# zhm1205/Multimodal_TTA

Hardware: AMD Instinct MI355X
Metric: adapted volumes/sec (higher is better)
Workload: dtype bf16

## Files before the change

include/mmtta.h:

```cpp
#ifndef MMTTA_H
#define MMTTA_H

#include <stdint.h>

#ifdef __cplusplus
extern "C" {
#endif

#define MMTTA_ABI_VERSION 2

typedef enum {
  MMTTA_OK = 0,
  MMTTA_ERR_INVALID = -1,
  MMTTA_ERR_UNSUPPORTED = -2,
  MMTTA_ERR_LAUNCH = -3,
  MMTTA_ERR_WORKSPACE = -4
} mmtta_status;

typedef enum { MMTTA_F32 = 0, MMTTA_BF16 = 1 } mmtta_dtype;

typedef struct {
  void* ptr;
  int32_t n, c, d, h, w;
  int64_t sn, sc, sd, sh, sw;
  int32_t dtype;
  int32_t flags;
} mmtta_tensor;

#define MMTTA_TENSOR_OWNS_PAD 1

#define MMTTA_ACT_NONE 0
#define MMTTA_ACT_RELU 1
#define MMTTA_ACT_LEAKY_RELU 2
typedef struct {
  const float* mean;
  const float* rstd;
  const float* gamma;
  const float* beta;
  int32_t relu;
  int32_t per_item;
  const float* scale;
  const float* shift;
  float negative_slope;
  int32_t _pad2;
} mmtta_norm_on_load;

const char* mmtta_last_error(void);
int mmtta_abi_version(void);

#define MMTTA_OPT_PROFILE_MAIN_KERNEL_ONLY 1
#define MMTTA_OPT_SPLITK_BELOW 2
#define MMTTA_OPT_SPLITK_TARGET 3
#define MMTTA_OPT_WGRAD_WORKGROUPS 4
#define MMTTA_OPT_WGRAD_THIN_SLABS 5
#define MMTTA_OPT_IGEMM_PIPELINE 6
#define MMTTA_OPT_EPILOGUE_VEC16 9
#define MMTTA_OPT_IGEMM_LEAN 10
#define MMTTA_OPT_WGRAD_VECTOR_STAGING 11
#define MMTTA_OPT_CLASS_FUSED_MIN_WORKGROUPS 12
#define MMTTA_OPT_THIN_MFMA 13
#define MMTTA_OPT_IGEMM_FRAGMENT_REUSE 14
int mmtta_set_option(int key, int value);

int mmtta_copy_strided(const mmtta_tensor* src, const mmtta_tensor* dst, void* stream);

typedef enum {
  MMTTA_CONV_FWD = 0,
  MMTTA_CONV_DGRAD = 1,
  MMTTA_CONVT_FWD = 2,
  MMTTA_CONVT_DGRAD = 3
} mmtta_conv_op;

typedef struct {
  int32_t op;
  int32_t ksize;
  int32_t stride;
  int32_t cin;
  int32_t cout;
  int32_t dtype;
} mmtta_conv_desc;

int64_t mmtta_conv_packed_bytes(const mmtta_conv_desc* desc);

int mmtta_conv_pack_weights(const mmtta_conv_desc* desc, const float* w_master, void* packed, void* stream);

typedef struct {
  mmtta_conv_desc desc;
  const float* w_master;
  void* packed;
} mmtta_pack_item;
int64_t mmtta_conv_pack_table_bytes(int count);
int mmtta_conv_pack_table_build(const mmtta_pack_item* items, int count, void* table_host, int64_t* total);
int mmtta_conv_pack_batched(const void* table_dev, int count, int64_t total, void* stream);

typedef struct {
  int32_t tiles;
  int32_t launches;
  int32_t ksplit;
  int32_t stats_rows;
  int32_t config;
  int32_t _pad;
  int64_t workspace_bytes;
} mmtta_conv_plan_t;

int mmtta_conv_plan(const mmtta_conv_desc* desc, const mmtta_tensor* x, const mmtta_tensor* y,
                    mmtta_conv_plan_t* plan);

typedef struct {
  const mmtta_tensor* add;
  mmtta_norm_on_load add_norm;
} mmtta_conv_epilogue;

int mmtta_conv_run(const mmtta_conv_desc* desc, const mmtta_tensor* x, const mmtta_norm_on_load* x_norm,
                   const void* packed, const float* bias, const mmtta_conv_epilogue* epi,
                   const mmtta_tensor* y, int accumulate, float* stats, void* workspace,
                   int64_t workspace_bytes, void* stream);

int mmtta_conv_route(const mmtta_conv_desc* desc, const mmtta_tensor* x, const mmtta_norm_on_load* x_norm,
                     const mmtta_conv_epilogue* epi, const mmtta_tensor* y, int accumulate, const float* stats);

typedef struct {
  int32_t items_per_set;
  int32_t inner;
  int64_t packed_outer, packed_inner;
  int64_t weight_outer, weight_inner;
  int64_t bias_outer, bias_inner;
} mmtta_param_sets;

int mmtta_conv_run_sets(const mmtta_conv_desc* desc, const mmtta_tensor* x, const mmtta_norm_on_load* x_norm,
                        const void* packed, const float* bias, const mmtta_conv_epilogue* epi,
                        const mmtta_tensor* y, int accumulate, float* stats, void* workspace,
                        int64_t workspace_bytes, const mmtta_param_sets* sets, void* stream);

int64_t mmtta_conv_wgrad_workspace_bytes(const mmtta_conv_desc* desc, const mmtta_tensor* x,
                                         const mmtta_tensor* dy);
int mmtta_conv_wgrad_kernel(const mmtta_conv_desc* desc, const mmtta_tensor* x, const mmtta_tensor* dy);
int mmtta_conv_wgrad(const mmtta_conv_desc* desc, const mmtta_tensor* x, const mmtta_norm_on_load* x_norm,
                     const mmtta_tensor* dy, float* dw, float* db, int accumulate, void* workspace,
                     int64_t workspace_bytes, void* stream);

int64_t mmtta_conv_wgrad_workspace_bytes_sets(const mmtta_conv_desc* desc, const mmtta_tensor* x, const mmtta_tensor* dy,
                                              const mmtta_param_sets* sets);
int mmtta_conv_wgrad_sets(const mmtta_conv_desc* desc, const mmtta_tensor* x, const mmtta_norm_on_load* x_norm,
                          const mmtta_tensor* dy, float* dw, float* db, int accumulate, void* workspace,
                          int64_t workspace_bytes, const mmtta_param_sets* sets, void* stream);
int mmtta_conv_wgrad_plan_sets(const mmtta_conv_desc* desc, const mmtta_tensor* x, const mmtta_tensor* dy,
                               const mmtta_param_sets* sets, int32_t plan[4]);

typedef struct {
  int32_t clip, zscore, masked, min_count;
  float lo, hi, mask_gt, eps;
  float mean, std;
  int32_t legacy, _pad;
} mmtta_intensity_rule;
int64_t mmtta_intensity_scratch_bytes(int channels);
int mmtta_intensity_normalize(const mmtta_tensor* x, const mmtta_intensity_rule* rules, const mmtta_tensor* y,
                              void* scratch, void* stream);

typedef enum {
  MMTTA_NORM_INSTANCE = 0,
  MMTTA_NORM_BATCH = 1,
  MMTTA_NORM_GROUP = 2
} mmtta_norm_kind;

int mmtta_norm_stats_finalize(int kind, int groups, const float* part, int rows_per_n, int n, int c,
                              int64_t count, float eps, int training, float* running_mean,
                              float* running_var, float momentum, float* mean, float* rstd,
                              const float* gamma, const float* beta, float* scale, float* shift,
                              double* scratch, void* stream);

typedef struct {
  int32_t items_per_set;
  int32_t _pad;
  int64_t affine_stride;
  int64_t stats_stride;
} mmtta_norm_sets;

int mmtta_norm_stats_finalize_sets(int kind, int groups, const float* part, int rows_per_n, int n, int c,
                                   int64_t count, float eps, int training, float* running_mean,
                                   float* running_var, float momentum, float* mean, float* rstd,
                                   const float* gamma, const float* beta, float* scale, float* shift,
                                   float* gamma_items, float* beta_items, double* scratch,
                                   const mmtta_norm_sets* sets, void* stream);

int mmtta_reduce_rows_per_n(const mmtta_tensor* t);

int mmtta_channel_stats(const mmtta_tensor* x, float* part, void* stream);

int mmtta_combine(const mmtta_tensor* a, const mmtta_norm_on_load* ta, const mmtta_tensor* b,
                  const mmtta_norm_on_load* tb, const mmtta_tensor* out, void* stream);

int mmtta_norm_bwd_reduce(const mmtta_tensor* dout, const mmtta_tensor* y, const mmtta_norm_on_load* t,
                          float* part, void* stream);

int mmtta_norm_bwd_finalize(int kind, int groups, const float* part, int rows_per_n, int n, int c, int64_t count,
                            const float* gamma, int training, float* m1, float* m2, float* dgamma,
                            float* dbeta, int accumulate, double* scratch , void* stream);

int mmtta_norm_bwd_finalize_sets(int kind, int groups, const float* part, int rows_per_n, int n, int c, int64_t count,
                                 const float* gamma, int training, float* m1, float* m2, float* dgamma,
                                 float* dbeta, int accumulate, double* scratch ,
                                 const mmtta_norm_sets* sets, void* stream);

int mmtta_norm_bwd_apply(const mmtta_tensor* dout, const mmtta_tensor* y, const mmtta_norm_on_load* t,
                         const float* m1, const float* m2, const mmtta_tensor* dy, void* stream);

int mmtta_norm_bwd_small_ok(const mmtta_tensor* dout, const mmtta_tensor* y, const mmtta_norm_on_load* t,
                            const mmtta_tensor* dy);
int mmtta_norm_bwd_small(const mmtta_tensor* dout, const mmtta_tensor* y, const mmtta_norm_on_load* t, int64_t count,
                         const mmtta_tensor* dy, void* stream);

int mmtta_upsample2x_fwd(const mmtta_tensor* x, const mmtta_tensor* y, void* stream);
int mmtta_upsample2x_bwd(const mmtta_tensor* dy, const mmtta_tensor* dx, int accumulate, void* stream);

int mmtta_lincomb(int count, const mmtta_tensor* const* in, const float* w, const mmtta_tensor* out,
                  int accumulate, void* stream);

#define MMTTA_PW_OP_CHANNEL_STATS 0
#define MMTTA_PW_OP_NORM_BWD_REDUCE 1
#define MMTTA_PW_OP_NORM_BWD_APPLY 2
#define MMTTA_PW_OP_NORM_BWD_SMALL 3
#define MMTTA_PW_OP_COMBINE 4
#define MMTTA_PW_OP_LINCOMB 5
#define MMTTA_PW_OP_UPSAMPLE_FWD 6
#define MMTTA_PW_OP_UPSAMPLE_BWD 7
#define MMTTA_PW_REDUCE 0
#define MMTTA_PW_REDUCE_STREAM 1
#define MMTTA_PW_ELEMENTWISE 2
#define MMTTA_PW_COMBINE8 3
#define MMTTA_PW_NORM_BWD_APPLY8 4
#define MMTTA_PW_NORM_BWD_SMALL 5
#define MMTTA_PW_LINCOMB 6
#define MMTTA_PW_UPSAMPLE_FWD 7
#define MMTTA_PW_UPSAMPLE_BWD 8
typedef struct {
  int64_t vox_per_row;
  int64_t work_items;
  int64_t grid_x;
  int32_t grid_y;
  int32_t family;
  int32_t mode;
  int32_t vec;
  int32_t it;
  int32_t count;
  int32_t bf16_a;
  int32_t bf16_b;
  int32_t bf16_o;
  int32_t has_b;
  int32_t rows_per_n;
  int32_t rows_per_block;
  int32_t cpl, nvl;
  int32_t trips;
  int32_t cb_passes;
  int32_t second_trip;
  int32_t leaky;
} mmtta_pointwise_route_t;
int mmtta_pointwise_route(int op, const mmtta_tensor* const* operands, int count, const mmtta_norm_on_load* t,
                          const mmtta_norm_on_load* t2, const float* m1, const float* m2, mmtta_pointwise_route_t* out);

int64_t mmtta_entropy_partials(const mmtta_tensor* logits);
int mmtta_entropy_loss(const mmtta_tensor* logits, int softmax, const mmtta_tensor* dlogits,
                       double* partial, float* loss, void* stream);

int64_t mmtta_entropy_partials_items(const mmtta_tensor* logits);
int mmtta_entropy_loss_items(const mmtta_tensor* logits, int softmax, const mmtta_tensor* dlogits,
                             double* partial, float* loss, void* stream);

int64_t mmtta_entropy_filtered_partials(const mmtta_tensor* logits);
int mmtta_entropy_filtered_items(const mmtta_tensor* logits, int softmax, float margin, const uint8_t* keep_in,
                                 uint8_t* keep_out, const mmtta_tensor* dlogits, double* partial, float* loss,
                                 int64_t* kept, void* stream);

int mmtta_mirror_views(const mmtta_tensor* x, const mmtta_tensor* y, int views, const int32_t* view_axes, void* stream);
int64_t mmtta_memo_partials(const mmtta_tensor* logits, int views);
int mmtta_memo_loss_items(const mmtta_tensor* logits, int softmax, int views, const int32_t* view_axes,
                          const mmtta_tensor* dlogits, double* partial, float* loss, void* stream);
int mmtta_memo_ensemble(const mmtta_tensor* logits, int softmax, int views, const int32_t* view_axes,
                        const mmtta_tensor* out, void* stream);

int64_t mmtta_consistency_partials(const mmtta_tensor* logits);
int mmtta_consistency_loss_items(const mmtta_tensor* logits, const mmtta_tensor* target, int softmax,
                                 const mmtta_tensor* dlogits, double* partial, float* loss, void* stream);
int64_t mmtta_cotta_update_partials(int64_t n, int sets);
int mmtta_cotta_update_sets(float* w, float* teacher, const float* source, int64_t n, int sets, int64_t w_stride,
                            int64_t teacher_stride, double alpha, float restore_p, uint64_t seed, const int32_t* step,
                            const int32_t* ordinals, int64_t* partial, int64_t* restored, void* stream);

int64_t mmtta_intensity_range_partials(const mmtta_tensor* x);
int mmtta_intensity_range(const mmtta_tensor* x, float* partial, float* range, void* stream);
int mmtta_augment_views(const mmtta_tensor* x, const mmtta_tensor* y, int views, const int32_t* view_axes,
                        const float* table_host, const float* table, const float* range, uint64_t seed,
                        const int32_t* ordinals, void* stream);

int64_t mmtta_entropy_weighted_partials(const mmtta_tensor* logits);
int mmtta_entropy_weighted_items(const mmtta_tensor* logits, int softmax, float margin, uint8_t* keep_out,
                                 const mmtta_tensor* dlogits, double* partial, float* loss, int64_t* kept, void* stream);
int64_t mmtta_pseudo_label_partials(const mmtta_tensor* logits);
int mmtta_pseudo_label_loss_items(const mmtta_tensor* logits, int softmax, const mmtta_tensor* dlogits, double* partial,
                                  float* loss, void* stream);
int mmtta_fisher_accumulate_sets(float* fisher, const float* grads, int64_t n, int sets, int64_t set_stride, void* stream);
int mmtta_fisher_scale(float* fisher, int64_t n, float count, void* stream);
int64_t mmtta_fisher_penalty_partials(int64_t n, int sets);
int mmtta_fisher_penalty_sets(const float* w, float* g, const float* fisher, const float* source, int64_t n, int sets,
                              int replicas, int64_t set_stride, float lambda, double* partial, float* penalty, void* stream);

int mmtta_adam_step(float* p, const float* g, float* m, float* v, int64_t n, int64_t n_decay, float lr,
                    float beta1, float beta2, float eps, float weight_decay, int32_t* step, void* stream);

enum { MMTTA_OPTIM_ADAM = 0, MMTTA_OPTIM_ADAMW = 1, MMTTA_OPTIM_SGD = 2 };
typedef struct mmtta_optim_desc {
  int32_t kind;
  float lr, beta1, beta2, eps, weight_decay;
  float momentum, dampening;
  int32_t nesterov;
} mmtta_optim_desc;
int mmtta_optim_step(const mmtta_optim_desc* desc, float* p, const float* g, float* m, float* v, int64_t n,
                     int64_t n_decay, int32_t* step, void* stream);

int mmtta_optim_step_sets(const mmtta_optim_desc* desc, float* p, const float* g, float* m, float* v, int64_t n,
                          int64_t n_decay, int sets, int64_t set_stride, int32_t* step, void* stream);

typedef struct mmtta_update_target {
  mmtta_optim_desc optim;
  float* w_p; float* w_m; float* w_v;
  float* b_p; float* b_m; float* b_v;
  float* b_grad;
  void* image[2];
  int64_t image_outer[2], image_inner[2];
  const int32_t* step;
  int32_t w_decay, b_decay;
} mmtta_update_target;
int mmtta_fused_update_enabled(void);
int mmtta_conv_wgrad_update_sets(const mmtta_conv_desc* desc, const mmtta_tensor* x, const mmtta_norm_on_load* x_norm,
                                 const mmtta_tensor* dy, const mmtta_update_target* target, void* workspace,
                                 int64_t workspace_bytes, const mmtta_param_sets* sets, void* stream);

int mmtta_optim_step_segments(const mmtta_optim_desc* desc, float* p, const float* g, float* m, float* v, const int64_t* segments,
                              int count, int64_t total, int sets, int64_t set_stride, int32_t* step, void* stream);

int64_t mmtta_sam_ascent_partials(int64_t n, int sets);
int mmtta_sam_ascent_sets(float* p, const float* g, float* saved, int64_t saved_stride, double* partial, int64_t n, int sets,
                          int replicas, int64_t set_stride, float rho, void* stream);

int mmtta_mask_dice_counts(const mmtta_tensor* logits, const mmtta_tensor* label, float threshold,
                           int64_t* counts, uint8_t* mask, void* stream);

int64_t mmtta_dice_ce_scratch_bytes(const mmtta_tensor* logits);
int mmtta_dice_ce_sums(const mmtta_tensor* logits, const mmtta_tensor* label, const float* weight,
                       int squared_pred, int softmax, double* out, void* scratch, void* stream);

int mmtta_dice_ce_grad(const mmtta_tensor* logits, const mmtta_tensor* label, const float* weight, int squared_pred,
                       int softmax, int jaccard, int include_background, float lambda_dice, float lambda_ce, float smooth_nr,
                       float smooth_dr, const double* sums, const mmtta_tensor* dlogits, void* stream);

int64_t mmtta_calibration_scratch_bytes(const mmtta_tensor* logits, int bins);
int mmtta_calibration_bins(const mmtta_tensor* logits, const mmtta_tensor* label, int softmax, int bins, int scope,
                           double* out, void* scratch, void* stream);

int64_t mmtta_components_scratch_bytes(int64_t n_masks, int64_t d, int64_t h, int64_t w);
int mmtta_components_filter(const uint8_t* mask_in, uint8_t* mask_out, const mmtta_tensor* label, int n, int r, int d, int h,
                            int w, int connectivity, const int64_t* min_voxels, const int32_t* keep_largest, int64_t* counts,
                            int64_t* stats, int32_t* labels, void* scratch, void* stream);

int64_t mmtta_lesionwise_scratch_bytes(int64_t n_masks, int64_t d, int64_t h, int64_t w);
int mmtta_lesionwise_scores(const uint8_t* mask, const mmtta_tensor* label, int n, int r, int d, int h, int w, int iterations,
                            int dilation_connectivity, const int64_t* min_lesion_voxels, int64_t* stats, int32_t* labels,
                            void* scratch, void* stream);

int64_t mmtta_mask_fill_nest_scratch_bytes(int64_t n_masks, int64_t d, int64_t h, int64_t w);
int mmtta_mask_fill_nest(uint8_t* mask, const mmtta_tensor* label, int n, int r, int d, int h, int w, int fill_connectivity,
                         const int32_t* fill_holes, const int64_t* max_hole_voxels, const int32_t* chain, int chain_len,
                         int nest_mode, int64_t* counts, int64_t* stats, void* scratch, void* stream);

int64_t mmtta_surface_scratch_bytes(int64_t n_masks, int64_t d, int64_t h, int64_t w);
int mmtta_surface_distances(const uint8_t* pred_mask, const mmtta_tensor* label, const double* spacing,
                            double percentile, int asd_symmetric, float* hd, float* asd, void* scratch, void* stream);

#ifdef __cplusplus
}
#endif
#endif
```

multimodal_tta_amd/_lib.py:

```python
from __future__ import annotations

import ctypes as C
import os
from typing import Optional, Sequence

import torch

_HERE = os.path.dirname(os.path.abspath(__file__))
LIB_PATH = os.path.join(_HERE, "csrc", "libmmtta.so")

F32, BF16 = 0, 1
CONV_FWD, CONV_DGRAD, CONVT_FWD, CONVT_DGRAD = 0, 1, 2, 3
NORM_INSTANCE, NORM_BATCH, NORM_GROUP = 0, 1, 2


class MmttaError(RuntimeError):
    pass


class Tensor(C.Structure):
    _fields_ = [
        ("ptr", C.c_void_p),
        ("n", C.c_int32), ("c", C.c_int32), ("d", C.c_int32), ("h", C.c_int32), ("w", C.c_int32),
        ("sn", C.c_int64), ("sc", C.c_int64), ("sd", C.c_int64), ("sh", C.c_int64), ("sw", C.c_int64),
        ("dtype", C.c_int32), ("flags", C.c_int32),
    ]


class NormOnLoad(C.Structure):
    _fields_ = [
        ("mean", C.c_void_p), ("rstd", C.c_void_p), ("gamma", C.c_void_p), ("beta", C.c_void_p),
        ("relu", C.c_int32), ("per_item", C.c_int32), ("scale", C.c_void_p), ("shift", C.c_void_p),
    ]


class NormOnLoadAct(NormOnLoad):
    _fields_ = [("negative_slope", C.c_float), ("_pad2", C.c_int32)]


class NormSets(C.Structure):
    _fields_ = [("items_per_set", C.c_int32), ("_pad", C.c_int32), ("affine_stride", C.c_int64), ("stats_stride", C.c_int64)]


class ConvDesc(C.Structure):
    _fields_ = [
        ("op", C.c_int32), ("ksize", C.c_int32), ("stride", C.c_int32), ("cin", C.c_int32), ("cout", C.c_int32),
        ("dtype", C.c_int32),
    ]


class PackItem(C.Structure):
    _fields_ = [("desc", ConvDesc), ("w_master", C.c_void_p), ("packed", C.c_void_p)]


class ParamSets(C.Structure):
    _fields_ = [("items_per_set", C.c_int32), ("inner", C.c_int32), ("packed_outer", C.c_int64), ("packed_inner", C.c_int64),
                ("weight_outer", C.c_int64), ("weight_inner", C.c_int64), ("bias_outer", C.c_int64), ("bias_inner", C.c_int64)]


class ConvPlan(C.Structure):
    _fields_ = [
        ("tiles", C.c_int32), ("launches", C.c_int32), ("ksplit", C.c_int32), ("stats_rows", C.c_int32),
        ("config", C.c_int32), ("_pad", C.c_int32), ("workspace_bytes", C.c_int64),
    ]


class PointwiseRoute(C.Structure):
    _fields_ = [("vox_per_row", C.c_int64), ("work_items", C.c_int64), ("grid_x", C.c_int64), ("grid_y", C.c_int32),
                ("family", C.c_int32), ("mode", C.c_int32), ("vec", C.c_int32), ("it", C.c_int32), ("count", C.c_int32),
                ("bf16_a", C.c_int32), ("bf16_b", C.c_int32), ("bf16_o", C.c_int32), ("has_b", C.c_int32),
                ("rows_per_n", C.c_int32), ("rows_per_block", C.c_int32), ("cpl", C.c_int32), ("nvl", C.c_int32),
                ("trips", C.c_int32), ("cb_passes", C.c_int32), ("second_trip", C.c_int32), ("leaky", C.c_int32)]


PW_OPS = ("channel_stats", "norm_bwd_reduce", "norm_bwd_apply", "norm_bwd_small", "combine", "lincomb", "upsample_fwd",
          "upsample_bwd")
PW_FAMILIES = ("reduce", "reduce_stream", "elementwise", "combine8", "norm_bwd_apply8", "norm_bwd_small", "lincomb",
               "upsample_fwd", "upsample_bwd")


class OptimDesc(C.Structure):
    _fields_ = [("kind", C.c_int32), ("lr", C.c_float), ("beta1", C.c_float), ("beta2", C.c_float), ("eps", C.c_float),
                ("weight_decay", C.c_float), ("momentum", C.c_float), ("dampening", C.c_float), ("nesterov", C.c_int32)]


class UpdateTarget(C.Structure):
    _fields_ = [("optim", OptimDesc), ("w_p", C.c_void_p), ("w_m", C.c_void_p), ("w_v", C.c_void_p), ("b_p", C.c_void_p),
                ("b_m", C.c_void_p), ("b_v", C.c_void_p), ("b_grad", C.c_void_p), ("image", C.c_void_p * 2),
                ("image_outer", C.c_int64 * 2), ("image_inner", C.c_int64 * 2), ("step", C.c_void_p),
                ("w_decay", C.c_int32), ("b_decay", C.c_int32)]


OPTIM_ADAM, OPTIM_ADAMW, OPTIM_SGD = 0, 1, 2


class ConvEpilogue(C.Structure):
    _fields_ = [("add", C.POINTER(Tensor)), ("add_norm", NormOnLoadAct)]


class IntensityRule(C.Structure):
    _fields_ = [("clip", C.c_int32), ("zscore", C.c_int32), ("masked", C.c_int32), ("min_count", C.c_int32),
                ("lo", C.c_float), ("hi", C.c_float), ("mask_gt", C.c_float), ("eps", C.c_float),
                ("mean", C.c_float), ("std", C.c_float), ("legacy", C.c_int32), ("_pad", C.c_int32)]


_P = C.POINTER
_SIGNATURES = {
    "mmtta_last_error": (C.c_char_p, []),
    "mmtta_abi_version": (C.c_int, []),
    "mmtta_set_option": (C.c_int, [C.c_int, C.c_int]),
    "mmtta_intensity_scratch_bytes": (C.c_int64, [C.c_int]),
    "mmtta_intensity_normalize": (C.c_int, [_P(Tensor), _P(IntensityRule), _P(Tensor), C.c_void_p, C.c_void_p]),
    "mmtta_copy_strided": (C.c_int, [_P(Tensor), _P(Tensor), C.c_void_p]),
    "mmtta_conv_packed_bytes": (C.c_int64, [_P(ConvDesc)]),
    "mmtta_conv_pack_weights": (C.c_int, [_P(ConvDesc), C.c_void_p, C.c_void_p, C.c_void_p]),
    "mmtta_conv_pack_table_bytes": (C.c_int64, [C.c_int]),
    "mmtta_conv_pack_table_build": (C.c_int, [_P(PackItem), C.c_int, C.c_void_p, _P(C.c_int64)]),
    "mmtta_conv_pack_batched": (C.c_int, [C.c_void_p, C.c_int, C.c_int64, C.c_void_p]),
    "mmtta_conv_plan": (C.c_int, [_P(ConvDesc), _P(Tensor), _P(Tensor), _P(ConvPlan)]),
    "mmtta_conv_run": (C.c_int, [_P(ConvDesc), _P(Tensor), _P(NormOnLoad), C.c_void_p, C.c_void_p, _P(ConvEpilogue),
                                 _P(Tensor), C.c_int, C.c_void_p, C.c_void_p, C.c_int64, C.c_void_p]),
    "mmtta_conv_run_sets": (C.c_int, [_P(ConvDesc), _P(Tensor), _P(NormOnLoad), C.c_void_p, C.c_void_p, _P(ConvEpilogue),
                                      _P(Tensor), C.c_int, C.c_void_p, C.c_void_p, C.c_int64, _P(ParamSets), C.c_void_p]),
    "mmtta_conv_route": (C.c_int, [_P(ConvDesc), _P(Tensor), _P(NormOnLoad), _P(ConvEpilogue), _P(Tensor), C.c_int, C.c_void_p]),
    "mmtta_conv_wgrad_workspace_bytes": (C.c_int64, [_P(ConvDesc), _P(Tensor), _P(Tensor)]),
    "mmtta_conv_wgrad_workspace_bytes_sets": (C.c_int64, [_P(ConvDesc), _P(Tensor), _P(Tensor), _P(ParamSets)]),
    "mmtta_conv_wgrad_plan_sets": (C.c_int, [_P(ConvDesc), _P(Tensor), _P(Tensor), _P(ParamSets), _P(C.c_int32)]),
    "mmtta_conv_wgrad_sets": (C.c_int, [_P(ConvDesc), _P(Tensor), _P(NormOnLoad), _P(Tensor), C.c_void_p, C.c_void_p,
                                        C.c_int, C.c_void_p, C.c_int64, _P(ParamSets), C.c_void_p]),
    "mmtta_conv_wgrad_kernel": (C.c_int, [_P(ConvDesc), _P(Tensor), _P(Tensor)]),
    "mmtta_conv_wgrad": (C.c_int, [_P(ConvDesc), _P(Tensor), _P(NormOnLoad), _P(Tensor), C.c_void_p, C.c_void_p,
                                   C.c_int, C.c_void_p, C.c_int64, C.c_void_p]),
    "mmtta_norm_stats_finalize": (C.c_int, [C.c_int, C.c_int, C.c_void_p, C.c_int, C.c_int, C.c_int, C.c_int64,
                                            C.c_float, C.c_int, C.c_void_p, C.c_void_p, C.c_float, C.c_void_p,
                                            C.c_void_p, C.c_void_p, C.c_void_p, C.c_void_p, C.c_void_p, C.c_void_p,
                                            C.c_void_p]),
    "mmtta_norm_stats_finalize_sets": (C.c_int, [C.c_int, C.c_int, C.c_void_p, C.c_int, C.c_int, C.c_int, C.c_int64,
                                                 C.c_float, C.c_int, C.c_void_p, C.c_void_p, C.c_float, C.c_void_p,
                                                 C.c_void_p, C.c_void_p, C.c_void_p, C.c_void_p, C.c_void_p, C.c_void_p,
                                                 C.c_void_p, C.c_void_p, _P(NormSets), C.c_void_p]),
    "mmtta_reduce_rows_per_n": (C.c_int, [_P(Tensor)]),
    "mmtta_channel_stats": (C.c_int, [_P(Tensor), C.c_void_p, C.c_void_p]),
    "mmtta_combine": (C.c_int, [_P(Tensor), _P(NormOnLoad), _P(Tensor), _P(NormOnLoad), _P(Tensor), C.c_void_p]),
    "mmtta_norm_bwd_reduce": (C.c_int, [_P(Tensor), _P(Tensor), _P(NormOnLoad), C.c_void_p, C.c_void_p]),
    "mmtta_norm_bwd_finalize": (C.c_int, [C.c_int, C.c_int, C.c_void_p, C.c_int, C.c_int, C.c_int, C.c_int64,
                                          C.c_void_p, C.c_int, C.c_void_p, C.c_void_p, C.c_void_p, C.c_void_p,
                                          C.c_int, C.c_void_p, C.c_void_p]),
    "mmtta_norm_bwd_finalize_sets": (C.c_int, [C.c_int, C.c_int, C.c_void_p, C.c_int, C.c_int, C.c_int, C.c_int64,
                                               C.c_void_p, C.c_int, C.c_void_p, C.c_void_p, C.c_void_p, C.c_void_p,
                                               C.c_int, C.c_void_p, _P(NormSets), C.c_void_p]),
    "mmtta_norm_bwd_apply": (C.c_int, [_P(Tensor), _P(Tensor), _P(NormOnLoad), C.c_void_p, C.c_void_p, _P(Tensor),
                                       C.c_void_p]),
    "mmtta_norm_bwd_small_ok": (C.c_int, [_P(Tensor), _P(Tensor), _P(NormOnLoad), _P(Tensor)]),
    "mmtta_norm_bwd_small": (C.c_int, [_P(Tensor), _P(Tensor), _P(NormOnLoad), C.c_int64, _P(Tensor), C.c_void_p]),
    "mmtta_upsample2x_fwd": (C.c_int, [_P(Tensor), _P(Tensor), C.c_void_p]),
    "mmtta_upsample2x_bwd": (C.c_int, [_P(Tensor), _P(Tensor), C.c_int, C.c_void_p]),
    "mmtta_lincomb": (C.c_int, [C.c_int, _P(_P(Tensor)), _P(C.c_float), _P(Tensor), C.c_int, C.c_void_p]),
    "mmtta_pointwise_route": (C.c_int, [C.c_int, _P(_P(Tensor)), C.c_int, _P(NormOnLoad), _P(NormOnLoad), C.c_void_p, C.c_void_p,
                                        _P(PointwiseRoute)]),
    "mmtta_entropy_partials": (C.c_int64, [_P(Tensor)]),
    "mmtta_entropy_loss": (C.c_int, [_P(Tensor), C.c_int, _P(Tensor), C.c_void_p, C.c_void_p, C.c_void_p]),
    "mmtta_entropy_partials_items": (C.c_int64, [_P(Tensor)]),
    "mmtta_entropy_loss_items": (C.c_int, [_P(Tensor), C.c_int, _P(Tensor), C.c_void_p, C.c_void_p, C.c_void_p]),
    "mmtta_entropy_filtered_partials": (C.c_int64, [_P(Tensor)]),
    "mmtta_entropy_filtered_items": (C.c_int, [_P(Tensor), C.c_int, C.c_float, C.c_void_p, C.c_void_p, _P(Tensor), C.c_void_p,
                                               C.c_void_p, C.c_void_p, C.c_void_p]),
    "mmtta_mirror_views": (C.c_int, [_P(Tensor), _P(Tensor), C.c_int, _P(C.c_int32), C.c_void_p]),
    "mmtta_memo_partials": (C.c_int64, [_P(Tensor), C.c_int]),
    "mmtta_memo_loss_items": (C.c_int, [_P(Tensor), C.c_int, C.c_int, _P(C.c_int32), _P(Tensor), C.c_void_p, C.c_void_p,
                                        C.c_void_p]),
    "mmtta_memo_ensemble": (C.c_int, [_P(Tensor), C.c_int, C.c_int, _P(C.c_int32), _P(Tensor), C.c_void_p]),
    "mmtta_consistency_partials": (C.c_int64, [_P(Tensor)]),
    "mmtta_consistency_loss_items": (C.c_int, [_P(Tensor), _P(Tensor), C.c_int, _P(Tensor), C.c_void_p, C.c_void_p, C.c_void_p]),
    "mmtta_cotta_update_partials": (C.c_int64, [C.c_int64, C.c_int]),
    "mmtta_cotta_update_sets": (C.c_int, [C.c_void_p, C.c_void_p, C.c_void_p, C.c_int64, C.c_int, C.c_int64, C.c_int64,
                                          C.c_double, C.c_float, C.c_uint64, C.c_void_p, C.c_void_p, C.c_void_p, C.c_void_p,
                                          C.c_void_p]),
    "mmtta_intensity_range_partials": (C.c_int64, [_P(Tensor)]),
    "mmtta_intensity_range": (C.c_int, [_P(Tensor), C.c_void_p, C.c_void_p, C.c_void_p]),
    "mmtta_augment_views": (C.c_int, [_P(Tensor), _P(Tensor), C.c_int, _P(C.c_int32), C.c_void_p, C.c_void_p, C.c_void_p,
                                      C.c_uint64, C.c_void_p, C.c_void_p]),
    "mmtta_entropy_weighted_partials": (C.c_int64, [_P(Tensor)]),
    "mmtta_entropy_weighted_items": (C.c_int, [_P(Tensor), C.c_int, C.c_float, C.c_void_p, _P(Tensor), C.c_void_p, C.c_void_p,
                                               C.c_void_p, C.c_void_p]),
    "mmtta_pseudo_label_partials": (C.c_int64, [_P(Tensor)]),
    "mmtta_pseudo_label_loss_items": (C.c_int, [_P(Tensor), C.c_int, _P(Tensor), C.c_void_p, C.c_void_p, C.c_void_p]),
    "mmtta_fisher_accumulate_sets": (C.c_int, [C.c_void_p, C.c_void_p, C.c_int64, C.c_int, C.c_int64, C.c_void_p]),
    "mmtta_fisher_scale": (C.c_int, [C.c_void_p, C.c_int64, C.c_float, C.c_void_p]),
    "mmtta_fisher_penalty_partials": (C.c_int64, [C.c_int64, C.c_int]),
    "mmtta_fisher_penalty_sets": (C.c_int, [C.c_void_p, C.c_void_p, C.c_void_p, C.c_void_p, C.c_int64, C.c_int, C.c_int,
                                            C.c_int64, C.c_float, C.c_void_p, C.c_void_p, C.c_void_p]),
    "mmtta_adam_step": (C.c_int, [C.c_void_p, C.c_void_p, C.c_void_p, C.c_void_p, C.c_int64, C.c_int64, C.c_float,
                                  C.c_float, C.c_float, C.c_float, C.c_float, C.c_void_p, C.c_void_p]),
    "mmtta_optim_step": (C.c_int, [_P(OptimDesc), C.c_void_p, C.c_void_p, C.c_void_p, C.c_void_p, C.c_int64, C.c_int64,
                                   C.c_void_p, C.c_void_p]),
    "mmtta_optim_step_sets": (C.c_int, [_P(OptimDesc), C.c_void_p, C.c_void_p, C.c_void_p, C.c_void_p, C.c_int64, C.c_int64,
                                        C.c_int, C.c_int64, C.c_void_p, C.c_void_p]),
    "mmtta_optim_step_segments": (C.c_int, [_P(OptimDesc), C.c_void_p, C.c_void_p, C.c_void_p, C.c_void_p, C.c_void_p, C.c_int,
                                            C.c_int64, C.c_int, C.c_int64, C.c_void_p, C.c_void_p]),
    "mmtta_fused_update_enabled": (C.c_int, []),
    "mmtta_conv_wgrad_update_sets": (C.c_int, [_P(ConvDesc), _P(Tensor), _P(NormOnLoad), _P(Tensor), _P(UpdateTarget),
                                               C.c_void_p, C.c_int64, _P(ParamSets), C.c_void_p]),
    "mmtta_sam_ascent_partials": (C.c_int64, [C.c_int64, C.c_int]),
    "mmtta_sam_ascent_sets": (C.c_int, [C.c_void_p, C.c_void_p, C.c_void_p, C.c_int64, C.c_void_p, C.c_int64, C.c_int, C.c_int,
                                        C.c_int64, C.c_float, C.c_void_p]),
    "mmtta_mask_dice_counts": (C.c_int, [_P(Tensor), _P(Tensor), C.c_float, C.c_void_p, C.c_void_p, C.c_void_p]),
    "mmtta_dice_ce_scratch_bytes": (C.c_int64, [_P(Tensor)]),
    "mmtta_dice_ce_sums": (C.c_int, [_P(Tensor), _P(Tensor), C.c_void_p, C.c_int, C.c_int, C.c_void_p, C.c_void_p, C.c_void_p]),
    "mmtta_dice_ce_grad": (C.c_int, [_P(Tensor), _P(Tensor), C.c_void_p, C.c_int, C.c_int, C.c_int, C.c_int, C.c_float, C.c_float,
                                     C.c_float, C.c_float, C.c_void_p, _P(Tensor), C.c_void_p]),
    "mmtta_calibration_scratch_bytes": (C.c_int64, [_P(Tensor), C.c_int]),
    "mmtta_calibration_bins": (C.c_int, [_P(Tensor), _P(Tensor), C.c_int, C.c_int, C.c_int, C.c_void_p, C.c_void_p, C.c_void_p]),
    "mmtta_components_scratch_bytes": (C.c_int64, [C.c_int64, C.c_int64, C.c_int64, C.c_int64]),
    "mmtta_components_filter": (C.c_int, [C.c_void_p, C.c_void_p, _P(Tensor), C.c_int, C.c_int, C.c_int, C.c_int, C.c_int, C.c_int,
                                          _P(C.c_int64), _P(C.c_int32), C.c_void_p, C.c_void_p, C.c_void_p, C.c_void_p, C.c_void_p]),
    "mmtta_lesionwise_scratch_bytes": (C.c_int64, [C.c_int64, C.c_int64, C.c_int64, C.c_int64]),
    "mmtta_lesionwise_scores": (C.c_int, [C.c_void_p, _P(Tensor), C.c_int, C.c_int, C.c_int, C.c_int, C.c_int, C.c_int, C.c_int,
                                          _P(C.c_int64), C.c_void_p, C.c_void_p, C.c_void_p, C.c_void_p]),
    "mmtta_mask_fill_nest_scratch_bytes": (C.c_int64, [C.c_int64, C.c_int64, C.c_int64, C.c_int64]),
    "mmtta_mask_fill_nest": (C.c_int, [C.c_void_p, _P(Tensor), C.c_int, C.c_int, C.c_int, C.c_int, C.c_int, C.c_int, _P(C.c_int32),
                                       _P(C.c_int64), _P(C.c_int32), C.c_int, C.c_int, C.c_void_p, C.c_void_p, C.c_void_p, C.c_void_p]),
    "mmtta_surface_scratch_bytes": (C.c_int64, [C.c_int64, C.c_int64, C.c_int64, C.c_int64]),
    "mmtta_surface_distances": (C.c_int, [C.c_void_p, _P(Tensor), _P(C.c_double), C.c_double, C.c_int, C.c_void_p,
                                          C.c_void_p, C.c_void_p, C.c_void_p]),
}

_lib = None


def load() -> C.CDLL:
    global _lib
    if _lib is not None:
        return _lib
    if not os.path.exists(LIB_PATH):
        raise MmttaError(
            f"{LIB_PATH} is missing: build it with `python -m multimodal_tta_amd.build` (hipcc, gfx950). "
            "There is no CPU or PyTorch fallback for the adaptation path."
        )
    lib = C.CDLL(LIB_PATH)
    for name, (res, args) in _SIGNATURES.items():
        fn = getattr(lib, name)
        fn.restype = res
        fn.argtypes = args
    if lib.mmtta_abi_version() != 2:
        raise MmttaError("libmmtta.so ABI version mismatch")
    if os.environ.get("MMTTA_NO_PIPE", "0") == "1":
        lib.mmtta_set_option(6, 0)
    if os.environ.get("MMTTA_NO_EPIVEC", "0") == "1":
        lib.mmtta_set_option(9, 0)
    if "MMTTA_WGVEC" in os.environ:
        lib.mmtta_set_option(11, int(os.environ["MMTTA_WGVEC"]))
    if "MMTTA_THINMFMA" in os.environ:
        lib.mmtta_set_option(13, int(os.environ["MMTTA_THINMFMA"]))
    if "MMTTA_CLSFUSE" in os.environ:
        lib.mmtta_set_option(12, int(os.environ["MMTTA_CLSFUSE"]))
    if "MMTTA_LEAN" in os.environ:
        lib.mmtta_set_option(10, int(os.environ["MMTTA_LEAN"]))
    _lib = lib
    return lib


def exported_names() -> Sequence[str]:
    return list(_SIGNATURES)


def check(status: int, what: str = "") -> None:
    if status != 0:
        msg = load().mmtta_last_error().decode("utf-8", "replace")
        raise MmttaError(f"{what or 'libmmtta'} failed with status {status}: {msg}")


def stream_ptr() -> int:
    return int(torch.cuda.current_stream().cuda_stream)


def ptr(t: Optional[torch.Tensor]) -> Optional[int]:
    return None if t is None else int(t.data_ptr())


TENSOR_OWNS_PAD = 1


def desc_cl(t: torch.Tensor) -> Tensor:
    if t.dim() != 5 or t.dtype not in (torch.float32, torch.bfloat16) or not t.is_cuda:
        raise MmttaError(f"expected a CUDA float32 / bfloat16 [N,D,H,W,C] view, got {tuple(t.shape)} {t.dtype} {t.device}")
    n, d, h, w, c = t.shape
    sn, sd, sh, sw, sc = t.stride()
    if sc != 1 and c != 1:
        raise MmttaError("activation views must have unit stride along C")
    flags = TENSOR_OWNS_PAD if getattr(t, "_mmtta_owns_pad", False) else 0
    return Tensor(t.data_ptr(), n, c, d, h, w, sn, 1, sd, sh, sw, BF16 if t.dtype == torch.bfloat16 else F32, flags)


def desc_ncdhw(t: torch.Tensor) -> Tensor:
    if t.dim() != 5 or t.dtype != torch.float32 or not t.is_cuda:
        raise MmttaError(f"expected a CUDA float32 [N,C,D,H,W] tensor, got {tuple(t.shape)} {t.dtype} {t.device}")
    n, c, d, h, w = t.shape
    sn, sc, sd, sh, sw = t.stride()
    return Tensor(t.data_ptr(), n, c, d, h, w, sn, sc, sd, sh, sw, F32, 0)


ACT_NONE, ACT_RELU, ACT_LEAKY_RELU = 0, 1, 2


def norm_on_load(mean=None, rstd=None, gamma=None, beta=None, relu=False, scale=None, shift=None,
                 per_item=False, act=None, negative_slope=0.0) -> NormOnLoadAct:
    code = (ACT_RELU if relu else ACT_NONE) if act is None else int(act)
    return NormOnLoadAct(ptr(mean), ptr(rstd), ptr(gamma), ptr(beta), code, 1 if per_item else 0, ptr(scale),
                      ptr(shift), float(negative_slope) if code == ACT_LEAKY_RELU else 0.0, 0)
```

multimodal_tta_amd/csrc/api.hip:

```cpp
#include "common.h"
#include <string.h>

namespace mmtta {
static thread_local char g_err[512] = "";
void set_error(const char* fmt, ...) {
  va_list ap;
  va_start(ap, fmt);
  vsnprintf(g_err, sizeof(g_err), fmt, ap);
  va_end(ap);
}
int g_profile_main_only = 0;
int g_igemm_pipeline = 1;
int g_epilogue_vec = 1;
int g_igemm_lean = 1;
int g_igemm_reuse = 1;
int g_cls_fused_min = 128;
int g_thin_mfma = 2;
int g_wgrad_vec = 1;
int g_tune[4] = {96, 128, 128, 256};
}

extern "C" int mmtta_set_option(int key, int value) {
  if (key == MMTTA_OPT_PROFILE_MAIN_KERNEL_ONLY) {
    const int prev = mmtta::g_profile_main_only;
    mmtta::g_profile_main_only = value;
    return prev;
  }
  if (key == MMTTA_OPT_WGRAD_VECTOR_STAGING) {
    const int prev = mmtta::g_wgrad_vec;
    mmtta::g_wgrad_vec = value ? 1 : 0;
    return prev;
  }
  if (key == MMTTA_OPT_THIN_MFMA) {
    const int prev = mmtta::g_thin_mfma;
    mmtta::g_thin_mfma = value < 0 ? 0 : (value > 3 ? 3 : value);
    return prev;
  }
  if (key == MMTTA_OPT_CLASS_FUSED_MIN_WORKGROUPS) {
    const int prev = mmtta::g_cls_fused_min;
    mmtta::g_cls_fused_min = value < 0 ? 0 : value;
    return prev;
  }
  if (key == MMTTA_OPT_IGEMM_LEAN) {
    const int prev = mmtta::g_igemm_lean;
    mmtta::g_igemm_lean = value ? 1 : 0;
    return prev;
  }
  if (key == MMTTA_OPT_IGEMM_FRAGMENT_REUSE) {
    const int prev = mmtta::g_igemm_reuse;
    mmtta::g_igemm_reuse = value ? 1 : 0;
    return prev;
  }
  if (key == MMTTA_OPT_EPILOGUE_VEC16) {
    const int prev = mmtta::g_epilogue_vec;
    mmtta::g_epilogue_vec = value ? 1 : 0;
    return prev;
  }
  if (key == MMTTA_OPT_IGEMM_PIPELINE) {
    const int prev = mmtta::g_igemm_pipeline;
    mmtta::g_igemm_pipeline = value ? 1 : 0;
    return prev;
  }
  if (key >= MMTTA_OPT_SPLITK_BELOW && key <= MMTTA_OPT_WGRAD_THIN_SLABS) {
    if (value < 1) return MMTTA_ERR_INVALID;
    const int prev = mmtta::g_tune[key - MMTTA_OPT_SPLITK_BELOW];
    mmtta::g_tune[key - MMTTA_OPT_SPLITK_BELOW] = value;
    return prev;
  }
  return MMTTA_ERR_INVALID;
}

extern "C" const char* mmtta_last_error(void) { return mmtta::g_err; }
extern "C" int mmtta_abi_version(void) { return MMTTA_ABI_VERSION; }
```

multimodal_tta_amd/csrc/common.h:

```cpp
#pragma once
#include <hip/hip_runtime.h>
#include <type_traits>
#include <stdint.h>
#include <stdio.h>
#include <stdarg.h>
#include "../../include/mmtta.h"

namespace mmtta {

constexpr int WAVE = 64;

void set_error(const char* fmt, ...);

#define MMTTA_CHECK(cond, code, ...)      \
  do {                                    \
    if (!(cond)) {                        \
      ::mmtta::set_error(__VA_ARGS__);    \
      return (code);                      \
    }                                     \
  } while (0)

inline int launch_status(const char* what) {
  hipError_t e = hipGetLastError();
  if (e != hipSuccess) {
    set_error("%s: %s", what, hipGetErrorString(e));
    return MMTTA_ERR_LAUNCH;
  }
  return MMTTA_OK;
}

extern int g_profile_main_only;
extern int g_igemm_pipeline;
extern int g_wgrad_vec;
extern int g_igemm_lean;
extern int g_igemm_reuse;
extern int g_cls_fused_min;
extern int g_thin_mfma;
extern int g_epilogue_vec;
extern int g_tune[4];

inline bool nl_leaky(const mmtta_norm_on_load* t) { return t != nullptr && t->relu == MMTTA_ACT_LEAKY_RELU; }
inline int nl_act_check(const mmtta_norm_on_load* t, const char* what) {
  MMTTA_CHECK(t == nullptr || (t->relu >= MMTTA_ACT_NONE && t->relu <= MMTTA_ACT_LEAKY_RELU), MMTTA_ERR_INVALID,
              "%s: activation code %d (MMTTA_ACT_NONE, _RELU or _LEAKY_RELU)", what, t ? t->relu : 0);
  MMTTA_CHECK(t == nullptr || t->relu != MMTTA_ACT_LEAKY_RELU || __builtin_isfinite(t->negative_slope), MMTTA_ERR_INVALID,
              "%s: LeakyReLU negative_slope must be finite", what);
  return MMTTA_OK;
}

struct PackImageGeo {
  int A, B, T, Kp, Np, kn_is_ba, plain_bf16;
};
int pack_image_geometry(const mmtta_conv_desc* d, PackImageGeo& g);

#define MMTTA_ACT_BODIES                                                                                                    \
  int conv_run_body(const mmtta_conv_desc* d, const mmtta_tensor* x, const mmtta_norm_on_load* x_norm, const void* packed,  \
                    const float* bias, const mmtta_conv_epilogue* epi, const mmtta_tensor* y, int accumulate, float* stats, \
                    void* workspace, int64_t workspace_bytes, const mmtta_param_sets* sets, void* stream);                \
  int conv_wgrad_body(const mmtta_conv_desc* d, const mmtta_tensor* x, const mmtta_norm_on_load* x_norm,                    \
                      const mmtta_tensor* dy, float* dw, float* db, int accumulate, void* workspace,                        \
                      int64_t workspace_bytes, const mmtta_param_sets* sets, void* stream,                                  \
                      const mmtta_update_target* upd);                                                                      \
  int combine_body(const mmtta_tensor* a, const mmtta_norm_on_load* ta, const mmtta_tensor* b,                              \
                   const mmtta_norm_on_load* tb, const mmtta_tensor* out, void* stream);                                    \
  int norm_bwd_reduce_body(const mmtta_tensor* dout, const mmtta_tensor* y, const mmtta_norm_on_load* t, float* part,      \
                           void* stream);                                                                                   \
  int norm_bwd_apply_body(const mmtta_tensor* dout, const mmtta_tensor* y, const mmtta_norm_on_load* t, const float* m1,   \
                          const float* m2, const mmtta_tensor* dy, void* stream);                                           \
  int norm_bwd_small_body(const mmtta_tensor* dout, const mmtta_tensor* y, const mmtta_norm_on_load* t, int64_t count,     \
                          const mmtta_tensor* dy, void* stream);
namespace leaky { MMTTA_ACT_BODIES }

#ifdef MMTTA_ACT_LEAKY_TU
#define MMTTA_ACT_NS_OPEN namespace leaky {
#define MMTTA_ACT_NS_CLOSE }
#else
#define MMTTA_ACT_NS_OPEN
#define MMTTA_ACT_NS_CLOSE
#endif

MMTTA_ACT_NS_OPEN
MMTTA_ACT_BODIES

inline bool is_cl(const mmtta_tensor* t) { return t->sc == 1 || t->c == 1; }

inline bool is_f32(const mmtta_tensor* t) { return t->dtype == MMTTA_F32; }
inline bool is_bf16(const mmtta_tensor* t) { return t->dtype == MMTTA_BF16; }

inline bool quad_aligned(const mmtta_tensor* t, int base_bytes, int elems = 4) {
  return ((uintptr_t)t->ptr) % base_bytes == 0 && t->sw % elems == 0 && t->sh % elems == 0 && t->sd % elems == 0 &&
         t->sn % elems == 0;
}
inline int quad_bytes(const mmtta_tensor* t) { return is_bf16(t) ? 8 : 16; }
inline bool item_fits_31(const mmtta_tensor* t, int64_t pad) {
  const int64_t last = (int64_t)(t->d - 1) * t->sd + (int64_t)(t->h - 1) * t->sh + (int64_t)(t->w - 1) * t->sw + pad;
  return last < ((int64_t)1 << 31);
}
inline bool strides_fit_24(const mmtta_tensor* t) { return t->sw < (1 << 24) && t->sh < (1 << 24) && t->sd < (1 << 24); }
inline bool voxel_dense(const mmtta_tensor* t) { return t->sc == 1 && t->sh == (int64_t)t->w * t->sw && t->sd == (int64_t)t->h * t->sh; }
inline bool dense_rows16(const mmtta_tensor* t) {
  const int q = is_bf16(t) ? 8 : 4;
  return voxel_dense(t) && ((uintptr_t)t->ptr) % 16 == 0 && t->sw % q == 0 && t->sn % q == 0 &&
         (int64_t)t->d * t->h * t->w * t->sw < ((int64_t)1 << 31);
}
inline bool same_shape(const mmtta_tensor* a, const mmtta_tensor* b) {
  return a->n == b->n && a->c == b->c && a->d == b->d && a->h == b->h && a->w == b->w;
}

__device__ __forceinline__ float bf16_bits_to_f32(unsigned int h) { return __uint_as_float(h << 16); }
__device__ __forceinline__ unsigned int f32x2_to_bf16x2(float lo, float hi) {
  typedef __bf16 bf2 __attribute__((ext_vector_type(2)));
  bf2 v;
  v[0] = (__bf16)lo;
  v[1] = (__bf16)hi;
  return __builtin_bit_cast(unsigned int, v);
}
__device__ __forceinline__ unsigned short f32_to_bf16_bits(float v) { return __builtin_bit_cast(unsigned short, (__bf16)v); }
__device__ __forceinline__ uint4 bf16x8_pack(const unsigned short* h) {
  uint4 q;
  q.x = h[0] | ((unsigned)h[1] << 16); q.y = h[2] | ((unsigned)h[3] << 16);
  q.z = h[4] | ((unsigned)h[5] << 16); q.w = h[6] | ((unsigned)h[7] << 16);
  return q;
}
__device__ __forceinline__ float4 ld4_any(const float* base, long long eoff, int bf) {
  if (bf) {
    const uint2 u = *reinterpret_cast<const uint2*>(reinterpret_cast<const unsigned short*>(base) + eoff);
    return make_float4(bf16_bits_to_f32(u.x & 0xffffu), bf16_bits_to_f32(u.x >> 16), bf16_bits_to_f32(u.y & 0xffffu),
                       bf16_bits_to_f32(u.y >> 16));
  }
  return *reinterpret_cast<const float4*>(base + eoff);
}
__device__ __forceinline__ void st4_any(float* base, long long eoff, float4 v, int bf) {
  if (bf) {
    uint2 u;
    u.x = f32x2_to_bf16x2(v.x, v.y);
    u.y = f32x2_to_bf16x2(v.z, v.w);
    *reinterpret_cast<uint2*>(reinterpret_cast<unsigned short*>(base) + eoff) = u;
  } else {
    *reinterpret_cast<float4*>(base + eoff) = v;
  }
}
__device__ __forceinline__ float ld1_any(const float* base, long long eoff, int bf) {
  if (bf) return bf16_bits_to_f32(reinterpret_cast<const unsigned short*>(base)[eoff]);
  return base[eoff];
}
__device__ __forceinline__ void st1_any(float* base, long long eoff, float v, int bf) {
  if (bf) reinterpret_cast<unsigned short*>(base)[eoff] = (unsigned short)(f32x2_to_bf16x2(v, 0.f) & 0xffffu);
  else base[eoff] = v;
}
__device__ __forceinline__ void ld8_any(const float* base, long long eoff, int bf, float4& lo, float4& hi) {
  if (bf) {
    const uint4 u = *reinterpret_cast<const uint4*>(reinterpret_cast<const unsigned short*>(base) + eoff);
    lo = make_float4(bf16_bits_to_f32(u.x & 0xffffu), bf16_bits_to_f32(u.x >> 16), bf16_bits_to_f32(u.y & 0xffffu),
                     bf16_bits_to_f32(u.y >> 16));
    hi = make_float4(bf16_bits_to_f32(u.z & 0xffffu), bf16_bits_to_f32(u.z >> 16), bf16_bits_to_f32(u.w & 0xffffu),
                     bf16_bits_to_f32(u.w >> 16));
  } else {
    lo = *reinterpret_cast<const float4*>(base + eoff);
    hi = *reinterpret_cast<const float4*>(base + eoff + 4);
  }
}

template <bool BF> struct Oct8 { float4 lo, hi; };
template <> struct Oct8<true> { uint4 q; };
template <bool BF>
__device__ __forceinline__ Oct8<BF> oct8_ld(const float* base, unsigned eoff_lo, unsigned eoff_hi) {
  Oct8<BF> o;
  if constexpr (BF) {
    o.q = *reinterpret_cast<const uint4*>(reinterpret_cast<const unsigned short*>(base) + eoff_lo);
  } else {
    o.lo = *reinterpret_cast<const float4*>(base + eoff_lo);
    o.hi = *reinterpret_cast<const float4*>(base + eoff_hi);
  }
  return o;
}
__device__ __forceinline__ void oct8_f8(const Oct8<false>& o, float (&v)[8]) {
  v[0] = o.lo.x; v[1] = o.lo.y; v[2] = o.lo.z; v[3] = o.lo.w; v[4] = o.hi.x; v[5] = o.hi.y; v[6] = o.hi.z; v[7] = o.hi.w;
}
__device__ __forceinline__ void oct8_f8(const Oct8<true>& o, float (&v)[8]) {
  v[0] = bf16_bits_to_f32(o.q.x & 0xffffu); v[1] = __uint_as_float(o.q.x & 0xffff0000u);
  v[2] = bf16_bits_to_f32(o.q.y & 0xffffu); v[3] = __uint_as_float(o.q.y & 0xffff0000u);
  v[4] = bf16_bits_to_f32(o.q.z & 0xffffu); v[5] = __uint_as_float(o.q.z & 0xffff0000u);
  v[6] = bf16_bits_to_f32(o.q.w & 0xffffu); v[7] = __uint_as_float(o.q.w & 0xffff0000u);
}


template <bool BF>
__device__ __forceinline__ void oct8_st(float* base, unsigned eoff, const float (&v)[8]) {
  if constexpr (BF) {
    uint4 q;
    q.x = f32x2_to_bf16x2(v[0], v[1]); q.y = f32x2_to_bf16x2(v[2], v[3]);
    q.z = f32x2_to_bf16x2(v[4], v[5]); q.w = f32x2_to_bf16x2(v[6], v[7]);
    *reinterpret_cast<uint4*>(reinterpret_cast<unsigned short*>(base) + eoff) = q;
  } else {
    *reinterpret_cast<float4*>(base + eoff) = make_float4(v[0], v[1], v[2], v[3]);
    *reinterpret_cast<float4*>(base + eoff + 4) = make_float4(v[4], v[5], v[6], v[7]);
  }
}
template <bool BF>
__device__ __forceinline__ const float* item_base(const float* p, long long n, long long sn) {
  return BF ? reinterpret_cast<const float*>(reinterpret_cast<const unsigned short*>(p) + n * sn) : p + n * sn;
}

template <int I, int N, class F>
__device__ __forceinline__ void static_for(F&& f) {
  if constexpr (I < N) {
    f(std::integral_constant<int, I>{});
    static_for<I + 1, N>(f);
  }
}

template <int I, int N, int STEP, class F>
__device__ __forceinline__ void static_for_step(F&& f) {
  if constexpr (I < N) {
    f(std::integral_constant<int, I>{});
    static_for_step<I + STEP, N, STEP>(f);
  }
}

template <bool BF> __device__ __forceinline__ float4 ld4_t(const float* base, long long eoff) { return ld4_any(base, eoff, BF ? 1 : 0); }
template <bool BF> __device__ __forceinline__ float ld1_t(const float* base, long long eoff) { return ld1_any(base, eoff, BF ? 1 : 0); }
template <bool BF> __device__ __forceinline__ void st4_t(float* base, long long eoff, float4 v) { st4_any(base, eoff, v, BF ? 1 : 0); }
template <bool BF> __device__ __forceinline__ void st1_t(float* base, long long eoff, float v) { st1_any(base, eoff, v, BF ? 1 : 0); }
template <bool BF> __device__ __forceinline__ void ld8_t(const float* base, long long eoff, float4& lo, float4& hi) {
  ld8_any(base, eoff, BF ? 1 : 0, lo, hi);
}
#define MMTTA_BF_DISPATCH(flag, NAME, ...) \
  do {                                      \
    if (flag) {                             \
      constexpr bool NAME = true;           \
      __VA_ARGS__                           \
    } else {                                \
      constexpr bool NAME = false;          \
      __VA_ARGS__                           \
    }                                       \
  } while (0)

struct TV {
  float* p;
  int n, c, d, h, w;
  long long sn, sc, sd, sh, sw;
  int flags;
  int bf;
};

inline TV tv(const mmtta_tensor* t) {
  TV v;
  v.p = (float*)t->ptr;
  v.flags = t->flags;
  v.bf = t->dtype == MMTTA_BF16 ? 1 : 0;
  v.n = t->n; v.c = t->c; v.d = t->d; v.h = t->h; v.w = t->w;
  v.sn = t->sn; v.sc = t->sc; v.sd = t->sd; v.sh = t->sh; v.sw = t->sw;
  return v;
}

__device__ __forceinline__ void vox_decompose(const TV& t, long long v, int& n, int& z, int& y, int& x) {
  x = (int)(v % t.w); v /= t.w;
  y = (int)(v % t.h); v /= t.h;
  z = (int)(v % t.d);
  n = (int)(v / t.d);
}
__device__ __forceinline__ long long vox_addr(const TV& t, int n, int z, int y, int x) {
  return (long long)n * t.sn + (long long)z * t.sd + (long long)y * t.sh + (long long)x * t.sw;
}

#ifdef MMTTA_ACT_LEAKY_TU
typedef float act_t;
#define MMTTA_ACT_ID 1.f
#else
typedef int act_t;
#define MMTTA_ACT_ID 0
#endif
inline act_t act_arg(const mmtta_norm_on_load* t) {
#ifdef MMTTA_ACT_LEAKY_TU
  if (t == nullptr) return 1.f;
  return t->relu == MMTTA_ACT_LEAKY_RELU ? t->negative_slope : (t->relu == MMTTA_ACT_RELU ? 0.f : 1.f);
#else
  return t == nullptr ? 0 : t->relu;
#endif
}

struct NL {
  const float* mean;
  const float* rstd;
  const float* gamma;
  const float* beta;
  act_t relu;
  const float* scale;
  const float* shift;
};

inline NL nl(const mmtta_norm_on_load* t) {
  NL r;
  if (t == nullptr) { r.mean = r.rstd = r.gamma = r.beta = r.scale = r.shift = nullptr; r.relu = MMTTA_ACT_ID; return r; }
  r.mean = t->mean; r.rstd = t->rstd; r.gamma = t->gamma; r.beta = t->beta; r.relu = act_arg(t);
  r.scale = t->scale; r.shift = t->scale ? t->shift : nullptr;
  return r;
}
template <class Args>
inline int epilogue_add(const mmtta_conv_epilogue* epi, const mmtta_tensor* y, Args& a) {
  a.add = nullptr; a.asn = a.asd = a.ash = a.asw = 0; a.tadd = nl(nullptr);
  if (!(epi && epi->add)) return MMTTA_OK;
  const mmtta_tensor* ad = epi->add;
  MMTTA_CHECK(ad->ptr && is_cl(ad) && same_shape(ad, y), MMTTA_ERR_INVALID,
              "conv: epilogue `add` must be channels-last with the shape of y");
  a.add = (const float*)ad->ptr; a.asn = ad->sn; a.asd = ad->sd; a.ash = ad->sh; a.asw = ad->sw;
  a.tadd = nl(&epi->add_norm);
  return MMTTA_OK;
}
inline int nl_per_item_check(const mmtta_norm_on_load* t, const char* what) {
  MMTTA_CHECK(t == nullptr || t->per_item == 0 || t->mean == nullptr || t->scale != nullptr, MMTTA_ERR_INVALID,
              "%s: a norm-on-load with per-item gamma / beta needs its precombined scale / shift", what);
  return MMTTA_OK;
}

struct PSets {
  int ips, inner;
  long long packed_outer, packed_inner;
  long long weight_outer, weight_inner;
  long long bias_outer, bias_inner;
};

inline PSets psets(const mmtta_param_sets* g) {
  PSets r;
  if (g == nullptr) { r.ips = 1; r.inner = 1; r.packed_outer = r.packed_inner = r.weight_outer = r.weight_inner = r.bias_outer = r.bias_inner = 0; return r; }
  r.ips = g->items_per_set; r.inner = g->inner;
  r.packed_outer = g->packed_outer; r.packed_inner = g->packed_inner;
  r.weight_outer = g->weight_outer; r.weight_inner = g->weight_inner;
  r.bias_outer = g->bias_outer; r.bias_inner = g->bias_inner;
  return r;
}
inline int psets_validate(const mmtta_param_sets* g, int n) {
  if (g == nullptr) return MMTTA_OK;
  MMTTA_CHECK(g->items_per_set >= 1 && g->inner >= 1, MMTTA_ERR_INVALID, "param sets: items_per_set %d, inner %d (both >= 1)",
              g->items_per_set, g->inner);
  MMTTA_CHECK(n % g->items_per_set == 0, MMTTA_ERR_INVALID, "param sets: batch %d is no multiple of items_per_set %d", n,
              g->items_per_set);
  MMTTA_CHECK(g->packed_outer % 16 == 0 && g->packed_inner % 16 == 0 && g->weight_outer % 4 == 0 && g->weight_inner % 4 == 0 &&
                  g->bias_outer % 4 == 0 && g->bias_inner % 4 == 0,
              MMTTA_ERR_INVALID, "param sets: strides must keep 16-byte alignment");
  return MMTTA_OK;
}
__host__ __device__ __forceinline__ bool psets_on(const PSets& g) {
  return (g.packed_outer | g.packed_inner | g.weight_outer | g.weight_inner | g.bias_outer | g.bias_inner) != 0;
}
__device__ __forceinline__ int pset_of(const PSets& g, int n) { return g.ips == 1 ? n : n / g.ips; }
__device__ __forceinline__ long long pset_packed_bytes(const PSets& g, int q) {
  return g.inner == 1 ? q * g.packed_outer : (q / g.inner) * g.packed_outer + (q % g.inner) * g.packed_inner;
}
__device__ __forceinline__ long long pset_weight_elems(const PSets& g, int q) {
  return g.inner == 1 ? q * g.weight_outer : (q / g.inner) * g.weight_outer + (q % g.inner) * g.weight_inner;
}
__device__ __forceinline__ long long pset_bias_elems(const PSets& g, int q) {
  return g.inner == 1 ? q * g.bias_outer : (q / g.inner) * g.bias_outer + (q % g.inner) * g.bias_inner;
}
template <class T>
__device__ __forceinline__ const T* pset_packed(const PSets& g, const T* base, int n) {
  return reinterpret_cast<const T*>(reinterpret_cast<const char*>(base) + pset_packed_bytes(g, pset_of(g, n)));
}
__device__ __forceinline__ const float* pset_bias(const PSets& g, const float* base, int n) {
  return base == nullptr ? nullptr : base + pset_bias_elems(g, pset_of(g, n));
}

__device__ __forceinline__ void nl_coeff(const NL& t, int n, int C, int c, float& sc, float& sh) {
  if (t.scale != nullptr) { sc = t.scale[n * C + c]; sh = t.shift[n * C + c]; return; }
  if (t.mean == nullptr) { sc = 1.f; sh = 0.f; return; }
  float mu = t.mean[n * C + c], rs = t.rstd[n * C + c];
  float g = t.gamma ? t.gamma[c] : 1.f;
  float b = t.beta ? t.beta[c] : 0.f;
  sc = rs * g;
  sh = b - mu * sc;
}

template <int J>
__device__ __forceinline__ void nl_coeff_vec(const NL& t, int n, int C, int c0, float* sc, float* sh) {
  if (t.scale != nullptr) {
#pragma unroll
    for (int j = 0; j < J; ++j) {
      const int i = n * C + min(c0 + j, C - 1);
      sc[j] = t.scale[i]; sh[j] = t.shift[i];
    }
  } else if (t.mean == nullptr) {
#pragma unroll
    for (int j = 0; j < J; ++j) { sc[j] = 1.f; sh[j] = 0.f; }
  } else {
    float mu[J], rs[J], g[J], b[J];
#pragma unroll
    for (int j = 0; j < J; ++j) {
      const int cc = min(c0 + j, C - 1);
      mu[j] = t.mean[n * C + cc]; rs[j] = t.rstd[n * C + cc];
      g[j] = 1.f; b[j] = 0.f;
    }
    if (t.gamma != nullptr) {
#pragma unroll
      for (int j = 0; j < J; ++j) g[j] = t.gamma[min(c0 + j, C - 1)];
    }
    if (t.beta != nullptr) {
#pragma unroll
      for (int j = 0; j < J; ++j) b[j] = t.beta[min(c0 + j, C - 1)];
    }
#pragma unroll
    for (int j = 0; j < J; ++j) { sc[j] = rs[j] * g[j]; sh[j] = b[j] - mu[j] * sc[j]; }
  }
#pragma unroll
  for (int j = 0; j < J; ++j)
    if (c0 + j >= C) { sc[j] = 0.f; sh[j] = 0.f; }
}

#ifdef MMTTA_ACT_LEAKY_TU
__device__ __forceinline__ float act_max(float v, float k) { return v > 0.f ? v : k * v; }
__device__ __forceinline__ float act_lo(float k) { return k; }
__device__ __forceinline__ float nl_apply(float x, float sc, float sh, float k) { return act_max(fmaf(x, sc, sh), k); }
#define MMTTA_ACT_BWD(dz, k, post) \
  do {                             \
    if (!((post) > 0.f)) (dz) *= (k); \
  } while (0)
#else
__device__ __forceinline__ float nl_apply(float x, float sc, float sh, int relu) {
  float v = fmaf(x, sc, sh);
  return relu ? fmaxf(v, 0.f) : v;
}
__device__ __forceinline__ float act_max(float v, float lo) { return fmaxf(v, lo); }
__device__ __forceinline__ float act_lo(int relu) { return relu ? 0.f : -__builtin_inff(); }
#define MMTTA_ACT_BWD(dz, relu, post) \
  do {                                \
    if ((relu) && !((post) > 0.f)) (dz) = 0.f; \
  } while (0)
#endif

__device__ __forceinline__ unsigned xcd_contiguous_id(unsigned b, unsigned nwg) {
  const unsigned x = b & 7u, i = b >> 3, q = nwg >> 3, r = nwg & 7u;
  return (x < r ? x * (q + 1) : r * (q + 1) + (x - r) * q) + i;
}

__device__ __forceinline__ void unit_range(long long units, unsigned lb, unsigned nwg, long long& first, long long& last) {
  const long long per = (units + nwg - 1) / nwg;
  first = per * lb;
  last = first + per < units ? first + per : units;
}

__device__ __forceinline__ float wave_sum(float v) {
  auto step = [](float x, auto ctrl, auto rmask) {
    const int moved = __builtin_amdgcn_update_dpp(0, __builtin_bit_cast(int, x), decltype(ctrl)::value, decltype(rmask)::value, 0xf, true);
    return x + __builtin_bit_cast(float, moved);
  };
  v = step(v, std::integral_constant<int, 0x111>{}, std::integral_constant<int, 0xf>{});
  v = step(v, std::integral_constant<int, 0x112>{}, std::integral_constant<int, 0xf>{});
  v = step(v, std::integral_constant<int, 0x114>{}, std::integral_constant<int, 0xf>{});
  v = step(v, std::integral_constant<int, 0x118>{}, std::integral_constant<int, 0xf>{});
  v = step(v, std::integral_constant<int, 0x142>{}, std::integral_constant<int, 0xa>{});
  v = step(v, std::integral_constant<int, 0x143>{}, std::integral_constant<int, 0xc>{});
  return __builtin_bit_cast(float, __builtin_amdgcn_readlane(__builtin_bit_cast(int, v), 63));
}
__device__ __forceinline__ double wave_sum_d(double v) {
#pragma unroll
  for (int o = 32; o > 0; o >>= 1) v += __shfl_xor(v, o, 64);
  return v;
}

__device__ __forceinline__ double block_sum_d(double v, double* sh) {
  v = wave_sum_d(v);
  const int lane = threadIdx.x & 63, wave = threadIdx.x >> 6;
  if (lane == 0) sh[wave] = v;
  __syncthreads();
  double t = 0.0;
  if (threadIdx.x == 0)
    for (int w = 0; w < (int)(blockDim.x >> 6); ++w) t += sh[w];
  return t;
}

__device__ __forceinline__ void bernoulli_entropy_terms(float t, float& h, float& g) {
  const float a = fabsf(t);
  const float e = __builtin_amdgcn_exp2f(-a * 1.4426950408889634f);
  const float r = __builtin_amdgcn_rcpf(1.f + e);
  const float sig = t >= 0.f ? r : e * r;
  const float series = e * fmaf(e, fmaf(e, fmaf(e, -0.25f, 0.33333334f), -0.5f), 1.f);
  const float lg = __builtin_amdgcn_logf(1.f + e) * 0.6931471805599453f;
  const float l1p = e < 0.015625f ? series : lg;
  h = fmaxf(t, 0.f) + l1p - t * sig;
  g = -t * (e * r * r);
}

__device__ __forceinline__ void fent_store_partials(double acc, int cnt, double* partial, double* sh) {
  const double s = block_sum_d(acc, sh);
  __syncthreads();
  const double c = block_sum_d((double)cnt, sh);
  if (threadIdx.x == 0) {
    double* p = partial + (long long)blockIdx.y * 2 * gridDim.x;
    p[blockIdx.x] = s;
    p[gridDim.x + blockIdx.x] = c;
  }
}

__device__ __forceinline__ float fent_scale(const long long* kept) {
  const long long k = kept[blockIdx.y];
  return k > 0 ? (float)(1.0 / (double)k) : 0.f;
}

struct OptimArgs {
  float lr, beta1, beta2, eps, wd, momentum, dampening;
  int nesterov;
};

template <int KIND>
__device__ __forceinline__ void optim_update(float& pi, float gi, float& mi, float& vi, bool decay, const OptimArgs& a,
                                             float step_size, float bc2_sqrt, bool first) {
#pragma clang fp contract(off)
  if (KIND == 0) {
    if (decay) gi = fmaf(a.wd, pi, gi);
    mi = fmaf(1.f - a.beta1, gi - mi, mi);
    vi = fmaf((1.f - a.beta2) * gi, gi, vi * a.beta2);
    const float denom = sqrtf(vi) / bc2_sqrt + a.eps;
    pi = fmaf(-step_size, mi / denom, pi);
  } else if (KIND == 1) {
    if (decay) pi = pi * (1.f - a.lr * a.wd);
    mi = fmaf(1.f - a.beta1, gi - mi, mi);
    vi = fmaf((1.f - a.beta2) * gi, gi, vi * a.beta2);
    const float denom = sqrtf(vi) / bc2_sqrt + a.eps;
    pi = fmaf(-step_size, mi / denom, pi);
  } else {
    if (decay) gi = fmaf(a.wd, pi, gi);
    if (a.momentum != 0.f) {
      mi = first ? gi : fmaf(a.momentum, mi, (1.f - a.dampening) * gi);
      gi = a.nesterov ? fmaf(a.momentum, mi, gi) : mi;
    }
    pi = fmaf(-a.lr, gi, pi);
  }
}

__device__ __forceinline__ void optim_scalars(int kind, const OptimArgs& a, int t0, float& step_size, float& bc2_sqrt) {
  const double t = (double)(t0 + 1);
  const double bc1 = 1.0 - pow((double)a.beta1, t);
  const double bc2 = 1.0 - pow((double)a.beta2, t);
  step_size = kind == 2 ? a.lr : (float)((double)a.lr / bc1);
  bc2_sqrt = kind == 2 ? 1.f : (float)sqrt(bc2);
}

int channel_partial_rows(const mmtta_tensor* t);
int launch_channel_sums(const mmtta_tensor* x, float* part, hipStream_t s);

bool direct_applicable(const mmtta_conv_desc* d);
long long upconv8_image_bytes(const mmtta_conv_desc* d);
long long chan_frag_bytes(const mmtta_conv_desc* d);
int direct_blocks_per_n(const mmtta_conv_desc* d, const mmtta_tensor* x, const mmtta_tensor* y);
bool pointwise_small_applicable(const mmtta_conv_desc* d, const mmtta_tensor* x, const mmtta_tensor* y, const float* stats,
                                const mmtta_tensor* add, const mmtta_norm_on_load* x_norm);
int pointwise_small_run(const mmtta_tensor* x, const void* packed, int Kp, int Np, const float* bias, const mmtta_tensor* y,
                        int accumulate, const PSets& sets, hipStream_t stream);
bool chan_applicable(const mmtta_conv_desc* d, const mmtta_tensor* x, const mmtta_tensor* y);
int chan_tiles_per_n(const mmtta_tensor* y);
int chan_conv_run(const mmtta_conv_desc* d, const mmtta_tensor* x, const mmtta_norm_on_load* x_norm, const void* packed, int Kp,
                  int Np, const float* bias, const mmtta_conv_epilogue* epi, const mmtta_tensor* y, int accumulate, float* stats,
                  const PSets& sets, hipStream_t stream);
int direct_conv_run(const mmtta_conv_desc* d, const mmtta_tensor* x, const mmtta_norm_on_load* x_norm, const void* packed,
                    const float* bias, const mmtta_conv_epilogue* epi, const mmtta_tensor* y, int accumulate, float* stats,
                    const PSets& sets, hipStream_t stream);

MMTTA_ACT_NS_CLOSE
}
```

multimodal_tta_amd/csrc/conv_igemm.hip:

```cpp
#include "common.h"

namespace mmtta {
MMTTA_ACT_NS_OPEN

typedef float f32x16 __attribute__((ext_vector_type(16)));
typedef __bf16 bf16x8 __attribute__((ext_vector_type(8)));
typedef __bf16 bf16x2 __attribute__((ext_vector_type(2)));

__device__ __forceinline__ unsigned int pack_bf16x2(float lo, float hi) {
  bf16x2 v;
  v[0] = (__bf16)lo;
  v[1] = (__bf16)hi;
  return __builtin_bit_cast(unsigned int, v);
}

struct Taps {
  int n;
  int slab[27];
  signed char dz[27], dy[27], dx[27];
  int zmin, ymin, xmin;
  int zext, yext, xext;
};

struct ClassInfo {
  int tap0, ntaps;
  int oz, oy, ox;
  int zmin, ymin, xmin;
  int zext, yext, xext;
  int Dg, Hg, Wg;
  int BX, BXY;
  unsigned mBX, mBXY;
};

struct GArgs {
  const float* in; long long isn, isd, ish, isw; int Ci, Di, Hi, Wi;
  NL tin;
  float* out; long long osn, osd, osh, osw; int Co, Do, Ho, Wo;
  int so;
  int si;
  const float* wp; int Kp, Np;
  const float* bias;
  PSets ps;
  const float* add; long long asn, asd, ash, asw; NL tadd;
  int accumulate;
  float* stats; int stats_rows_per_n;
  float* ws; int ksplit, stages_per_split, nstages;
  int tz, ty, tx;
  int in_bf, out_bf, add_bf;
  int vec4;
  int ovec;
  int coef_off;
  int rowload;
  int flip27;
  int ncls;
  ClassInfo cls[8];
  int toff[27];
  int slab[27];
};

__device__ __forceinline__ void class_of_tile(const GArgs& a, int tile, int& cidx, int& t) {
  if (a.ncls == 8) { cidx = 7 - (tile & 7); t = tile >> 3; }
  else { cidx = 0; t = tile; }
}

template <int TZ, int TY, int TX, bool PERM>
__device__ __forceinline__ void row_to_local(int v, int& zl, int& yl, int& xl) {
  if (PERM) {
    static_assert(TX == 8 && TY % 4 == 0, "the permutation assumes 4 x 8 row blocks");
    const int r = v & 31, q = r >> 2;
    const int y = (0xEB14 >> (2 * q)) & 3;
    const int xh = (q >> 1) & 1;
    v = (v & ~31) + y * 8 + xh * 4 + (r & 3);
  }
  xl = v % TX;
  yl = (v / TX) % TY;
  zl = v / (TX * TY);
}

constexpr int LDS_PITCH_BF16 = 12;

__host__ __device__ constexpr int tap27_off(int t, int rby) { return ((t / 9) * rby + (t / 3) % 3) * LDS_PITCH_BF16 + t % 3; }

__host__ __device__ constexpr int reuse_xslot(int bx) { return (bx & 1) * 5 + (bx >> 1); }
__host__ __device__ constexpr int reuse_row(int i, int b) {
  const int yl = i >> 2, x = 2 * (i & 3) + b, xh = x >> 2;
  int q = 0;
  for (int c = 0; c < 8; ++c)
    if (((0xEB14 >> (2 * c)) & 3) == yl && ((c >> 1) & 1) == xh) q = c;
  return q * 4 + (x & 3);
}

template <int TZ, int TY, int TX, int MB, bool PERM, bool ABF, bool XPAR = false>
__device__ __forceinline__ void epilogue_vec16(const GArgs& a, const float* biasp, const ClassInfo& ci, f32x16 (&acc)[MB], float* tr,
                                               int lane, int rowblock0, int colbase, bool colact, int n, int gz0, int gy0, int gx0,
                                               float (&ssum)[4], float (&ssq)[4]) {
  int osd = (int)a.osd, osh = (int)a.osh, osw = (int)a.osw, asd = (int)a.asd, ash_ = (int)a.ash, asw = (int)a.asw;
  int so = a.so, Do = a.Do, Ho = a.Ho, Wo = a.Wo, coz = ci.oz, coy = ci.oy, cox = ci.ox, cDg = ci.Dg, cHg = ci.Hg, cWg = ci.Wg;
  asm volatile("" : "+s"(osd), "+s"(osh), "+s"(osw), "+s"(asd), "+s"(ash_), "+s"(asw), "+s"(so), "+s"(Do), "+s"(Ho), "+s"(Wo));
  asm volatile("" : "+s"(coz), "+s"(coy), "+s"(cox), "+s"(cDg), "+s"(cHg), "+s"(cWg));
  const int h = lane >> 5, r = lane & 31;
  const int rsub = lane >> 3, c4 = (lane & 7) * 4;
  const int colv = colbase + c4;
  const bool cvok = colact && colv < a.Co;
  const int colc = min(colv, a.Co - 4);
  float4 bias4 = make_float4(0.f, 0.f, 0.f, 0.f);
  float asc[4] = {1.f, 1.f, 1.f, 1.f}, ash[4] = {0.f, 0.f, 0.f, 0.f};
  if (biasp) bias4 = *reinterpret_cast<const float4*>(biasp + colc);
  if (a.add) nl_coeff_vec<4>(a.tadd, n, a.Co, colc, asc, ash);
#pragma unroll
  for (int j = 0; j < 4; ++j) { ssum[j] = 0.f; ssq[j] = 0.f; }
  const float* addb = a.add;
  float* outb = a.out;
  const long long abase = (long long)n * a.asn + colc, obase = (long long)n * a.osn + colc;
  auto finish = [&](const float4& val, const float4& addq, const float4& oldq, bool okk, int oo) {
    float v[4] = {val.x + bias4.x, val.y + bias4.y, val.z + bias4.z, val.w + bias4.w};
    if (a.add) {
      const float av[4] = {addq.x, addq.y, addq.z, addq.w};
#pragma unroll
      for (int j = 0; j < 4; ++j) v[j] += nl_apply(av[j], asc[j], ash[j], a.tadd.relu);
    }
    if (a.accumulate) { v[0] += oldq.x; v[1] += oldq.y; v[2] += oldq.z; v[3] += oldq.w; }
    if (okk) {
      st4_t<ABF>(outb, obase + oo, make_float4(v[0], v[1], v[2], v[3]));
#pragma unroll
      for (int j = 0; j < 4; ++j) { ssum[j] += v[j]; ssq[j] += v[j] * v[j]; }
    }
  };
  if constexpr (XPAR) {
    static_assert(MB == 2, "two parity blocks");
#pragma unroll
    for (int b = 0; b < 2; ++b)
#pragma unroll
      for (int i = 0; i < 16; ++i) tr[(reuse_row(i, b) + 32 * h) * 36 + r] = acc[b][i];
  }
  const bool interior = PERM && so == 1 && coz == 0 && coy == 0 && cox == 0 && gz0 + TZ <= min(cDg, Do) && gy0 + TY <= min(cHg, Ho) &&
                        gx0 + TX <= min(cWg, Wo);
  if (interior) {
    const bool lb = (rsub >> 2) != 0;
    const int lxo = (rsub & 3) * osw, lxa = (rsub & 3) * asw;
    constexpr int T = 0xEB14;
    auto row_off = [&](int mb, int k, int sd_, int sh_, int sw_, int lx) {
      const int rb = rowblock0 + mb;
      const int zl = TY == 4 ? rb : (rb >> 1), yb = TY == 4 ? 0 : (rb & 1) * 4;
      const int u = (gz0 + zl) * sd_ + (gy0 + yb) * sh_ + (gx0 + 4 * (k & 1)) * sw_;
      const int y0 = (T >> (2 * (2 * k))) & 3, y1 = (T >> (2 * (2 * k + 1))) & 3;
      return (lb ? u + y1 * sh_ : u + y0 * sh_) + lx;
    };
    const bool one_operand = (a.add != nullptr) != (a.accumulate != 0);
    float4 pre[MB][4];
    if (one_operand) {
#pragma unroll
      for (int mb = 0; mb < MB; ++mb)
#pragma unroll
        for (int k = 0; k < 4; ++k)
          pre[mb][k] = a.add ? ld4_t<ABF>(addb, abase + row_off(mb, k, asd, ash_, asw, lxa))
                             : ld4_t<ABF>(outb, obase + row_off(mb, k, osd, osh, osw, lxo));
    }
#pragma unroll
    for (int mb = 0; mb < MB; ++mb) {
      if constexpr (!XPAR) {
#pragma unroll
        for (int i = 0; i < 16; ++i) tr[((i & 3) + 8 * (i >> 2) + 4 * h) * 36 + r] = acc[mb][i];
      }
      const float* trb = tr + (XPAR ? mb * 32 * 36 : 0);
      float4 val[4], addv[4], oldv[4];
#pragma unroll
      for (int k = 0; k < 4; ++k) val[k] = *reinterpret_cast<const float4*>(trb + (rsub + 8 * k) * 36 + c4);
      if (!one_operand) {
        if (a.add) {
#pragma unroll
          for (int k = 0; k < 4; ++k) addv[k] = ld4_t<ABF>(addb, abase + row_off(mb, k, asd, ash_, asw, lxa));
        }
        if (a.accumulate) {
#pragma unroll
          for (int k = 0; k < 4; ++k) oldv[k] = ld4_t<ABF>(outb, obase + row_off(mb, k, osd, osh, osw, lxo));
        }
      }
#pragma unroll
      for (int k = 0; k < 4; ++k) {
        const int oo = row_off(mb, k, osd, osh, osw, lxo);
        if (one_operand) finish(val[k], pre[mb][k], pre[mb][k], cvok, oo);
        else finish(val[k], addv[k], oldv[k], cvok, oo);
      }
    }
  } else {
#pragma unroll
  for (int mb = 0; mb < MB; ++mb) {
    if constexpr (!XPAR) {
#pragma unroll
      for (int i = 0; i < 16; ++i) tr[((i & 3) + 8 * (i >> 2) + 4 * h) * 36 + r] = acc[mb][i];
    }
    const float* trb = tr + (XPAR ? mb * 32 * 36 : 0);
    int ooff[4], aoff[4];
    bool ok[4];
    float4 val[4];
#pragma unroll
    for (int k = 0; k < 4; ++k) {
      const int row = rsub + 8 * k;
      val[k] = *reinterpret_cast<const float4*>(trb + row * 36 + c4);
      int zl, yl, xl;
      row_to_local<TZ, TY, TX, PERM>((rowblock0 + mb) * 32 + row, zl, yl, xl);
      const int gz = gz0 + zl, gy = gy0 + yl, gx = gx0 + xl;
      const int oz = gz * so + coz, oy = gy * so + coy, ox = gx * so + cox;
      ok[k] = cvok && gz < cDg && gy < cHg && gx < cWg && oz < Do && oy < Ho && ox < Wo;
      const int cz = min(oz, Do - 1), cy = min(oy, Ho - 1), cx = min(ox, Wo - 1);
      ooff[k] = cz * osd + cy * osh + cx * osw;
      aoff[k] = cz * asd + cy * ash_ + cx * asw;
    }
    float4 addv[4], oldv[4];
    if (a.add) {
#pragma unroll
      for (int k = 0; k < 4; ++k) addv[k] = ld4_t<ABF>(addb, abase + aoff[k]);
    }
    if (a.accumulate) {
#pragma unroll
      for (int k = 0; k < 4; ++k) oldv[k] = ld4_t<ABF>(outb, obase + ooff[k]);
    }
#pragma unroll
    for (int k = 0; k < 4; ++k) finish(val[k], addv[k], oldv[k], ok[k], ooff[k]);
  }
  }
#pragma unroll
  for (int j = 0; j < 4; ++j) {
#pragma unroll
    for (int o = 8; o < 64; o <<= 1) { ssum[j] += __shfl_xor(ssum[j], o, 64); ssq[j] += __shfl_xor(ssq[j], o, 64); }
  }
}

constexpr int EPI_TILE_FLOATS = 32 * 36;

template <int NB, int MB, int TZ, int TY, int TX, int KCI, bool BF, int OCC = 2, bool ABF = false>
__global__ __launch_bounds__(256, OCC) void igemm_kernel(GArgs a) {
  constexpr bool REUSE = false;
#include "conv_igemm_body.h"
}

template <bool ABF>
__global__ __launch_bounds__(256, 3) void igemm_reuse_kernel(GArgs a) {
  constexpr int NB = 1, MB = 2, TZ = 4, TY = 8, TX = 8, KCI = 16, OCC = 3;
  constexpr bool BF = true, REUSE = true;
#include "conv_igemm_body.h"
}

struct ClsTap { int cls, d, slab; };
__host__ __device__ constexpr ClsTap cls_tap(int f) {
  int idx = 0;
  for (int cls = 0; cls < 8; ++cls) {
    const int pz = (cls >> 2) & 1, py = (cls >> 1) & 1, px = cls & 1;
    for (int a = 0; a <= pz; ++a)
      for (int b = 0; b <= py; ++b)
        for (int c = 0; c <= px; ++c) {
          const int kz = pz ? (a == 0 ? 0 : 2) : 1, dz = pz ? (a == 0 ? 1 : 0) : 0;
          const int ky = py ? (b == 0 ? 0 : 2) : 1, dy = py ? (b == 0 ? 1 : 0) : 0;
          const int kx = px ? (c == 0 ? 0 : 2) : 1, dx = px ? (c == 0 ? 1 : 0) : 0;
          if (idx == f) return ClsTap{cls, (dz * 2 + dy) * 2 + dx, (kz * 3 + ky) * 3 + kx};
          ++idx;
        }
  }
  return ClsTap{0, 0, 0};
}

template <int KCI, bool ABF>
__global__ __launch_bounds__(256, 2) void igemm_cls8_kernel(GArgs a) {
  constexpr int TZ = 4, TY = 4, TX = 8, VS = KCI + 8, LP = LDS_PITCH_BF16, KS = KCI / 16, KC8 = KCI / 8;
  constexpr int BZ = TZ + 1, BY = TY + 1, BX = TX + 1;
  constexpr int BOX_HW = BZ * BY * LP * VS;
  constexpr int WIMG = 27 * KC8 * 32;
  extern __shared__ float lds[];
  unsigned short* lh = reinterpret_cast<unsigned short*>(lds);
  uint4* wimg = reinterpret_cast<uint4*>(lh + (BOX_HW + 7) / 8 * 8);
  const int tid = threadIdx.x, lane = tid & 63;
  const int wave = __builtin_amdgcn_readfirstlane(tid >> 6);
  const int h = lane >> 5, r = lane & 31;
  int t = blockIdx.x;
  const int tile_in_n = t % (a.tz * a.ty * a.tx);
  const int txi = t % a.tx; t /= a.tx;
  const int tyi = t % a.ty; t /= a.ty;
  const int tzi = t % a.tz;
  const int n = t / a.tz;
  const float* biasn = pset_bias(a.ps, a.bias, n);
  const int gz0 = tzi * TZ, gy0 = tyi * TY, gx0 = txi * TX;
  const int colbase = blockIdx.y * 32;
  const bool colact = colbase < a.Np;

  int zl, yl, xl;
  row_to_local<TZ, TY, TX, true>(wave * 32 + r, zl, yl, xl);
  const unsigned short* arow = lh + ((zl * BY + yl) * LP + xl) * VS + 8 * h;
  const uint4* brow = wimg + h * 32 + r;

  f32x16 acc[8];
#pragma unroll
  for (int c = 0; c < 8; ++c)
#pragma unroll
    for (int i = 0; i < 16; ++i) acc[c][i] = 0.f;

  const uint4* wq = reinterpret_cast<const uint4*>(pset_packed(a.ps, a.wp, n));
  const long long slabsz8 = (long long)(a.Kp / 8) * a.Np;
  const unsigned isd = (unsigned)a.isd, ish = (unsigned)a.ish, isw = (unsigned)a.isw;
  const int cmax = ABF ? ((a.Ci - 1) & ~7) : ((a.Ci - 1) & ~3);
  constexpr int AIT = (BZ * BY * BX * KC8 + 255) / 256;
  constexpr int BIT = (WIMG + 255) / 256;
  const float relu_lo = act_lo(a.tin.relu);

  for (int ks = 0; ks < a.nstages; ++ks) {
    const int c0 = ks * KCI;
    const float* sb = reinterpret_cast<const float*>(reinterpret_cast<const char*>(a.in) + ((long long)n * a.isn + c0) * (ABF ? 2 : 4));
    uint4 wv[BIT];
#pragma unroll
    for (int j = 0; j < BIT; ++j) {
      const int i = min(tid + 256 * j, WIMG - 1);
      const int tap = i / (KC8 * 32), rem = i - tap * (KC8 * 32), k8l = rem >> 5, col = rem & 31;
      wv[j] = wq[tap * slabsz8 + (long long)(c0 / 8 + k8l) * a.Np + colbase + col];
    }
    Oct8<ABF> av[AIT];
    unsigned aok = 0u;
    int alds[AIT];
#pragma unroll
    for (int j = 0; j < AIT; ++j) {
      const int i = min(tid + 256 * j, BZ * BY * BX * KC8 - 1);
      const int cv = i % KC8, bv = i / KC8;
      const int bz = bv / (BY * BX), brem = bv - bz * (BY * BX), by = brem / BX, bx = brem - by * BX;
      const int iz = gz0 + bz, iy = gy0 + by, ix = gx0 + bx;
      const bool ok = iz < a.Di && iy < a.Hi && ix < a.Wi;
      aok |= (ok ? 1u : 0u) << j;
      const unsigned off = __umul24((unsigned)min(iz, a.Di - 1), isd) + __umul24((unsigned)min(iy, a.Hi - 1), ish) +
                           __umul24((unsigned)min(ix, a.Wi - 1), isw) + cv * 8;
      const int over = max(c0 + cv * 8 - cmax, 0), over_hi = max(c0 + cv * 8 + 4 - cmax, 0);
      av[j] = oct8_ld<ABF>(sb, off - over, off + 4 - over_hi);
      alds[j] = ((bz * BY + by) * LP + bx) * VS + cv * 8;
    }
    float sc[AIT][8], sh[AIT][8];
#pragma unroll
    for (int j = 0; j < AIT; ++j) {
      const int i = min(tid + 256 * j, BZ * BY * BX * KC8 - 1);
      nl_coeff_vec<8>(a.tin, n, a.Ci, c0 + (i % KC8) * 8, sc[j], sh[j]);
    }
#pragma unroll
    for (int j = 0; j < BIT; ++j)
      if (tid + 256 * j < WIMG) wimg[tid + 256 * j] = wv[j];
#pragma unroll
    for (int j = 0; j < AIT; ++j) {
      float v[8];
      oct8_f8(av[j], v);
#pragma unroll
      for (int q = 0; q < 8; ++q) v[q] = act_max(fmaf(v[q], sc[j][q], sh[j][q]), relu_lo);
      const unsigned okm = ((aok >> j) & 1u) ? 0xffffffffu : 0u;
      uint4 pk;
      pk.x = pack_bf16x2(v[0], v[1]) & okm; pk.y = pack_bf16x2(v[2], v[3]) & okm;
      pk.z = pack_bf16x2(v[4], v[5]) & okm; pk.w = pack_bf16x2(v[6], v[7]) & okm;
      if (tid + 256 * j < BZ * BY * BX * KC8) *reinterpret_cast<uint4*>(lh + alds[j]) = pk;
    }
    __syncthreads();
    if (colact) {
#pragma unroll
      for (int k16 = 0; k16 < KS; ++k16) {
        uint4 af[8];
#pragma unroll
        for (int d = 0; d < 8; ++d)
          af[d] = *reinterpret_cast<const uint4*>(arow + ((((d >> 2) & 1) * BY + ((d >> 1) & 1)) * LP + (d & 1)) * VS + k16 * 16);
        constexpr int LA = 3;
        uint4 bring[LA + 1];
        static_for<0, LA>([&](auto fc) {
          constexpr int f = decltype(fc)::value;
          bring[f] = brow[(cls_tap(f).slab * KC8 + k16 * 2) * 32];
        });
        __builtin_amdgcn_sched_barrier(0);
        static_for<0, 27>([&](auto fc) {
          constexpr int f = decltype(fc)::value;
          constexpr ClsTap ct = cls_tap(f);
          if constexpr (f + LA < 27) bring[(f + LA) % (LA + 1)] = brow[(cls_tap(f + LA).slab * KC8 + k16 * 2) * 32];
          acc[ct.cls] = __builtin_amdgcn_mfma_f32_32x32x16_bf16(__builtin_bit_cast(bf16x8, af[ct.d]),
                                                                __builtin_bit_cast(bf16x8, bring[f % (LA + 1)]), acc[ct.cls], 0, 0, 0);
          __builtin_amdgcn_sched_barrier(0);
        });
      }
    }
    __syncthreads();
  }
  float tsum[4] = {0.f, 0.f, 0.f, 0.f}, tsq[4] = {0.f, 0.f, 0.f, 0.f};
#pragma unroll
  for (int c = 0; c < 8; ++c) {
    float v_sum[4], v_sq[4];
    epilogue_vec16<TZ, TY, TX, 1, true, ABF>(a, biasn, a.cls[c], *reinterpret_cast<f32x16(*)[1]>(&acc[c]), lds + wave * EPI_TILE_FLOATS,
                                             lane, wave, colbase, colact, n, gz0, gy0, gx0, v_sum, v_sq);
#pragma unroll
    for (int j = 0; j < 4; ++j) { tsum[j] += v_sum[j]; tsq[j] += v_sq[j]; }
  }
  if (a.stats != nullptr) {
    float* red = lds + 4 * EPI_TILE_FLOATS;
    if (lane < 8) {
#pragma unroll
      for (int j = 0; j < 4; ++j) {
        red[(wave * 2 + 0) * 32 + lane * 4 + j] = tsum[j];
        red[(wave * 2 + 1) * 32 + lane * 4 + j] = tsq[j];
      }
    }
    __syncthreads();
    const int col = colbase + tid;
    if (tid < 32 && col < a.Co) {
      float ts = 0.f, tq = 0.f;
#pragma unroll
      for (int g = 0; g < 4; ++g) { ts += red[(g * 2 + 0) * 32 + tid]; tq += red[(g * 2 + 1) * 32 + tid]; }
      const long long row = (long long)n * a.stats_rows_per_n + tile_in_n;
      a.stats[(row * 2 + 0) * a.Co + col] = ts;
      a.stats[(row * 2 + 1) * a.Co + col] = tq;
    }
  }
}

template <int KCI, bool ABF>
static int launch_cls8_t(const GArgs& a, int tiles, hipStream_t s) {
  constexpr int VS = KCI + 8;
  size_t lds = ((size_t)(5 * 5 * LDS_PITCH_BF16 * VS + 7) / 8 * 8) * 2 + (size_t)27 * (KCI / 8) * 32 * 16;
  const size_t epi = (4 * EPI_TILE_FLOATS + 4 * 2 * 32) * sizeof(float);
  if (lds < epi) lds = epi;
  auto kern = igemm_cls8_kernel<KCI, ABF>;
  static bool attr_set = false;
  if (!attr_set) {
    (void)hipFuncSetAttribute((const void*)kern, hipFuncAttributeMaxDynamicSharedMemorySize, 160 * 1024);
    attr_set = true;
  }
  hipLaunchKernelGGL(kern, dim3(tiles, a.Np / 32), dim3(256), lds, s, a);
  return launch_status("conv igemm (class-fused stride-2 form)");
}

template <int TZ, int TY, int TX, bool PERM, bool ABF = false>
__global__ __launch_bounds__(256) void splitk_finalize_kernel(GArgs a, int tiles) {
  __shared__ float red[2][8][32];
  constexpr int MT = TZ * TY * TX;
  constexpr int RB = MT / 32;
  const int tid = threadIdx.x, r = tid & 31, rg = tid >> 5;
  const int tile = blockIdx.x / RB, rb = blockIdx.x % RB;
  int cidx, t;
  class_of_tile(a, tile, cidx, t);
  const ClassInfo ci = a.cls[cidx];
  const int tile_in_n = t % (a.tz * a.ty * a.tx);
  const int txi = t % a.tx; t /= a.tx;
  const int tyi = t % a.ty; t /= a.ty;
  const int tzi = t % a.tz;
  const int n = t / a.tz;
  const int col = blockIdx.y * 32 + r;
  const bool colok = col < a.Co;
  float bias = 0.f, asc = 1.f, ash = 0.f;
  if (colok) {
    const float* biasn = pset_bias(a.ps, a.bias, n);
    if (biasn) bias = biasn[col];
    if (a.add) nl_coeff(a.tadd, n, a.Co, col, asc, ash);
  }
  float s_sum = 0.f, s_sq = 0.f;
  const int colc = min(col, a.Co - 1);
  const long long kstride = (long long)tiles * MT * a.Np;
  const float* wsp[4];
  long long ooff[4], aoff[4];
  bool ok[4];
  float s4[4] = {0.f, 0.f, 0.f, 0.f};
#pragma unroll
  for (int q = 0; q < 4; ++q) {
    const int v = rb * 32 + rg * 4 + q;
    int zl, yl, xl;
    row_to_local<TZ, TY, TX, PERM>(v, zl, yl, xl);
    const int gz = tzi * TZ + zl, gy = tyi * TY + yl, gx = txi * TX + xl;
    const int oz = gz * a.so + ci.oz, oy = gy * a.so + ci.oy, ox = gx * a.so + ci.ox;
    ok[q] = colok && gz < ci.Dg && gy < ci.Hg && gx < ci.Wg && oz < a.Do && oy < a.Ho && ox < a.Wo;
    const int cz = min(oz, a.Do - 1), cy = min(oy, a.Ho - 1), cx = min(ox, a.Wo - 1);
    ooff[q] = (long long)n * a.osn + cz * a.osd + cy * a.osh + cx * a.osw + colc;
    aoff[q] = (long long)n * a.asn + cz * a.asd + cy * a.ash + cx * a.asw + colc;
    wsp[q] = a.ws + ((long long)tile * MT + v) * a.Np + min(col, a.Np - 1);
  }
  for (int kz = 0; kz < a.ksplit; kz += 4) {
    float v[4][4];
#pragma unroll
    for (int u = 0; u < 4; ++u)
#pragma unroll
      for (int q = 0; q < 4; ++q) v[q][u] = wsp[q][(long long)min(kz + u, a.ksplit - 1) * kstride];
#pragma unroll
    for (int u = 0; u < 4; ++u)
#pragma unroll
      for (int q = 0; q < 4; ++q) s4[q] += kz + u < a.ksplit ? v[q][u] : 0.f;
  }
  float addv[4] = {0.f, 0.f, 0.f, 0.f}, oldv[4] = {0.f, 0.f, 0.f, 0.f};
  if (a.add) {
#pragma unroll
    for (int q = 0; q < 4; ++q) addv[q] = ld1_t<ABF>(a.add, aoff[q]);
  }
  if (a.accumulate) {
#pragma unroll
    for (int q = 0; q < 4; ++q) oldv[q] = ld1_t<ABF>(a.out, ooff[q]);
  }
#pragma unroll
  for (int q = 0; q < 4; ++q) {
    float val = s4[q] + bias;
    if (a.add) val += nl_apply(addv[q], asc, ash, a.tadd.relu);
    if (a.accumulate) val += oldv[q];
    if (ok[q]) {
      st1_t<ABF>(a.out, ooff[q], val);
      s_sum += val;
      s_sq += val * val;
    }
  }
  if (a.stats != nullptr) {
    red[0][rg][r] = s_sum;
    red[1][rg][r] = s_sq;
    __syncthreads();
    if (rg == 0 && colok) {
      float ts = 0.f, tq = 0.f;
#pragma unroll
      for (int g = 0; g < 8; ++g) { ts += red[0][g][r]; tq += red[1][g][r]; }
      const long long row = (long long)n * a.stats_rows_per_n + (cidx * (a.tz * a.ty * a.tx) + tile_in_n) * RB + rb;
      a.stats[(row * 2 + 0) * a.Co + col] = ts;
      a.stats[(row * 2 + 1) * a.Co + col] = tq;
    }
  }
}

__device__ __forceinline__ void upconv8_put_pair(unsigned short* img, int K, int k, int co, const float* src) {
  for (int dp = 0; dp < 64; ++dp) {
    const int d = dp >> 3, p = dp & 7;
    int tap = 0;
    bool owned = true;
#pragma unroll
    for (int ax = 2; ax >= 0; --ax) {
      const int pa = (p >> ax) & 1, da = (d >> ax) & 1;
      owned = owned && !(pa == 0 && da == 1);
      tap = tap * 3 + (pa == 0 ? 1 : (da == 1 ? 0 : 2));
    }
    const float v = (owned && src != nullptr) ? src[tap] : 0.f;
    img[(((d * (K >> 4) + (k >> 4)) * 64 + ((k >> 3) & 1) * 32 + p * 4 + co) << 3) + (k & 7)] =
        (unsigned short)(f32x2_to_bf16x2(v, 0.f) & 0xffffu);
  }
}

__global__ void pack_upconv8_kernel(const float* __restrict__ w, unsigned short* __restrict__ img, int K, int N) {
  const int i = blockIdx.x * blockDim.x + threadIdx.x;
  if (i >= K * 4) return;
  const int k = i >> 2, co = i & 3;
  upconv8_put_pair(img, K, k, co, co < N ? w + ((long long)k * N + co) * 27 : nullptr);
}

__global__ void pack_weights_kernel(const float* __restrict__ w, float* __restrict__ p, int A, int B, int T,
                                    int Kp, int Np, int kn_is_ba) {
  const long long total = (long long)T * Kp * Np;
  for (long long i = blockIdx.x * (long long)blockDim.x + threadIdx.x; i < total;
       i += (long long)gridDim.x * blockDim.x) {
    const int nn = (int)(i % Np);
    const int k = (int)((i / Np) % Kp);
    const int tp = (int)(i / ((long long)Np * Kp));
    const int K = kn_is_ba ? B : A, N = kn_is_ba ? A : B;
    float v = 0.f;
    if (k < K && nn < N) {
      const int ai = kn_is_ba ? nn : k, bi = kn_is_ba ? k : nn;
      v = w[((long long)ai * B + bi) * T + tp];
    }
    p[i] = v;
  }
}

__global__ void pack_weights_bf16_kernel(const float* __restrict__ w, unsigned short* __restrict__ p, int A, int B, int T,
                                         int Kp, int Np, int kn_is_ba) {
  const long long total = (long long)T * Kp * Np;
  for (long long i = blockIdx.x * (long long)blockDim.x + threadIdx.x; i < total;
       i += (long long)gridDim.x * blockDim.x) {
    const int j = (int)(i & 7);
    const int nn = (int)((i >> 3) % Np);
    const int k8 = (int)((i / (8LL * Np)) % (Kp / 8));
    const int tp = (int)(i / ((long long)Kp * Np));
    const int k = k8 * 8 + j;
    const int K = kn_is_ba ? B : A, N = kn_is_ba ? A : B;
    float v = 0.f;
    if (k < K && nn < N) {
      const int ai = kn_is_ba ? nn : k, bi = kn_is_ba ? k : nn;
      v = w[((long long)ai * B + bi) * T + tp];
    }
    p[i] = __builtin_bit_cast(unsigned short, (__bf16)v);
  }
}

struct PackEntry {
  const float* w; void* p;
  unsigned short* up8;
  uint4* chfr; int KI, NO;
  int A, B, T, Kp, Np, kn_is_ba, bf16, direct;
  long long start;
};

constexpr int PK = 8, PN = 32;

template <int T>
__device__ __forceinline__ void pack_tile(const PackEntry& e, int lb, float* tile) {
  const int tiles_n = e.Np / PN;
  const int k0 = (lb / tiles_n) * PK, n0 = (lb % tiles_n) * PN;
  const int K = e.kn_is_ba ? e.B : e.A, N = e.kn_is_ba ? e.A : e.B;
  constexpr int RS = PK * T + 1;
  constexpr int IT = PN * PK * T / 256, U = IT % 9 == 0 ? 9 : 1;
  static_assert(PN * PK * T % 256 == 0, "pack tile: whole trips");
  constexpr int RUN4 = (T == 27) ? PK * T / 4 : 1;
  const bool full = T == 27 && k0 + PK <= K && n0 + PN <= N && e.B % 4 == 0 && ((uintptr_t)e.w) % 16 == 0;
  if (T == 27 && full) {
    constexpr int N4 = PN * PK * T / 4, IT4 = (N4 + 255) / 256;
    float4 v[IT4];
    if (e.kn_is_ba) {
#pragma unroll
      for (int u = 0; u < IT4; ++u) {
        const int i4 = min(u * 256 + (int)threadIdx.x, N4 - 1);
        const int nn = i4 / RUN4, r4 = i4 % RUN4;
        v[u] = *reinterpret_cast<const float4*>(e.w + ((long long)(n0 + nn) * e.B + k0) * T + r4 * 4);
      }
#pragma unroll
      for (int u = 0; u < IT4; ++u) {
        const int i4 = u * 256 + (int)threadIdx.x;
        if (i4 < N4) {
          const int nn = i4 / RUN4, r4 = i4 % RUN4;
          float* d = tile + nn * RS + r4 * 4;
          d[0] = v[u].x; d[1] = v[u].y; d[2] = v[u].z; d[3] = v[u].w;
        }
      }
    } else {
      constexpr int KRUN4 = PN * T / 4;
#pragma unroll
      for (int u = 0; u < IT4; ++u) {
        const int i4 = min(u * 256 + (int)threadIdx.x, N4 - 1);
        const int kk = i4 / KRUN4, r4 = i4 % KRUN4;
        v[u] = *reinterpret_cast<const float4*>(e.w + ((long long)(k0 + kk) * e.B + n0) * T + r4 * 4);
      }
#pragma unroll
      for (int u = 0; u < IT4; ++u) {
        const int i4 = u * 256 + (int)threadIdx.x;
        if (i4 < N4) *reinterpret_cast<float4*>(tile + i4 * 4) = v[u];
      }
    }
  } else
  if (e.kn_is_ba) {
    for (int it = 0; it < IT; it += U) {
      float v[U]; int dst[U]; bool ok[U];
#pragma unroll
      for (int u = 0; u < U; ++u) {
        const int idx = (it + u) * 256 + threadIdx.x;
        const int nn = idx / (PK * T), r = idx % (PK * T);
        const int kk = r / T;
        ok[u] = n0 + nn < N && k0 + kk < K;
        v[u] = e.w[((long long)min(n0 + nn, N - 1) * e.B + min(k0 + kk, K - 1)) * T + (r - kk * T)];
        dst[u] = nn * RS + r;
      }
#pragma unroll
      for (int u = 0; u < U; ++u) tile[dst[u]] = ok[u] ? v[u] : 0.f;
    }
  } else {
    for (int it = 0; it < IT; it += U) {
      float v[U]; bool ok[U];
#pragma unroll
      for (int u = 0; u < U; ++u) {
        const int idx = (it + u) * 256 + threadIdx.x;
        const int kk = idx / (PN * T), r = idx % (PN * T);
        const int nn = r / T;
        ok[u] = k0 + kk < K && n0 + nn < N;
        v[u] = e.w[((long long)min(k0 + kk, K - 1) * e.B + min(n0 + nn, N - 1)) * T + (r - nn * T)];
      }
#pragma unroll
      for (int u = 0; u < U; ++u) tile[(it + u) * 256 + threadIdx.x] = ok[u] ? v[u] : 0.f;
    }
  }
  __syncthreads();
  const long long slab = (long long)e.Kp * e.Np;
  if (e.bf16) {
    for (int o = threadIdx.x; o < T * PN; o += 256) {
      const int nn = o % PN, tp = o / PN;
      unsigned short h[8];
#pragma unroll
      for (int kk = 0; kk < PK; ++kk) {
        const float v = e.kn_is_ba ? tile[nn * RS + kk * T + tp] : tile[kk * (PN * T) + nn * T + tp];
        h[kk] = f32_to_bf16_bits(v);
      }
      *reinterpret_cast<uint4*>((unsigned short*)e.p + tp * slab + ((long long)(k0 >> 3) * e.Np + n0 + nn) * 8) = bf16x8_pack(h);
    }
  } else {
    for (int o = threadIdx.x; o < T * PK * PN; o += 256) {
      const int nn = o % PN, kk = (o / PN) % PK, tp = o / (PN * PK);
      const float v = e.kn_is_ba ? tile[nn * RS + kk * T + tp] : tile[kk * (PN * T) + nn * T + tp];
      ((float*)e.p)[tp * slab + (long long)(k0 + kk) * e.Np + n0 + nn] = v;
    }
  }
}

__device__ __forceinline__ void chan_frags_write(const float* img, uint4* fr, int Kp, int Np, int KI, int N) {
  const int NB = N / 32;
  for (int i = threadIdx.x; i < 7 * NB * 64; i += blockDim.x) {
    const int lane = i & 63, frn = i >> 6, s2 = frn / NB, nb = frn % NB;
    const int h = lane >> 5, col = nb * 32 + (lane & 31);
    float wv[8];
#pragma unroll
    for (int e = 0; e < 8; ++e) {
      const int tap = s2 * 4 + h * 2 + (e >> 2), c = e & 3;
      wv[e] = (tap < 27 && c < KI && col < N) ? img[((long long)tap * Kp + c) * Np + col] : 0.f;
    }
    uint4 pk;
    pk.x = f32x2_to_bf16x2(wv[0], wv[1]); pk.y = f32x2_to_bf16x2(wv[2], wv[3]);
    pk.z = f32x2_to_bf16x2(wv[4], wv[5]); pk.w = f32x2_to_bf16x2(wv[6], wv[7]);
    fr[i] = pk;
  }
}
__global__ __launch_bounds__(256) void pack_chan_frags_kernel(const float* img, uint4* fr, int Kp, int Np, int KI, int N) {
  chan_frags_write(img, fr, Kp, Np, KI, N);
}
__global__ __launch_bounds__(256) void pack_chan_frags_batched_kernel(const PackEntry* __restrict__ tab) {
  const PackEntry e = tab[blockIdx.x];
  if (e.chfr != nullptr) chan_frags_write((const float*)e.p, e.chfr, e.Kp, e.Np, e.KI, e.NO);
}

__global__ __launch_bounds__(256) void pack_batched_kernel(const PackEntry* __restrict__ tab, int count) {
  __shared__ __attribute__((aligned(16))) float tile[PN * (PK * 27 + 1)];
  int lo = 0, hi = count - 1;
  while (lo < hi) {
    const int mid = (lo + hi + 1) >> 1;
    if (tab[mid].start <= (long long)blockIdx.x) lo = mid; else hi = mid - 1;
  }
  const PackEntry e = tab[lo];
  const int lb = (int)(blockIdx.x - e.start);
  if (e.direct) {
    const int li = lb * 256 + threadIdx.x;
    if (li >= e.Kp * e.Np) return;
    const int nn = li % e.Np, k = li / e.Np;
    const int N = e.kn_is_ba ? e.A : e.B;
    const int ai = e.kn_is_ba ? nn : k, bi = e.kn_is_ba ? k : nn;
    const float* src = e.w + ((long long)ai * e.B + bi) * e.T;
    for (int tp = 0; tp < e.T; ++tp)
      ((float*)e.p)[(long long)tp * e.Kp * e.Np + li] = nn < N ? src[tp] : 0.f;
    if (e.up8 != nullptr) upconv8_put_pair(e.up8, e.Kp, k, nn, nn < N ? src : nullptr);
    return;
  }
  if (e.T == 27) pack_tile<27>(e, lb, tile);
  else pack_tile<1>(e, lb, tile);
}


struct PWArgs {
  const float* in; long long isn; unsigned isw; int Ci;
  float* out; long long osn; unsigned osw; int Co;
  const float* add; long long asn; unsigned asw; NL tadd;
  const float* wp; const float* bias; int Np; PSets ps;
  int accumulate; long long dhw;
};

template <int KB, int NB, bool BF>
__global__ __launch_bounds__(256) void pointwise_mfma_kernel(PWArgs a) {
  constexpr int TP = NB * 32 + 4;
  __shared__ __attribute__((aligned(16))) float tile[4][32][TP];
  __shared__ float coef[3][NB * 32];
  const int n = blockIdx.y;
  const int tid = threadIdx.x, lane = tid & 63;
  const int wave = __builtin_amdgcn_readfirstlane(tid >> 6);
  const int h = lane >> 5, r = lane & 31;
  const float* wpn = pset_packed(a.ps, a.wp, n);
  const float* biasn = pset_bias(a.ps, a.bias, n);
  uint4 bfr[KB][NB];
  {
    const uint4* wq = reinterpret_cast<const uint4*>(wpn);
#pragma unroll
    for (int ks = 0; ks < KB; ++ks)
#pragma unroll
      for (int nb = 0; nb < NB; ++nb) bfr[ks][nb] = wq[(long long)(ks * 2 + h) * a.Np + nb * 32 + r];
  }
  if (tid < NB * 32) {
    const int col = min(tid, a.Co - 1);
    float sc = 1.f, sh = 0.f;
    if (a.add) nl_coeff(a.tadd, n, a.Co, col, sc, sh);
    coef[0][tid] = (biasn && tid < a.Co) ? biasn[col] : 0.f;
    coef[1][tid] = sc; coef[2][tid] = sh;
  }
  __syncthreads();
  const float* inn = item_base<BF>(a.in, n, a.isn);
  float* outn = const_cast<float*>(item_base<BF>(a.out, n, a.osn));
  const float* addn = a.add == nullptr ? nullptr : item_base<BF>(a.add, n, a.asn);
  const float relu_lo = act_lo(a.tadd.relu);
  for (long long base = (long long)blockIdx.x * 128; base < a.dhw; base += (long long)gridDim.x * 128) {
    const long long v0 = base + wave * 32;
    const unsigned vo = (unsigned)min(v0 + r, a.dhw - 1) * a.isw;
    uint4 af[KB];
#pragma unroll
    for (int ks = 0; ks < KB; ++ks) {
      const unsigned c0 = ks * 16 + h * 8;
      if (c0 + 8 <= a.isw) {
        if constexpr (BF) {
          af[ks] = *reinterpret_cast<const uint4*>(reinterpret_cast<const unsigned short*>(inn) + vo + c0);
        } else {
          const float4 lo = *reinterpret_cast<const float4*>(inn + vo + c0), hi = *reinterpret_cast<const float4*>(inn + vo + c0 + 4);
          af[ks] = make_uint4(f32x2_to_bf16x2(lo.x, lo.y), f32x2_to_bf16x2(lo.z, lo.w), f32x2_to_bf16x2(hi.x, hi.y), f32x2_to_bf16x2(hi.z, hi.w));
        }
      } else if (!BF && c0 + 4 <= a.isw) {
        const float4 lo = *reinterpret_cast<const float4*>(inn + vo + c0);
        af[ks] = make_uint4(f32x2_to_bf16x2(lo.x, lo.y), f32x2_to_bf16x2(lo.z, lo.w), 0u, 0u);
      } else {
        af[ks] = make_uint4(0u, 0u, 0u, 0u);
      }
      if ((int)c0 + 8 > a.Ci) {
        auto pm = [&](int c) { return (c < a.Ci ? 0xffffu : 0u) | (c + 1 < a.Ci ? 0xffff0000u : 0u); };
        af[ks].x &= pm(c0); af[ks].y &= pm(c0 + 2); af[ks].z &= pm(c0 + 4); af[ks].w &= pm(c0 + 6);
      }
    }
    f32x16 acc[NB];
#pragma unroll
    for (int nb = 0; nb < NB; ++nb)
#pragma unroll
      for (int i = 0; i < 16; ++i) acc[nb][i] = 0.f;
#pragma unroll
    for (int ks = 0; ks < KB; ++ks)
#pragma unroll
      for (int nb = 0; nb < NB; ++nb)
        acc[nb] = __builtin_amdgcn_mfma_f32_32x32x16_bf16(__builtin_bit_cast(bf16x8, af[ks]), __builtin_bit_cast(bf16x8, bfr[ks][nb]), acc[nb], 0, 0, 0);
#pragma unroll
    for (int i = 0; i < 16; ++i)
#pragma unroll
      for (int nb = 0; nb < NB; ++nb) tile[wave][(i & 3) + 8 * (i >> 2) + 4 * h][nb * 32 + r] = acc[nb][i];
    __builtin_amdgcn_fence(__ATOMIC_RELEASE, "wavefront");
    __builtin_amdgcn_wave_barrier();
    __builtin_amdgcn_fence(__ATOMIC_ACQUIRE, "wavefront");
#pragma unroll
    for (int q = 0; q < 2 * NB; ++q) {
      const int item = lane + 64 * q, vl = item / (4 * NB), c8 = item % (4 * NB), c0 = c8 * 8;
      const long long vv = v0 + vl;
      if (vv < a.dhw && c0 < a.Co) {
        const float4 t0 = *reinterpret_cast<const float4*>(&tile[wave][vl][c0]), t1 = *reinterpret_cast<const float4*>(&tile[wave][vl][c0 + 4]);
        float v[8] = {t0.x, t0.y, t0.z, t0.w, t1.x, t1.y, t1.z, t1.w};
        const bool full = c0 + 8 <= a.Co;
        const unsigned oo = (unsigned)vv * a.osw + c0;
#pragma unroll
        for (int e = 0; e < 8; ++e) v[e] += coef[0][c0 + e];
        if (a.add) {
          float ad[8];
          if (full || c0 + 8 <= (int)a.asw) {
            oct8_f8(oct8_ld<BF>(addn, (unsigned)vv * a.asw + c0, (unsigned)vv * a.asw + c0 + 4), ad);
          } else {
#pragma unroll
            for (int e = 0; e < 8; ++e) ad[e] = c0 + e < a.Co ? ld1_t<BF>(addn, (unsigned)vv * a.asw + c0 + e) : 0.f;
          }
#pragma unroll
          for (int e = 0; e < 8; ++e) v[e] += act_max(fmaf(ad[e], coef[1][c0 + e], coef[2][c0 + e]), relu_lo);
        }
        if (full) {
          if (a.accumulate) {
            float old[8];
            oct8_f8(oct8_ld<BF>(outn, oo, oo + 4), old);
#pragma unroll
            for (int e = 0; e < 8; ++e) v[e] += old[e];
          }
          oct8_st<BF>(outn, oo, v);
        } else {
#pragma unroll
          for (int e = 0; e < 8; ++e)
            if (c0 + e < a.Co) st1_t<BF>(outn, oo + e, a.accumulate ? v[e] + ld1_t<BF>(outn, oo + e) : v[e]);
        }
      }
    }
    __builtin_amdgcn_fence(__ATOMIC_RELEASE, "wavefront");
    __builtin_amdgcn_wave_barrier();
  }
}

template <int KB, bool BF>
static void launch_pointwise_mfma_nb(const PWArgs& a, int nb, dim3 grid, hipStream_t s) {
  if (nb == 1) hipLaunchKernelGGL((pointwise_mfma_kernel<KB, 1, BF>), grid, dim3(256), 0, s, a);
  else hipLaunchKernelGGL((pointwise_mfma_kernel<KB, 2, BF>), grid, dim3(256), 0, s, a);
}
template <bool BF>
static void launch_pointwise_mfma(const PWArgs& a, int kb, int nb, dim3 grid, hipStream_t s) {
  switch (kb) {
    case 1: launch_pointwise_mfma_nb<1, BF>(a, nb, grid, s); break;
    case 2: launch_pointwise_mfma_nb<2, BF>(a, nb, grid, s); break;
    case 3: launch_pointwise_mfma_nb<3, BF>(a, nb, grid, s); break;
    case 4: launch_pointwise_mfma_nb<4, BF>(a, nb, grid, s); break;
    case 6: launch_pointwise_mfma_nb<6, BF>(a, nb, grid, s); break;
    default: launch_pointwise_mfma_nb<8, BF>(a, nb, grid, s); break;
  }
}

struct Config { int NB, MB, TZ, TY, TX, KCI; bool bf; };

static inline int roundup(int v, int m) { return (v + m - 1) / m * m; }

static void op_dims(const mmtta_conv_desc* d, int& K, int& N, int& si, bool& classes) {
  switch (d->op) {
    case MMTTA_CONV_FWD: K = d->cin; N = d->cout; si = d->stride; classes = false; break;
    case MMTTA_CONV_DGRAD: K = d->cout; N = d->cin; si = 1; classes = d->stride == 2; break;
    case MMTTA_CONVT_FWD: K = d->cin; N = d->cout; si = 1; classes = true; break;
    default: K = d->cout; N = d->cin; si = 2; classes = false; break;
  }
}

static Config pick_config(int Np, int si, long long voxels, int K, bool bf) {
  if (si == 1) {
    if (Np == 32 && bf && g_igemm_lean) return {1, 2, 4, 8, 8, 16, bf};
    if (Np == 32) return {1, 4, 8, 8, 8, bf ? 16 : 8, bf};
    if (Np == 64) return {2, 4, 4, 8, 8, bf ? 32 : 16, bf};
    const long long tiles = (voxels + 127) / 128, colgroups = (Np + 127) / 128;
    if (tiles * colgroups * ((K + 31) / 32) < 384) return {4, 4, 4, 4, 8, bf ? 16 : 8, bf};
    return {4, 4, 4, 4, 8, 32, bf};
  }
  if (Np == 32) return {1, 1, 4, 4, 8, bf ? 16 : 8, bf};
  if (Np == 64) return {2, 2, 4, 4, 8, bf ? 16 : 8, bf};
  return {4, 4, 4, 4, 8, bf ? 16 : 8, bf};
}

static bool use_bf16(const mmtta_conv_desc* d, int K) {
  return d->dtype == MMTTA_BF16 && K >= 16 && !direct_applicable(d);
}

static int validate_desc(const mmtta_conv_desc* d) {
  MMTTA_CHECK(d != nullptr, MMTTA_ERR_INVALID, "conv: null desc");
  MMTTA_CHECK(d->op >= 0 && d->op <= 3, MMTTA_ERR_INVALID, "conv: bad op %d", d->op);
  MMTTA_CHECK(d->ksize == 1 || d->ksize == 3, MMTTA_ERR_UNSUPPORTED, "conv: ksize %d (1 or 3)", d->ksize);
  MMTTA_CHECK(d->stride == 1 || d->stride == 2, MMTTA_ERR_UNSUPPORTED, "conv: stride %d (1 or 2)", d->stride);
  MMTTA_CHECK(!(d->ksize == 1 && d->stride != 1), MMTTA_ERR_UNSUPPORTED, "conv: 1x1x1 with stride 2");
  MMTTA_CHECK(d->cin > 0 && d->cout > 0, MMTTA_ERR_INVALID, "conv: channels must be positive");
  MMTTA_CHECK(d->dtype == MMTTA_F32 || d->dtype == MMTTA_BF16, MMTTA_ERR_UNSUPPORTED, "conv: dtype %d", d->dtype);
  if (d->op == MMTTA_CONVT_FWD || d->op == MMTTA_CONVT_DGRAD)
    MMTTA_CHECK(d->ksize == 3 && d->stride == 2, MMTTA_ERR_UNSUPPORTED,
                "conv_transpose: only k3 s2 p1 op1 (the monai UNet up layer)");
  return MMTTA_OK;
}

static int config_id(const Config& c) {
  int id;
  if (c.bf && c.NB == 1 && c.MB == 2) return 14;
  if (c.NB == 1) id = c.MB == 4 ? 0 : 3;
  else if (c.NB == 2) id = c.MB == 4 ? 1 : 4;
  else id = c.KCI == 32 ? 2 : 5;
  return c.bf ? id + 7 : id;
}

enum CRoute : int {
  C_DIRECT = 6,
  C_THIN = 13,
  C_CLS_FUSED = 15,
  C_PW_SMALL = 16,
  C_PW_MFMA = 17,
  C_IGEMM_REUSE = 18,
};

struct RunFacts {
  const float* stats; const mmtta_tensor* add; const mmtta_norm_on_load* x_norm;
  int accumulate;
  const float* bias;
};

struct Geometry {
  int route;
  int K, N, Kp, Np, si;
  bool classes;
  Config cfg;
  int tz, ty, tx, tiles_per_n, tiles, ncls;
  int nstages, ksplit, sps;
  int stats_rows;
  int64_t workspace_bytes;
};

static int expected_out_dim(const mmtta_conv_desc* d, int in) {
  switch (d->op) {
    case MMTTA_CONV_FWD: return d->stride == 1 ? in : (in + 1) / 2;
    case MMTTA_CONVT_FWD: return in * 2;
    case MMTTA_CONVT_DGRAD: return in / 2;
    default: return -1;
  }
}

static bool pointwise_mfma_applicable(const mmtta_conv_desc* d, const mmtta_tensor* x, const mmtta_tensor* y, const Geometry& g,
                                      const RunFacts& rt) {
  static const bool pw_on = !(getenv("MMTTA_POINTWISE_MFMA") && atoi(getenv("MMTTA_POINTWISE_MFMA")) == 0);
  const int kb = (g.K + 15) / 16;
  auto rows_ok = [&](const mmtta_tensor* t) { return dense_rows16(t) && is_bf16(t) == is_bf16(x); };
  return pw_on && d->ksize == 1 && (d->op == MMTTA_CONV_FWD || d->op == MMTTA_CONV_DGRAD) && use_bf16(d, g.K) &&
         (kb <= 4 || kb == 6 || kb == 8) && g.Np <= 64 && rt.stats == nullptr && !(rt.x_norm && (rt.x_norm->mean || rt.x_norm->scale)) &&
         (long long)y->d * y->h * y->w >= 4096 && rows_ok(x) && rows_ok(y) && (rt.add == nullptr || (rows_ok(rt.add) && same_shape(rt.add, y)));
}

static bool rowload_operand(const mmtta_tensor* x) {
  const int64_t lim24 = (int64_t)1 << 24;
  return quad_aligned(x, 16, is_bf16(x) ? 8 : 4) && strides_fit_24(x) && x->d < lim24 && x->h < lim24 && x->w < lim24 &&
         item_fits_31(x, x->c + 16);
}

static bool igemm_reuse_applicable(const mmtta_conv_desc* d, const mmtta_tensor* x, const mmtta_tensor* y, const Geometry& g,
                                   const RunFacts& rt) {
  const mmtta_tensor* ad = rt.add;
  return g_igemm_reuse && g_igemm_pipeline && g_epilogue_vec && g.route == 14 && !g.classes && d->ksize == 3 && g.si == 1 &&
         g.K == 32 && g.N == 32 && g.ksplit == 1 && rowload_operand(x) && quad_aligned(y, quad_bytes(y)) && (!ad || quad_aligned(ad, quad_bytes(ad))) &&
         is_bf16(x) == is_bf16(y) && (!ad || is_bf16(ad) == is_bf16(y)) && ((uintptr_t)rt.bias) % 16 == 0;
}

static bool cls_fused_operand(const mmtta_tensor* t) {
  return quad_aligned(t, 16, is_bf16(t) ? 8 : 4) && strides_fit_24(t) && item_fits_31(t, t->c + 16);
}

static int stats_rows_per_tile(const Geometry& g) {
  if (g.route == C_CLS_FUSED) return 1;
  return g.ksplit > 1 ? g.cfg.TZ * g.cfg.TY * g.cfg.TX / 32 : 1;
}

static int geometry(const mmtta_conv_desc* d, const mmtta_tensor* x, const mmtta_tensor* y, const RunFacts* rt, Geometry& g) {
  int st = validate_desc(d);
  if (st) return st;
  MMTTA_CHECK(x && y && x->ptr && y->ptr, MMTTA_ERR_INVALID, "conv: null tensor");
  MMTTA_CHECK(is_cl(x) && is_cl(y), MMTTA_ERR_UNSUPPORTED, "conv: tensors must be channels-last (sc == 1)");
  op_dims(d, g.K, g.N, g.si, g.classes);
  MMTTA_CHECK(x->c == g.K && y->c == g.N, MMTTA_ERR_INVALID, "conv: channel mismatch (x.c=%d want %d, y.c=%d want %d)",
              x->c, g.K, y->c, g.N);
  MMTTA_CHECK(x->n == y->n, MMTTA_ERR_INVALID, "conv: batch mismatch");
  const int xd[3] = {x->d, x->h, x->w}, yd[3] = {y->d, y->h, y->w};
  for (int i = 0; i < 3; ++i) {
    int e = expected_out_dim(d, xd[i]);
    if (e >= 0) {
      MMTTA_CHECK(yd[i] == e, MMTTA_ERR_INVALID, "conv: spatial mismatch axis %d: in %d -> out %d, expected %d", i, xd[i],
                  yd[i], e);
      if (d->op == MMTTA_CONVT_DGRAD)
        MMTTA_CHECK(xd[i] % 2 == 0, MMTTA_ERR_INVALID, "conv_transpose dgrad: dy extent must be even");
    } else {
      int want = d->stride == 1 ? yd[i] : (yd[i] + 1) / 2;
      MMTTA_CHECK(xd[i] == want, MMTTA_ERR_INVALID, "conv dgrad: dy extent %d does not match dx extent %d", xd[i], yd[i]);
    }
  }
  g.Kp = roundup(g.K, 32);
  g.Np = roundup(g.N, 32);
  int Dg = y->d, Hg = y->h, Wg = y->w;
  if (g.classes) { Dg = (y->d + 1) / 2; Hg = (y->h + 1) / 2; Wg = (y->w + 1) / 2; }
  g.cfg = pick_config(g.Np, g.si, (long long)Dg * Hg * Wg * (g.classes ? 8 : 1), g.K, use_bf16(d, g.K));
  g.tz = (Dg + g.cfg.TZ - 1) / g.cfg.TZ;
  g.ty = (Hg + g.cfg.TY - 1) / g.cfg.TY;
  g.tx = (Wg + g.cfg.TX - 1) / g.cfg.TX;
  g.tiles_per_n = g.tz * g.ty * g.tx;
  g.ncls = g.classes ? 8 : 1;
  g.tiles = g.tiles_per_n * x->n * g.ncls;
  g.nstages = (g.K + g.cfg.KCI - 1) / g.cfg.KCI;
  const int ncolgroups = (g.Np + 32 * g.cfg.NB - 1) / (32 * g.cfg.NB);
  const int wgs = g.tiles_per_n * g.ncls * ncolgroups;
  g.ksplit = 1;
  g.sps = g.nstages;
  if (wgs < g_tune[0] && g.nstages > 1) {
    int want = (g_tune[1] + wgs - 1) / wgs;
    if (want > g.nstages) want = g.nstages;
    g.sps = (g.nstages + want - 1) / want;
    g.ksplit = (g.nstages + g.sps - 1) / g.sps;
  }
  g.route = config_id(g.cfg);
  if (g.classes && g.cfg.bf && g_cls_fused_min > 0) {
    const int ftz = (Dg + 3) / 4, fty = (Hg + 3) / 4, ftx = (Wg + 7) / 8;
    const long long fw = (long long)ftz * fty * ftx * (g.Np / 32);
    if (fw >= g_cls_fused_min && cls_fused_operand(x) && cls_fused_operand(y) && y->c % 4 == 0 && is_bf16(x) == is_bf16(y) &&
        g_epilogue_vec) {
      g.route = C_CLS_FUSED;
      g.tz = ftz; g.ty = fty; g.tx = ftx;
      g.tiles_per_n = ftz * fty * ftx;
      g.ncls = 1;
      g.tiles = g.tiles_per_n * x->n;
      g.nstages = (g.K + 15) / 16;
      g.ksplit = 1; g.sps = g.nstages;
    }
  }
  const bool f32_operands = !use_bf16(d, g.K);
  if (direct_applicable(d)) {
    g.route = C_DIRECT; g.ksplit = 1;
    g.tiles = direct_blocks_per_n(d, x, y) * y->n;
  } else if (rt && f32_operands && is_f32(x) && pointwise_small_applicable(d, x, y, rt->stats, rt->add, rt->x_norm)) {
    g.route = C_PW_SMALL;
  } else if (f32_operands && chan_applicable(d, x, y)) {
    g.route = C_THIN; g.ksplit = 1;
    g.tiles = chan_tiles_per_n(y) * y->n;
  } else if (rt && pointwise_mfma_applicable(d, x, y, g, *rt)) {
    g.route = C_PW_MFMA;
  } else if (rt && igemm_reuse_applicable(d, x, y, g, *rt)) {
    g.route = C_IGEMM_REUSE;
  }
  g.stats_rows = g.tiles * stats_rows_per_tile(g);
  g.workspace_bytes = g.ksplit > 1 ? (int64_t)g.ksplit * g.tiles * g.cfg.TZ * g.cfg.TY * g.cfg.TX * g.Np * (int64_t)sizeof(float) : 0;
  return MMTTA_OK;
}

static void build_taps(const mmtta_conv_desc* d, int pz, int py, int px, Taps& t) {
  int n = 0;
  const bool classes = (d->op == MMTTA_CONVT_FWD) || (d->op == MMTTA_CONV_DGRAD && d->stride == 2);
  if (d->ksize == 1) {
    t.dz[0] = t.dy[0] = t.dx[0] = 0; t.slab[0] = 0; n = 1;
  } else if (!classes) {
    const int sgn = (d->op == MMTTA_CONV_DGRAD) ? -1 : 1;
    for (int m = 0; m < 27; ++m) {
      const int q = sgn < 0 ? 26 - m : m, kz = q / 9, ky = q / 3 % 3, kx = q % 3;
      t.dz[n] = (signed char)(sgn * (kz - 1)); t.dy[n] = (signed char)(sgn * (ky - 1));
      t.dx[n] = (signed char)(sgn * (kx - 1)); t.slab[n] = q; ++n;
    }
  } else {
    int kzs[2], dzs[2], nz, kys[2], dys[2], ny, kxs[2], dxs[2], nx;
    auto axis = [](int p, int* ks, int* ds) { if (p == 0) { ks[0] = 1; ds[0] = 0; return 1; }
                                              ks[0] = 0; ds[0] = 1; ks[1] = 2; ds[1] = 0; return 2; };
    nz = axis(pz, kzs, dzs); ny = axis(py, kys, dys); nx = axis(px, kxs, dxs);
    for (int a = 0; a < nz; ++a) for (int b = 0; b < ny; ++b) for (int c = 0; c < nx; ++c) {
      t.dz[n] = (signed char)dzs[a]; t.dy[n] = (signed char)dys[b]; t.dx[n] = (signed char)dxs[c];
      t.slab[n] = (kzs[a] * 3 + kys[b]) * 3 + kxs[c]; ++n;
    }
  }
  t.n = n;
  int zmn = 9, zmx = -9, ymn = 9, ymx = -9, xmn = 9, xmx = -9;
  for (int i = 0; i < n; ++i) {
    zmn = t.dz[i] < zmn ? t.dz[i] : zmn; zmx = t.dz[i] > zmx ? t.dz[i] : zmx;
    ymn = t.dy[i] < ymn ? t.dy[i] : ymn; ymx = t.dy[i] > ymx ? t.dy[i] : ymx;
    xmn = t.dx[i] < xmn ? t.dx[i] : xmn; xmx = t.dx[i] > xmx ? t.dx[i] : xmx;
  }
  t.zmin = zmn; t.ymin = ymn; t.xmin = xmn;
  t.zext = zmx - zmn; t.yext = ymx - ymn; t.xext = xmx - xmn;
}

template <int NB, int MB, int TZ, int TY, int TX, int KCI, bool BF, int OCC, bool ABF, bool REUSE = false>
static int launch_cfg_t(const GArgs& a_in, const Taps* ht, int tiles, hipStream_t s) {
  GArgs a = a_in;
  size_t lds = 0;
  for (int c = 0; c < a.ncls; ++c) {
    const Taps& tp = ht[c];
    const int BZ = (TZ - 1) * a.si + tp.zext + 1, BY = (TY - 1) * a.si + tp.yext + 1, BX = (TX - 1) * a.si + tp.xext + 1;
    const int LP = (BF && a.si == 1) ? LDS_PITCH_BF16 : BX;
    for (int t = 0; t < tp.n; ++t) {
      a.toff[a.cls[c].tap0 + t] = ((tp.dz[t] - tp.zmin) * BY + (tp.dy[t] - tp.ymin)) * LP + (tp.dx[t] - tp.xmin);
      a.slab[a.cls[c].tap0 + t] = tp.slab[t];
    }
    a.cls[c].BX = BX; a.cls[c].BXY = BX * BY;
    a.cls[c].mBX = (unsigned)(((1ULL << 32) + BX - 1) / BX);
    a.cls[c].mBXY = (unsigned)(((1ULL << 32) + (unsigned long long)BX * BY - 1) / ((unsigned long long)BX * BY));
    const size_t need = BF ? (size_t)BZ * BY * LP * (KCI + 8) * 2 : (size_t)BZ * BY * BX * (KCI + 1) * sizeof(float);
    if (need > lds) lds = need;
  }
  if (BF && a.rowload && a.si == 1 && a.ncls == 1 && a.cls[0].ntaps == 27) {
    a.flip27 = a.slab[0] == 26 ? 1 : 0;
    for (int t = 0; t < 27; ++t)
      if (a.toff[t] != tap27_off(t, TY + 2) || a.slab[t] != (a.flip27 ? 26 - t : t)) a.rowload = 0;
  }
  constexpr size_t epi = (4 * (REUSE ? 2 : 1) * EPI_TILE_FLOATS + 4 * 2 * 32) * sizeof(float);
  if (lds < epi) lds = epi;
  if constexpr (REUSE) {
    if (!(a.rowload && a.ovec && a.ksplit == 1 && a.Ci == KCI * a.nstages))
      return launch_cfg_t<NB, MB, TZ, TY, TX, KCI, BF, OCC, ABF, false>(a_in, ht, tiles, s);
  }
  lds = (lds + 15) / 16 * 16;
  a.coef_off = (int)(lds / sizeof(float));
  if (BF) lds += (size_t)2 * a.stages_per_split * KCI * sizeof(float);
  MMTTA_CHECK(lds <= 160 * 1024, MMTTA_ERR_UNSUPPORTED, "conv: LDS box of %zu bytes exceeds 160 KiB", lds);
  int st;
  void (*kern)(GArgs) = igemm_kernel<NB, MB, TZ, TY, TX, KCI, BF, OCC, ABF>;
  if constexpr (REUSE) kern = igemm_reuse_kernel<ABF>;
  static bool attr_set = false;
  if (!attr_set) {
    (void)hipFuncSetAttribute((const void*)kern, hipFuncAttributeMaxDynamicSharedMemorySize, 160 * 1024);
    attr_set = true;
  }
  dim3 grid(tiles, (a.Np + 32 * NB - 1) / (32 * NB), a.ksplit);
  hipLaunchKernelGGL(kern, grid, dim3(256), lds, s, a);
  st = launch_status("conv igemm");
  if (st) return st;
  if (a.ksplit > 1 && !g_profile_main_only) {
    dim3 g2(tiles * (TZ * TY * TX / 32), (a.Np + 31) / 32);
    hipLaunchKernelGGL((splitk_finalize_kernel<TZ, TY, TX, BF, ABF>), g2, dim3(256), 0, s, a, tiles);
    st = launch_status("conv split-K finalize");
  }
  return st;
}

template <int NB, int MB, int TZ, int TY, int TX, int KCI, bool BF, int OCC = 2, bool REUSE = false>
static int launch_cfg(const GArgs& a, const Taps* ht, int tiles, hipStream_t s) {
  if constexpr (BF) {
    if (a.in_bf || a.out_bf || a.add_bf) {
      MMTTA_CHECK(a.in_bf && a.out_bf && (a.add == nullptr || a.add_bf), MMTTA_ERR_UNSUPPORTED,
                  "conv: input, output and fused add must share one storage type (in %d out %d add %d)", a.in_bf, a.out_bf,
                  a.add_bf);
      return launch_cfg_t<NB, MB, TZ, TY, TX, KCI, BF, OCC, true, REUSE>(a, ht, tiles, s);
    }
  }
  return launch_cfg_t<NB, MB, TZ, TY, TX, KCI, BF, OCC, false, REUSE>(a, ht, tiles, s);
}

static int launch_any(int route, const GArgs& a, const Taps* ht, int tiles, hipStream_t s) {
  switch (route) {
    case 0: return launch_cfg<1, 4, 8, 8, 8, 8, false>(a, ht, tiles, s);
    case 1: return launch_cfg<2, 4, 4, 8, 8, 16, false>(a, ht, tiles, s);
    case 2: return launch_cfg<4, 4, 4, 4, 8, 32, false>(a, ht, tiles, s);
    case 3: return launch_cfg<1, 1, 4, 4, 8, 8, false>(a, ht, tiles, s);
    case 4: return launch_cfg<2, 2, 4, 4, 8, 8, false>(a, ht, tiles, s);
    case 5: return launch_cfg<4, 4, 4, 4, 8, 8, false>(a, ht, tiles, s);
    case 14: return launch_cfg<1, 2, 4, 8, 8, 16, true, 3>(a, ht, tiles, s);
    case C_IGEMM_REUSE: return launch_cfg<1, 2, 4, 8, 8, 16, true, 3, true>(a, ht, tiles, s);
    case 7: return launch_cfg<1, 4, 8, 8, 8, 16, true>(a, ht, tiles, s);
    case 8: return launch_cfg<2, 4, 4, 8, 8, 32, true>(a, ht, tiles, s);
    case 9: return launch_cfg<4, 4, 4, 4, 8, 32, true>(a, ht, tiles, s);
    case 10: return launch_cfg<1, 1, 4, 4, 8, 16, true>(a, ht, tiles, s);
    case 11: return launch_cfg<2, 2, 4, 4, 8, 16, true>(a, ht, tiles, s);
    default: return launch_cfg<4, 4, 4, 4, 8, 16, true>(a, ht, tiles, s);
  }
}

struct ConvCall {
  const mmtta_conv_desc* d; const mmtta_tensor* x; const mmtta_norm_on_load* x_norm; const void* packed; const float* bias;
  const mmtta_conv_epilogue* epi; const mmtta_tensor* y; int accumulate; float* stats; void* workspace; int64_t workspace_bytes;
  PSets ps; hipStream_t stream;
};

static int fill_gargs(const ConvCall& c, const Geometry& g, GArgs& a, Taps* ht) {
  const mmtta_tensor *x = c.x, *y = c.y, *ad = (c.epi && c.epi->add) ? c.epi->add : nullptr;
  a.in = (const float*)x->ptr; a.isn = x->sn; a.isd = x->sd; a.ish = x->sh; a.isw = x->sw;
  a.Ci = x->c; a.Di = x->d; a.Hi = x->h; a.Wi = x->w; a.tin = nl(c.x_norm);
  a.out = (float*)y->ptr; a.osn = y->sn; a.osd = y->sd; a.osh = y->sh; a.osw = y->sw;
  a.Co = y->c; a.Do = y->d; a.Ho = y->h; a.Wo = y->w;
  a.si = g.si; a.bias = c.bias; a.ps = c.ps; a.accumulate = c.accumulate;
  a.wp = (const float*)c.packed; a.Kp = g.Kp; a.Np = g.Np;
  const int st = epilogue_add(c.epi, y, a);
  if (st) return st;
  a.in_bf = is_bf16(x) ? 1 : 0; a.out_bf = is_bf16(y) ? 1 : 0; a.add_bf = (ad && is_bf16(ad)) ? 1 : 0;
  const bool oal = quad_aligned(y, quad_bytes(y)) && y->c % 4 == 0 &&
                   (!ad || quad_aligned(ad, quad_bytes(ad))) && (c.bias == nullptr || ((uintptr_t)c.bias) % 16 == 0);
  a.ovec = (oal && g_epilogue_vec) ? 1 : 0;
  a.stats = c.stats; a.stats_rows_per_n = g.ncls * g.tiles_per_n * stats_rows_per_tile(g);
  a.ws = (float*)c.workspace; a.ksplit = g.ksplit; a.stages_per_split = g.sps; a.nstages = g.nstages;
  a.tz = g.tz; a.ty = g.ty; a.tx = g.tx;
  MMTTA_CHECK(g.cfg.bf || (!a.in_bf && !a.out_bf && !a.add_bf), MMTTA_ERR_UNSUPPORTED,
              "conv: bf16-stored tensors need a bf16-operand layer (K >= 16 in bf16 precision)");
  const bool al = quad_aligned(x, 16, a.in_bf ? 8 : 4);
  a.vec4 = al ? 1 : 0; a.flip27 = 0;
  a.rowload = (rowload_operand(x) && g_igemm_pipeline) ? 1 : 0;
  a.ncls = g.classes ? 8 : 1; a.so = g.classes ? 2 : 1;
  int tap0 = 0;
  for (int cls = 0; cls < a.ncls; ++cls) {
    const int pz = (cls >> 2) & 1, py = (cls >> 1) & 1, px = cls & 1;
    build_taps(c.d, pz, py, px, ht[cls]);
    ClassInfo& ci = a.cls[cls];
    ci.tap0 = tap0; ci.ntaps = ht[cls].n; tap0 += ht[cls].n;
    ci.zmin = ht[cls].zmin; ci.ymin = ht[cls].ymin; ci.xmin = ht[cls].xmin;
    ci.zext = ht[cls].zext; ci.yext = ht[cls].yext; ci.xext = ht[cls].xext;
    if (g.classes) {
      ci.oz = pz; ci.oy = py; ci.ox = px;
      ci.Dg = (y->d - pz + 1) / 2; ci.Hg = (y->h - py + 1) / 2; ci.Wg = (y->w - px + 1) / 2;
    } else {
      ci.oz = ci.oy = ci.ox = 0;
      ci.Dg = y->d; ci.Hg = y->h; ci.Wg = y->w;
    }
  }
  return MMTTA_OK;
}

static int igemm_run(const ConvCall& c, const Geometry& g) {
  MMTTA_CHECK(g.workspace_bytes == 0 || (c.workspace != nullptr && c.workspace_bytes >= g.workspace_bytes), MMTTA_ERR_WORKSPACE,
              "conv: workspace %lld bytes, need %lld", (long long)c.workspace_bytes, (long long)g.workspace_bytes);
  GArgs a; Taps ht[8];
  const int st = fill_gargs(c, g, a, ht);
  if (st) return st;
  return launch_any(g.route, a, ht, g.tiles, c.stream);
}

static int cls_fused_run(const ConvCall& c, const Geometry& g) {
  GArgs a; Taps ht[8];
  const int st = fill_gargs(c, g, a, ht);
  if (st) return st;
  MMTTA_CHECK(a.ovec && a.vec4, MMTTA_ERR_UNSUPPORTED,
              "conv (class-fused stride-2 form): the epilogue operands must admit 16-byte accesses");
  MMTTA_CHECK(a.in_bf == a.out_bf && (a.add == nullptr || a.add_bf == a.out_bf), MMTTA_ERR_UNSUPPORTED,
              "conv: input, output and fused add must share one storage type (in %d out %d add %d)", a.in_bf, a.out_bf, a.add_bf);
  return a.in_bf ? launch_cls8_t<16, true>(a, g.tiles, c.stream) : launch_cls8_t<16, false>(a, g.tiles, c.stream);
}

static int pointwise_mfma_run(const ConvCall& c, const Geometry& g) {
  const mmtta_tensor *x = c.x, *y = c.y, *ad = (c.epi && c.epi->add) ? c.epi->add : nullptr;
  PWArgs q;
  q.in = (const float*)x->ptr; q.isn = x->sn; q.isw = (unsigned)x->sw; q.Ci = x->c;
  q.out = (float*)y->ptr; q.osn = y->sn; q.osw = (unsigned)y->sw; q.Co = y->c;
  q.add = ad ? (const float*)ad->ptr : nullptr; q.asn = ad ? ad->sn : 0; q.asw = ad ? (unsigned)ad->sw : 0u;
  q.tadd = ad ? nl(&c.epi->add_norm) : nl(nullptr);
  q.wp = (const float*)c.packed; q.bias = c.bias; q.Np = g.Np; q.ps = c.ps; q.accumulate = c.accumulate;
  q.dhw = (long long)y->d * y->h * y->w;
  long long blocks = (q.dhw + 127) / 128;
  if (blocks > 2048) blocks = 2048;
  const dim3 grid((unsigned)blocks, y->n);
  if (is_bf16(x)) launch_pointwise_mfma<true>(q, (g.K + 15) / 16, g.Np / 32, grid, c.stream);
  else launch_pointwise_mfma<false>(q, (g.K + 15) / 16, g.Np / 32, grid, c.stream);
  return launch_status("1x1 conv (streaming MFMA)");
}

static int plan_run(const mmtta_conv_desc* d, const mmtta_tensor* x, const mmtta_norm_on_load* x_norm, const mmtta_conv_epilogue* epi,
                    const mmtta_tensor* y, int accumulate, const float* stats, const float* bias, Geometry& g) {
  const RunFacts rt{stats, epi ? epi->add : nullptr, x_norm, accumulate, bias};
  return geometry(d, x, y, &rt, g);
}

int conv_run_body(const mmtta_conv_desc* d, const mmtta_tensor* x, const mmtta_norm_on_load* x_norm, const void* packed,
                  const float* bias, const mmtta_conv_epilogue* epi, const mmtta_tensor* y, int accumulate, float* stats,
                  void* workspace, int64_t workspace_bytes, const mmtta_param_sets* sets, void* stream) {
  Geometry g;
  int st = plan_run(d, x, x_norm, epi, y, accumulate, stats, bias, g);
  if (st) return st;
  MMTTA_CHECK(packed != nullptr, MMTTA_ERR_INVALID, "conv: null packed weights");
  st = psets_validate(sets, x->n);
  if (st) return st;
  const ConvCall c{d, x, x_norm, packed, bias, epi, y, accumulate, stats, workspace, workspace_bytes, psets(sets), (hipStream_t)stream};
  switch (g.route) {
    case C_DIRECT: return direct_conv_run(d, x, x_norm, packed, bias, epi, y, accumulate, stats, c.ps, c.stream);
    case C_PW_SMALL: return pointwise_small_run(x, packed, g.Kp, g.Np, bias, y, accumulate, c.ps, c.stream);
    case C_THIN: return chan_conv_run(d, x, x_norm, packed, g.Kp, g.Np, bias, epi, y, accumulate, stats, c.ps, c.stream);
    case C_PW_MFMA: return pointwise_mfma_run(c, g);
    case C_CLS_FUSED: return cls_fused_run(c, g);
    default: return igemm_run(c, g);
  }
}

MMTTA_ACT_NS_CLOSE
}

#ifndef MMTTA_ACT_LEAKY_TU
using namespace mmtta;

static int pack_entry_geometry(const mmtta_conv_desc* d, PackEntry& e, bool& up8, bool& chfr) {
  int st = validate_desc(d);
  if (st) return st;
  int K, N, si; bool cl;
  op_dims(d, K, N, si, cl);
  const bool convt = d->op == MMTTA_CONVT_FWD || d->op == MMTTA_CONVT_DGRAD;
  const bool direct = direct_applicable(d);
  e.w = nullptr; e.p = nullptr; e.up8 = nullptr; e.chfr = nullptr;
  e.A = convt ? d->cin : d->cout; e.B = convt ? d->cout : d->cin;
  e.T = d->ksize * d->ksize * d->ksize;
  e.Kp = direct ? K : roundup(K, 32); e.Np = direct ? 4 : roundup(N, 32);
  e.kn_is_ba = (d->op == MMTTA_CONV_FWD || d->op == MMTTA_CONVT_DGRAD) ? 1 : 0;
  e.bf16 = use_bf16(d, K) ? 1 : 0; e.direct = direct ? 1 : 0;
  up8 = direct && upconv8_image_bytes(d) > 0;
  chfr = !direct && chan_frag_bytes(d) > 0;
  e.KI = K; e.NO = N;
  MMTTA_CHECK(e.T == 1 || e.T == 27, MMTTA_ERR_UNSUPPORTED, "pack: ksize %d", d->ksize);
  e.start = 0;
  return MMTTA_OK;
}

static int fill_pack_entry(const mmtta_conv_desc* d, const float* w, void* packed, PackEntry& e) {
  bool up8, chfr;
  int st = pack_entry_geometry(d, e, up8, chfr);
  if (st) return st;
  MMTTA_CHECK(w && packed, MMTTA_ERR_INVALID, "pack: null pointer");
  e.w = w; e.p = packed;
  e.up8 = up8 ? (unsigned short*)((char*)packed + (size_t)e.T * e.Kp * e.Np * 4) : nullptr;
  e.chfr = chfr ? (uint4*)((char*)packed + (size_t)e.T * e.Kp * e.Np * 4) : nullptr;
  return MMTTA_OK;
}

extern "C" int64_t mmtta_conv_packed_bytes(const mmtta_conv_desc* d) {
  PackEntry e;
  bool up8, chfr;
  if (pack_entry_geometry(d, e, up8, chfr)) return -1;
  return (int64_t)e.T * e.Kp * e.Np * (int64_t)(e.bf16 ? 2 : sizeof(float)) + (e.direct ? upconv8_image_bytes(d) : chan_frag_bytes(d));
}

extern "C" int mmtta_conv_pack_weights(const mmtta_conv_desc* d, const float* w, void* packed, void* stream) {
  PackEntry e;
  int st = fill_pack_entry(d, w, packed, e);
  if (st) return st;
  const long long total = (long long)e.T * e.Kp * e.Np;
  int blocks = (int)((total + 255) / 256);
  if (blocks > 4096) blocks = 4096;
  if (e.bf16)
    hipLaunchKernelGGL(pack_weights_bf16_kernel, dim3(blocks), dim3(256), 0, (hipStream_t)stream, w, (unsigned short*)packed,
                       e.A, e.B, e.T, e.Kp, e.Np, e.kn_is_ba);
  else
    hipLaunchKernelGGL(pack_weights_kernel, dim3(blocks), dim3(256), 0, (hipStream_t)stream, w, (float*)packed, e.A, e.B, e.T,
                       e.Kp, e.Np, e.kn_is_ba);
  if (e.up8)
    hipLaunchKernelGGL(pack_upconv8_kernel, dim3((e.KI * 4 + 255) / 256), dim3(256), 0, (hipStream_t)stream, w, e.up8, e.KI, e.NO);
  if (e.chfr)
    hipLaunchKernelGGL(pack_chan_frags_kernel, dim3(1), dim3(256), 0, (hipStream_t)stream, (const float*)packed, e.chfr, e.Kp,
                       e.Np, e.KI, e.NO);
  return launch_status("pack weights");
}

namespace mmtta {
int pack_image_geometry(const mmtta_conv_desc* d, PackImageGeo& g) {
  PackEntry e;
  bool up8, chfr;
  const int st = pack_entry_geometry(d, e, up8, chfr);
  if (st) return st;
  g.A = e.A; g.B = e.B; g.T = e.T; g.Kp = e.Kp; g.Np = e.Np; g.kn_is_ba = e.kn_is_ba;
  g.plain_bf16 = (e.bf16 && !e.direct && !up8 && !chfr) ? 1 : 0;
  return MMTTA_OK;
}
}

extern "C" int64_t mmtta_conv_pack_table_bytes(int count) { return count < 0 ? -1 : (int64_t)count * (int64_t)sizeof(PackEntry); }

extern "C" int mmtta_conv_pack_table_build(const mmtta_pack_item* items, int count, void* table_host, int64_t* total) {
  MMTTA_CHECK(items && table_host && total && count > 0, MMTTA_ERR_INVALID, "pack table: bad argument");
  PackEntry* tab = (PackEntry*)table_host;
  long long run = 0;
  for (int i = 0; i < count; ++i) {
    int st = fill_pack_entry(&items[i].desc, items[i].w_master, items[i].packed, tab[i]);
    if (st) return st;
    tab[i].start = run;
    run += tab[i].direct ? ((long long)tab[i].Kp * tab[i].Np + 255) / 256
                         : (long long)(tab[i].Kp / PK) * (tab[i].Np / PN);
  }
  *total = run;
  return MMTTA_OK;
}

extern "C" int mmtta_conv_pack_batched(const void* table_dev, int count, int64_t total, void* stream) {
  MMTTA_CHECK(table_dev && count > 0 && total > 0, MMTTA_ERR_INVALID, "pack batched: bad argument");
  MMTTA_CHECK(total < (1LL << 31), MMTTA_ERR_UNSUPPORTED, "pack batched: %lld workgroups", (long long)total);
  hipLaunchKernelGGL(pack_batched_kernel, dim3((unsigned)total), dim3(256), 0, (hipStream_t)stream, (const PackEntry*)table_dev,
                     count);
  int st = launch_status("pack batched");
  if (st) return st;
  hipLaunchKernelGGL(pack_chan_frags_batched_kernel, dim3((unsigned)count), dim3(256), 0, (hipStream_t)stream, (const PackEntry*)table_dev);
  return launch_status("pack batched (thin-K fragments)");
}

extern "C" int mmtta_conv_plan(const mmtta_conv_desc* d, const mmtta_tensor* x, const mmtta_tensor* y,
                               mmtta_conv_plan_t* plan) {
  MMTTA_CHECK(plan != nullptr, MMTTA_ERR_INVALID, "conv plan: null plan");
  Geometry g;
  int st = geometry(d, x, y, nullptr, g);
  if (st) return st;
  *plan = mmtta_conv_plan_t{g.tiles,  1, g.ksplit, g.stats_rows, g.route, 0, g.workspace_bytes};
  return MMTTA_OK;
}

extern "C" int mmtta_conv_route(const mmtta_conv_desc* d, const mmtta_tensor* x, const mmtta_norm_on_load* x_norm,
                                const mmtta_conv_epilogue* epi, const mmtta_tensor* y, int accumulate, const float* stats) {
  Geometry g;
  const int st = plan_run(d, x, x_norm, epi, y, accumulate, stats, nullptr, g);
  if (st) return st < 0 ? st : -st;
  return g.route;
}

extern "C" int mmtta_conv_run(const mmtta_conv_desc* d, const mmtta_tensor* x, const mmtta_norm_on_load* x_norm,
                              const void* packed, const float* bias, const mmtta_conv_epilogue* epi,
                              const mmtta_tensor* y, int accumulate, float* stats, void* workspace,
                              int64_t workspace_bytes, void* stream) {
  return mmtta_conv_run_sets(d, x, x_norm, packed, bias, epi, y, accumulate, stats, workspace, workspace_bytes, nullptr, stream);
}

extern "C" int mmtta_conv_run_sets(const mmtta_conv_desc* d, const mmtta_tensor* x, const mmtta_norm_on_load* x_norm,
                                   const void* packed, const float* bias, const mmtta_conv_epilogue* epi,
                                   const mmtta_tensor* y, int accumulate, float* stats, void* workspace,
                                   int64_t workspace_bytes, const mmtta_param_sets* sets, void* stream) {
  const mmtta_norm_on_load* add_norm = (epi && epi->add) ? &epi->add_norm : nullptr;
  {
    int st = nl_act_check(x_norm, "conv_run (x_norm)");
    if (st) return st;
    st = nl_act_check(add_norm, "conv_run (epilogue add_norm)");
    if (st) return st;
    st = nl_per_item_check(x_norm, "conv_run (x_norm)");
    if (st) return st;
    st = nl_per_item_check(epi ? &epi->add_norm : nullptr, "conv_run (epilogue add_norm)");
    if (st) return st;
  }
  if (nl_leaky(x_norm) || nl_leaky(add_norm))
    return leaky::conv_run_body(d, x, x_norm, packed, bias, epi, y, accumulate, stats, workspace, workspace_bytes, sets, stream);
  return conv_run_body(d, x, x_norm, packed, bias, epi, y, accumulate, stats, workspace, workspace_bytes, sets, stream);
}
#endif
```

multimodal_tta_amd/csrc/conv_igemm_body.h:

```cpp
  extern __shared__ float lds[];
  static_assert(!REUSE || (NB == 1 && MB == 2 && TZ == 4 && TY == 8 && TX == 8 && KCI == 16 && BF && OCC > 2),
                "fragment reuse is built for the lean tile");
  constexpr int VS = BF ? (KCI + 8) : (KCI + 1);
  static_assert(!BF || KCI % 16 == 0, "bf16 stages are multiples of the MFMA K=16");
  constexpr int MT = TZ * TY * TX;
  constexpr int MG = 4 / NB;
  static_assert(MT == 32 * MB * MG, "tile rows must equal 32*MB*(4/NB)");

  const int tid = threadIdx.x, lane = tid & 63, wave = tid >> 6;
  const int cb = wave % NB, mg = wave / NB;
  const int h = lane >> 5, r = lane & 31;

  const unsigned lflat = xcd_contiguous_id(blockIdx.x + gridDim.x * (blockIdx.y + gridDim.y * blockIdx.z),
                                           gridDim.x * gridDim.y * gridDim.z);
  const int bx = (int)(lflat % gridDim.x);
  const int lby = (int)((lflat / gridDim.x) % gridDim.y), lbz = (int)(lflat / (gridDim.x * gridDim.y));
  int cidx, t;
  class_of_tile(a, bx, cidx, t);
  const ClassInfo ci = a.cls[cidx];
  const int tile_in_n = t % (a.tz * a.ty * a.tx);
  const int txi = t % a.tx; t /= a.tx;
  const int tyi = t % a.ty; t /= a.ty;
  const int tzi = t % a.tz;
  const int n = t / a.tz;
  const float* wpn = pset_packed(a.ps, a.wp, n);
  const float* biasn = pset_bias(a.ps, a.bias, n);
  const int gz0 = tzi * TZ, gy0 = tyi * TY, gx0 = txi * TX;
  const int BZ = (TZ - 1) * a.si + ci.zext + 1;
  const int BY = (TY - 1) * a.si + ci.yext + 1;
  const int BX = (TX - 1) * a.si + ci.xext + 1;
  const int boxvox = BZ * BY * BX;
  const int LP = (BF && a.si == 1) ? LDS_PITCH_BF16 : BX;
  const int iz0 = gz0 * a.si + ci.zmin, iy0 = gy0 * a.si + ci.ymin, ix0 = gx0 * a.si + ci.xmin;

  const int colbase = (lby * NB + cb) * 32;
  const bool colact = REUSE || colbase < a.Np;

  int rowaddr[MB];
#pragma unroll
  for (int mb = 0; mb < MB; ++mb) {
    int zl, yl, xl;
    row_to_local<TZ, TY, TX, BF>((mg * MB + mb) * 32 + r, zl, yl, xl);
    rowaddr[mb] = (((zl * a.si) * BY + yl * a.si) * LP + xl * a.si) * VS + (BF ? 8 * h : h);
    if constexpr (REUSE) rowaddr[mb] = ((mg * (TY + 2) + (r >> 3) + 4 * ((r >> 2) & 1)) * LDS_PITCH_BF16 + (r & 3)) * VS + 8 * h;
  }

  f32x16 acc[MB];
#pragma unroll
  for (int mb = 0; mb < MB; ++mb)
#pragma unroll
    for (int i = 0; i < 16; ++i) acc[mb][i] = 0.f;

  const int ks0 = lbz * a.stages_per_split;
  const int ks1 = min(a.nstages, ks0 + a.stages_per_split);
  const float* inb = a.in;
  const long long inoff = (long long)n * a.isn;

  constexpr int RCV8 = BF ? KCI / 8 : 1;
  constexpr int RBY = TY + 2, RBZ = TZ + 2, RBX = TX + 2;
  constexpr int RIPR = RBX * RCV8;
  constexpr int RRPP = 256 / RIPR;
  constexpr int RNROW = RBZ * RBY;
  constexpr int RGP = (RNROW + RRPP - 1) / RRPP;
  constexpr int RPG = !BF ? 0 : (OCC > 2 ? 0 : (KCI == 16 ? (ABF ? 4 : 2) : 0));
  constexpr int RGPA = BF ? RGP : 1;
  const bool fast = REUSE || (BF && a.rowload && ci.ntaps == 27 && a.si == 1);
  const bool pipe = fast && RPG > 0;
  Oct8<ABF> gv[RGPA];
  unsigned voff[RGPA];
  unsigned pok = 0u;
  constexpr bool RHOIST = KCI == 16;
  const int rrsub = min(tid / RIPR, RRPP - 1), rrem = tid % RIPR, rbx = rrem / RCV8, rcv = rrem % RCV8;
  auto geometry = [&]() {
    int rs = rrsub;
    if constexpr (!RHOIST) asm volatile("" : "+v"(rs));
    const int ix = ix0 + rbx;
    const bool xok = (unsigned)ix < (unsigned)a.Wi;
    const unsigned xoff = __umul24((unsigned)min(max(ix, 0), a.Wi - 1), (unsigned)a.isw) + rcv * 8;
    pok = 0u;
    static_for<0, RGP>([&](auto pc) {
      constexpr int P = decltype(pc)::value;
      const int row = min(RRPP * P + rs, RNROW - 1);
      const int bz = row / RBY, by = row - bz * RBY;
      const int iz = iz0 + bz, iy = iy0 + by;
      const bool ok = xok && (unsigned)iz < (unsigned)a.Di && (unsigned)iy < (unsigned)a.Hi;
      pok |= (ok ? 1u : 0u) << P;
      voff[P] = __umul24((unsigned)min(max(iz, 0), a.Di - 1), (unsigned)a.isd) + __umul24((unsigned)min(max(iy, 0), a.Hi - 1), (unsigned)a.ish) + xoff;
    });
  };
  unsigned short* lh0 = reinterpret_cast<unsigned short*>(lds);
  unsigned short* rst = lh0 + (rrsub * LDS_PITCH_BF16 + (REUSE ? reuse_xslot(rbx) : rbx)) * VS + rcv * 8;
  float* coef = lds + a.coef_off;
  const int cbase = ks0 * KCI, nch = (ks1 - ks0) * KCI;
  if (fast) {
    for (int cch = tid; cch < nch; cch += 256) {
      float sc1 = 0.f, sh1 = 0.f;
      if (cbase + cch < a.Ci) nl_coeff(a.tin, n, a.Ci, cbase + cch, sc1, sh1);
      coef[cch] = sc1;
      coef[nch + cch] = sh1;
    }
    if constexpr (RHOIST) geometry();
  }
  auto stage_base = [&](int ks) {
    return reinterpret_cast<const float*>(reinterpret_cast<const char*>(a.in) + ((long long)n * a.isn + (long long)ks * KCI) * (ABF ? 2 : 4));
  };
  const int cmax8 = ABF ? ((a.Ci - 1) & ~7) : ((a.Ci - 1) & ~3);
  auto load_item = [&](auto pc, const float* sb, int c0) {
    constexpr int P = decltype(pc)::value;
    const int over = max(c0 + rcv * 8 - cmax8, 0), over_hi = max(c0 + rcv * 8 + 4 - cmax8, 0);
    gv[P] = oct8_ld<ABF>(sb, voff[P] - over, voff[P] + 4 - over_hi);
  };
  auto issue = [&](int ks) {
    const float* sb = stage_base(ks);
    static_for<0, RPG>([&](auto pc) { load_item(pc, sb, ks * KCI); });
  };
  if (fast && ks0 < ks1) {
    if (pipe) issue(ks0);
    __syncthreads();
  }

  constexpr bool CANON_CFG = BF && OCC > 2;
  const long long wslab16 = (long long)(a.Kp / 8) * a.Np * 16;
  const char* const wuni = reinterpret_cast<const char*>(wpn) + (a.flip27 ? 26 * wslab16 : 0);
  const long long wstep16 = a.flip27 ? -wslab16 : wslab16;
  const unsigned wlane16 = (unsigned)(h * a.Np + colbase + r) * 16u;
  auto wfrag27 = [&](int c0, int t, int k2) {
    const char* ub = wuni + ((long long)(c0 / 8) * a.Np + (long long)k2 * 2 * a.Np) * 16 + t * wstep16;
    return *reinterpret_cast<const uint4*>(ub + wlane16);
  };

  for (int ks = ks0; ks < ks1; ++ks) {
    const int stage = ks;
    const int c0 = ks * KCI;
    constexpr int WG0 = BF ? (OCC > 2 ? 3 : (KCI == 16 ? 9 : 5)) : 1;
    constexpr int WKS = BF ? KCI / 16 : 1;
    uint4 wfirst[WG0][WKS];
    bool wfirst_ok = false;
    if constexpr (BF) {
      if (REUSE || (colact && ci.ntaps == 27 && ((min(KCI, a.Ci - c0) + 15) >> 4) == WKS)) {
        wfirst_ok = true;
        const long long slabsz8 = (long long)(a.Kp / 8) * a.Np;
        if (CANON_CFG && fast) {
#pragma unroll
          for (int t = 0; t < WG0; ++t)
#pragma unroll
            for (int k2 = 0; k2 < WKS; ++k2) wfirst[t][k2] = wfrag27(c0, t, k2);
        } else {
          const uint4* wq0 = reinterpret_cast<const uint4*>(wpn) + (long long)(c0 / 8 + h) * a.Np + colbase + r;
#pragma unroll
          for (int t = 0; t < WG0; ++t)
#pragma unroll
            for (int k2 = 0; k2 < WKS; ++k2) wfirst[t][k2] = wq0[(a.slab + ci.tap0)[t] * slabsz8 + k2 * 2 * a.Np];
        }
      }
    }
    if constexpr (BF) {
      unsigned short* lh = reinterpret_cast<unsigned short*>(lds);
      if (fast) {
        const float* sb = stage_base(ks);
        constexpr int RB = ABF ? 6 : 4;
        constexpr int R1 = RPG + RB < RGP ? RPG + RB : RGP;
        if constexpr (!RHOIST) geometry();
        static_for<RPG, R1>([&](auto pc) { load_item(pc, sb, c0); });
        float sc[8], sh[8];
        {
          const float4* cq = reinterpret_cast<const float4*>(coef + (c0 - cbase) + rcv * 8);
          const float4* hq = reinterpret_cast<const float4*>(coef + nch + (c0 - cbase) + rcv * 8);
          const float4 s0 = cq[0], s1 = cq[1], h0 = hq[0], h1 = hq[1];
          sc[0] = s0.x; sc[1] = s0.y; sc[2] = s0.z; sc[3] = s0.w; sc[4] = s1.x; sc[5] = s1.y; sc[6] = s1.z; sc[7] = s1.w;
          sh[0] = h0.x; sh[1] = h0.y; sh[2] = h0.z; sh[3] = h0.w; sh[4] = h1.x; sh[5] = h1.y; sh[6] = h1.z; sh[7] = h1.w;
        }
        const float relu_lo = act_lo(a.tin.relu);
        auto commit_item = [&](auto pc) {
          constexpr int P = decltype(pc)::value;
          float v[8];
          oct8_f8(gv[P], v);
#pragma unroll
          for (int j = 0; j < 8; ++j) v[j] = act_max(fmaf(v[j], sc[j], sh[j]), relu_lo);
          const unsigned okm = ((pok >> P) & 1u) ? 0xffffffffu : 0u;
          uint4 pk;
          pk.x = pack_bf16x2(v[0], v[1]) & okm; pk.y = pack_bf16x2(v[2], v[3]) & okm;
          pk.z = pack_bf16x2(v[4], v[5]) & okm; pk.w = pack_bf16x2(v[6], v[7]) & okm;
          if (RNROW % RRPP == 0 || P + 1 < RGP || RRPP * P + rrsub < RNROW)
            *reinterpret_cast<uint4*>(rst + P * (RRPP * LDS_PITCH_BF16 * VS)) = pk;
        };
        static_for<0, R1>(commit_item);
        static_for_step<R1, RGP, RB>([&](auto r0) {
          constexpr int A = decltype(r0)::value, B = A + RB < RGP ? A + RB : RGP;
          static_for<A, B>([&](auto pc) { load_item(pc, sb, c0); });
          static_for<A, B>(commit_item);
        });
      } else if (a.vec4) {
        constexpr int CV8 = KCI / 8;
        const int cv = tid % CV8;
        const int c = c0 + cv * 8;
        float sc[8], sh[8];
        constexpr int STEP = 256 / CV8;
        const int first_item = 0;
        nl_coeff_vec<8>(a.tin, n, a.Ci, c, sc, sh);
        constexpr int U = OCC > 2 ? 2 : 4;
        const bool tail = (a.Ci & 7) != 0;
        for (int bv0 = tid / CV8 + first_item * STEP; bv0 < boxvox; bv0 += U * STEP) {
          float4 x0[U], x1[U];
          bool ok[U];
#pragma unroll
          for (int u = 0; u < U; ++u) {
            const int bv = bv0 + u * STEP;
            const int bz = (int)__umulhi((unsigned)bv, ci.mBXY), brem = bv - bz * ci.BXY;
            const int by = (int)__umulhi((unsigned)brem, ci.mBX), bx = brem - by * ci.BX;
            const int iz = iz0 + bz, iy = iy0 + by, ix = ix0 + bx;
            ok[u] = bv < boxvox && (unsigned)iz < (unsigned)a.Di && (unsigned)iy < (unsigned)a.Hi &&
                    (unsigned)ix < (unsigned)a.Wi && c < a.Ci;
            x0[u] = make_float4(0.f, 0.f, 0.f, 0.f);
            x1[u] = make_float4(0.f, 0.f, 0.f, 0.f);
            if (ok[u]) {
              const long long so = inoff + (long long)iz * a.isd + (long long)iy * a.ish + (long long)ix * a.isw + c;
              if constexpr (ABF) ld8_t<true>(inb, so, x0[u], x1[u]);
              else {
                x0[u] = *reinterpret_cast<const float4*>(inb + so);
                if (c + 4 < a.Ci) x1[u] = *reinterpret_cast<const float4*>(inb + so + 4);
              }
            }
          }
#pragma unroll
          for (int u = 0; u < U; ++u) {
            const int bv = bv0 + u * STEP;
            if (bv < boxvox) {
              uint4 pk = make_uint4(0u, 0u, 0u, 0u);
              if (ok[u]) {
                const float xs[8] = {x0[u].x, x0[u].y, x0[u].z, x0[u].w, x1[u].x, x1[u].y, x1[u].z, x1[u].w};
                float v[8];
#pragma unroll
                for (int j = 0; j < 8; ++j) {
                  v[j] = nl_apply(xs[j], sc[j], sh[j], a.tin.relu);
                  if (tail && c + j >= a.Ci) v[j] = 0.f;
                }
                pk.x = pack_bf16x2(v[0], v[1]); pk.y = pack_bf16x2(v[2], v[3]);
                pk.z = pack_bf16x2(v[4], v[5]); pk.w = pack_bf16x2(v[6], v[7]);
              }
              const int bz = (int)__umulhi((unsigned)bv, ci.mBXY), brem = bv - bz * ci.BXY;
              const int by = (int)__umulhi((unsigned)brem, ci.mBX), bx = brem - by * ci.BX;
              *reinterpret_cast<uint4*>(lh + ((bz * BY + by) * LP + bx) * VS + cv * 8) = pk;
            }
          }
        }
      } else {
        const int cc = tid % KCI;
        const int c = c0 + cc;
        float sc, sh;
        nl_coeff_vec<1>(a.tin, n, a.Ci, c, &sc, &sh);
        for (int bv = tid / KCI; bv < boxvox; bv += 256 / KCI) {
          const int bz = (int)__umulhi((unsigned)bv, ci.mBXY), brem = bv - bz * ci.BXY;
          const int by = (int)__umulhi((unsigned)brem, ci.mBX), bx = brem - by * ci.BX;
          const int iz = iz0 + bz, iy = iy0 + by, ix = ix0 + bx;
          float v = 0.f;
          if ((unsigned)iz < (unsigned)a.Di && (unsigned)iy < (unsigned)a.Hi && (unsigned)ix < (unsigned)a.Wi &&
              c < a.Ci)
            v = nl_apply(ld1_t<ABF>(inb, inoff + (long long)iz * a.isd + (long long)iy * a.ish + (long long)ix * a.isw + c), sc, sh,
                         a.tin.relu);
          lh[((bz * BY + by) * LP + bx) * VS + cc] = __builtin_bit_cast(unsigned short, (__bf16)v);
        }
      }
    } else {
    if (a.vec4) {
      constexpr int CV = KCI / 4;
      const int cv = tid % CV;
      const int c = c0 + cv * 4;
      float sc[4], sh[4];
      nl_coeff_vec<4>(a.tin, n, a.Ci, c, sc, sh);
      constexpr int U = 4, STEP = 256 / CV;
      for (int bv0 = tid / CV; bv0 < boxvox; bv0 += U * STEP) {
        float4 xin[U];
        bool ok[U];
#pragma unroll
        for (int u = 0; u < U; ++u) {
          const int bv = bv0 + u * STEP;
          const int bz = (int)__umulhi((unsigned)bv, ci.mBXY), brem = bv - bz * ci.BXY;
          const int by = (int)__umulhi((unsigned)brem, ci.mBX), bx = brem - by * ci.BX;
          const int iz = iz0 + bz, iy = iy0 + by, ix = ix0 + bx;
          ok[u] = bv < boxvox && (unsigned)iz < (unsigned)a.Di && (unsigned)iy < (unsigned)a.Hi &&
                  (unsigned)ix < (unsigned)a.Wi && c < a.Ci;
          xin[u] = make_float4(0.f, 0.f, 0.f, 0.f);
          if (ok[u]) xin[u] = *reinterpret_cast<const float4*>(inb + inoff + iz * a.isd + iy * a.ish + ix * a.isw + c);
        }
#pragma unroll
        for (int u = 0; u < U; ++u) {
          const int bv = bv0 + u * STEP;
          if (bv < boxvox) {
            float4 v = make_float4(0.f, 0.f, 0.f, 0.f);
            if (ok[u]) {
              v.x = nl_apply(xin[u].x, sc[0], sh[0], a.tin.relu);
              v.y = (c + 1 < a.Ci) ? nl_apply(xin[u].y, sc[1], sh[1], a.tin.relu) : 0.f;
              v.z = (c + 2 < a.Ci) ? nl_apply(xin[u].z, sc[2], sh[2], a.tin.relu) : 0.f;
              v.w = (c + 3 < a.Ci) ? nl_apply(xin[u].w, sc[3], sh[3], a.tin.relu) : 0.f;
            }
            float* d = lds + bv * VS + cv * 4;
            d[0] = v.x; d[1] = v.y; d[2] = v.z; d[3] = v.w;
          }
        }
      }
    } else {
      const int cc = tid % KCI;
      const int c = c0 + cc;
      float sc, sh;
      nl_coeff_vec<1>(a.tin, n, a.Ci, c, &sc, &sh);
      for (int bv = tid / KCI; bv < boxvox; bv += 256 / KCI) {
        const int bx = bv % BX, by = (bv / BX) % BY, bz = bv / (BX * BY);
        const int iz = iz0 + bz, iy = iy0 + by, ix = ix0 + bx;
        float v = 0.f;
        if ((unsigned)iz < (unsigned)a.Di && (unsigned)iy < (unsigned)a.Hi && (unsigned)ix < (unsigned)a.Wi &&
            c < a.Ci)
          v = nl_apply(inb[inoff + iz * a.isd + iy * a.ish + ix * a.isw + c], sc, sh, a.tin.relu);
        lds[bv * VS + cc] = v;
      }
    }
    }
    __syncthreads();

    if constexpr (BF) {
      if (colact) {
        constexpr int KS = KCI / 16;
        const unsigned short* lh = reinterpret_cast<const unsigned short*>(lds);
        const int kreal = min(KCI, a.Ci - c0);
        const int nks = (kreal + 15) >> 4;
        const uint4* wq = reinterpret_cast<const uint4*>(wpn);
        const long long slabsz8 = (long long)(a.Kp / 8) * a.Np;
        const uint4* wcol = wq + (long long)(c0 / 8 + h) * a.Np + colbase + r;
        const int np2 = 2 * a.Np;
        const int ntap = ci.ntaps;
        const int* tslab = a.slab + ci.tap0;
        const int* ttoff = a.toff + ci.tap0;
        if constexpr (REUSE) {
          constexpr int G = 3, NG = 9;
          static_assert(G == WG0 && KS == 1 && WKS == 1, "a weight group is one box row");
          auto rfrag = [&](int j, int m) {
            return *reinterpret_cast<const uint4*>(lh + rowaddr[0] + (((j / 3) * RBY + j % 3) * LDS_PITCH_BF16 + reuse_xslot(m)) * VS);
          };
          uint4 wset[2][G];
#pragma unroll
          for (int t = 0; t < G; ++t) wset[0][t] = wfirst[t][0];
          uint4 f[4], fn[2];
          f[0] = rfrag(0, 0);
          f[1] = rfrag(0, 1);
#pragma unroll
          for (int g = 0; g < NG; ++g) {
            if (g + 1 < NG) {
#pragma unroll
              for (int t = 0; t < G; ++t) wset[(g + 1) & 1][t] = wfrag27(c0, (g + 1) * G + t, 0);
            }
            __builtin_amdgcn_sched_barrier(0);
#pragma unroll
            for (int t = 0; t < G; ++t) {
              const bf16x8 bfr = __builtin_bit_cast(bf16x8, wset[g & 1][t]);
              if (t < 2) f[t + 2] = rfrag(g, t + 2);
              else if (g + 1 < NG) fn[0] = rfrag(g + 1, 0);
              acc[0] = __builtin_amdgcn_mfma_f32_32x32x16_bf16(__builtin_bit_cast(bf16x8, f[t]), bfr, acc[0], 0, 0, 0);
              if (t == 2 && g + 1 < NG) fn[1] = rfrag(g + 1, 1);
              acc[1] = __builtin_amdgcn_mfma_f32_32x32x16_bf16(__builtin_bit_cast(bf16x8, f[t + 1]), bfr, acc[1], 0, 0, 0);
              const bool rd0 = t < 2 || g + 1 < NG, rd1 = t == 2 && g + 1 < NG;
              if (rd0) __builtin_amdgcn_sched_group_barrier(0x100, 1, 0);
              __builtin_amdgcn_sched_group_barrier(0x008, 1, 0);
              if (rd1) __builtin_amdgcn_sched_group_barrier(0x100, 1, 0);
              __builtin_amdgcn_sched_group_barrier(0x008, 1, 0);
            }
            f[0] = fn[0];
            f[1] = fn[1];
            __builtin_amdgcn_sched_barrier(0);
          }
        } else if (nks == KS && ntap == 27) {
          constexpr int G = OCC > 2 ? 3 : (KS == 1 ? 9 : 5);
          constexpr int NG = (27 + G - 1) / G;
          static_assert(G == WG0 && KS == WKS, "first-group prefetch must match the group shape");
          auto stage27 = [&](auto fc) {
          constexpr bool CANON = decltype(fc)::value;
          uint4 wset[2][G][KS];
#pragma unroll
          for (int t = 0; t < G; ++t)
#pragma unroll
            for (int ks = 0; ks < KS; ++ks) wset[0][t][ks] = wfirst[t][ks];
          uint4 avc[MB];
          {
            const int ta0 = CANON ? 0 : ttoff[0] * VS;
#pragma unroll
            for (int mb = 0; mb < MB; ++mb) avc[mb] = *reinterpret_cast<const uint4*>(lh + rowaddr[mb] + ta0);
          }
#pragma unroll
          for (int g = 0; g < NG; ++g) {
            if (g + 1 < NG) {
#pragma unroll
              for (int t = 0; t < G; ++t) {
                if ((g + 1) * G + t < 27) {
#pragma unroll
                  for (int ks = 0; ks < KS; ++ks)
                    wset[(g + 1) & 1][t][ks] = CANON ? wfrag27(c0, (g + 1) * G + t, ks) : wcol[tslab[(g + 1) * G + t] * slabsz8 + ks * np2];
                }
              }
            }
            if (g == NG - 2 && pipe && stage + 1 < ks1) issue(stage + 1);
            __builtin_amdgcn_sched_barrier(0);
#pragma unroll
            for (int t = 0; t < G; ++t) {
              if (g * G + t < 27) {
#pragma unroll
                for (int ks = 0; ks < KS; ++ks) {
                  const bf16x8 bfr = __builtin_bit_cast(bf16x8, wset[g & 1][t][ks]);
                  const int idx = g * G + t;
                  const bool more = !(idx == 26 && ks == KS - 1);
                  const int nidx = ks + 1 < KS ? idx : idx + 1, nks2 = ks + 1 < KS ? ks + 1 : 0;
                  uint4 avn[MB];
                  int tan = 0;
                  if (more) tan = (CANON ? tap27_off(nidx, RBY) : ttoff[nidx]) * VS + nks2 * 16;
#pragma unroll
                  for (int mb = 0; mb < MB; ++mb) {
                    if (more) avn[mb] = *reinterpret_cast<const uint4*>(lh + rowaddr[mb] + tan);
                    acc[mb] = __builtin_amdgcn_mfma_f32_32x32x16_bf16(__builtin_bit_cast(bf16x8, avc[mb]), bfr, acc[mb], 0, 0, 0);
                  }
#pragma unroll
                  for (int mb = 0; mb < MB; ++mb) {
                    if (more) __builtin_amdgcn_sched_group_barrier(0x100, 1, 0);
                    __builtin_amdgcn_sched_group_barrier(0x008, 1, 0);
                  }
                  if (more) {
#pragma unroll
                    for (int mb = 0; mb < MB; ++mb) avc[mb] = avn[mb];
                  }
                }
              }
            }
            __builtin_amdgcn_sched_barrier(0);
          }
          };
          if constexpr (CANON_CFG) {
            if (fast) stage27(std::true_type{});
            else stage27(std::false_type{});
          } else {
            stage27(std::false_type{});
          }
        } else if (nks == KS && ntap >= 4) {
          constexpr int D = 4;
          uint4 ring[D][KS];
#pragma unroll
          for (int d = 0; d < D; ++d) {
            const uint4* wb = wcol + tslab[d] * slabsz8;
#pragma unroll
            for (int ks = 0; ks < KS; ++ks) ring[d][ks] = wb[ks * np2];
          }
          const int ntap_pad = (ntap + D - 1) / D * D;
          for (int tp0 = 0; tp0 < ntap_pad; tp0 += D) {
#pragma unroll
            for (int d = 0; d < D; ++d) {
              const int tp = tp0 + d;
              const bool live = tp < ntap;
              bf16x8 bfrag[KS];
#pragma unroll
              for (int ks = 0; ks < KS; ++ks) {
                uint4 q = ring[d][ks];
                q.x = live ? q.x : 0u; q.y = live ? q.y : 0u; q.z = live ? q.z : 0u; q.w = live ? q.w : 0u;
                bfrag[ks] = __builtin_bit_cast(bf16x8, q);
              }
              const uint4* wb = wcol + tslab[min(tp + D, ntap - 1)] * slabsz8;
#pragma unroll
              for (int ks = 0; ks < KS; ++ks) ring[d][ks] = wb[ks * np2];
              const int ta = ttoff[min(tp, ntap - 1)] * VS;
#pragma unroll
              for (int ks = 0; ks < KS; ++ks) {
#pragma unroll
                for (int mb = 0; mb < MB; ++mb) {
                  const uint4 av = *reinterpret_cast<const uint4*>(lh + rowaddr[mb] + ta + ks * 16);
                  acc[mb] = __builtin_amdgcn_mfma_f32_32x32x16_bf16(__builtin_bit_cast(bf16x8, av), bfrag[ks], acc[mb], 0, 0, 0);
                }
              }
            }
          }
        } else {
          for (int tp = 0; tp < ntap; ++tp) {
            const uint4* wb = wcol + tslab[tp] * slabsz8;
            const int ta = ttoff[tp] * VS;
            for (int ks = 0; ks < nks; ++ks) {
              const bf16x8 bfrag = __builtin_bit_cast(bf16x8, wb[ks * np2]);
#pragma unroll
              for (int mb = 0; mb < MB; ++mb) {
                const uint4 av = *reinterpret_cast<const uint4*>(lh + rowaddr[mb] + ta + ks * 16);
                acc[mb] = __builtin_amdgcn_mfma_f32_32x32x16_bf16(__builtin_bit_cast(bf16x8, av), bfrag, acc[mb], 0, 0, 0);
              }
            }
          }
        }
      } else if (pipe && stage + 1 < ks1) {
        issue(stage + 1);
      }
    } else {
    if (colact) {
      constexpr int KK = KCI / 2;
      const int kreal = min(KCI, a.Ci - c0);
      const float* wcol = wpn + (long long)c0 * a.Np + colbase + r + (long long)h * a.Np;
      const long long slabsz = (long long)a.Kp * a.Np;
      const int np2 = 2 * a.Np;
      const int ntap = ci.ntaps;
      const int* tslab = a.slab + ci.tap0;
      const int* ttoff = a.toff + ci.tap0;
      if (kreal == KCI) {
        float bcur[KK], bnxt[KK];
        {
          const float* wb = wcol + tslab[0] * slabsz;
#pragma unroll
          for (int kk = 0; kk < KK; ++kk) bcur[kk] = wb[kk * np2];
        }
        for (int tp = 0; tp < ntap; ++tp) {
          const int tn = min(tp + 1, ntap - 1);
          const float* wb = wcol + tslab[tn] * slabsz;
#pragma unroll
          for (int kk = 0; kk < KK; ++kk) bnxt[kk] = wb[kk * np2];
          const int ta = ttoff[tp] * VS;
#pragma unroll
          for (int kk = 0; kk < KK; ++kk) {
#pragma unroll
            for (int mb = 0; mb < MB; ++mb) {
              const float av = lds[rowaddr[mb] + ta + 2 * kk];
              acc[mb] = __builtin_amdgcn_mfma_f32_32x32x2f32(av, bcur[kk], acc[mb], 0, 0, 0);
            }
          }
#pragma unroll
          for (int kk = 0; kk < KK; ++kk) bcur[kk] = bnxt[kk];
        }
      } else {
        const int kkn = (kreal + 1) >> 1;
        for (int tp = 0; tp < ntap; ++tp) {
          const float* wb = wcol + tslab[tp] * slabsz;
          const int ta = ttoff[tp] * VS;
          for (int kk = 0; kk < kkn; ++kk) {
            const float b = wb[kk * np2];
#pragma unroll
            for (int mb = 0; mb < MB; ++mb) {
              const float av = lds[rowaddr[mb] + ta + 2 * kk];
              acc[mb] = __builtin_amdgcn_mfma_f32_32x32x2f32(av, b, acc[mb], 0, 0, 0);
            }
          }
        }
      }
    }
    }
    __syncthreads();
  }

  const int col = colbase + r;
  const bool colok = colact && col < a.Co;
  float s_sum = 0.f, s_sq = 0.f;
  if (!REUSE && a.ksplit > 1) {
    if (colact) {
      float* wsb = a.ws + ((long long)lbz * gridDim.x + bx) * MT * a.Np + col;
#pragma unroll
      for (int mb = 0; mb < MB; ++mb)
#pragma unroll
        for (int i = 0; i < 16; ++i) {
          const int row = (i & 3) + 8 * (i >> 2) + 4 * h;
          const int v = (mg * MB + mb) * 32 + row;
          wsb[(long long)v * a.Np] = acc[mb][i];
        }
    }
    return;
  }
  if (REUSE || a.ovec) {
    constexpr int ETF = (REUSE ? 2 : 1) * EPI_TILE_FLOATS;
    float v_sum[4], v_sq[4];
    epilogue_vec16<TZ, TY, TX, MB, BF, ABF, REUSE>(a, biasn, ci, acc, lds + wave * ETF, lane, mg * MB, colbase, colact, n, gz0,
                                                   gy0, gx0, v_sum, v_sq);
    if (a.stats != nullptr) {
      float* red = lds + 4 * ETF;
      if (lane < 8) {
#pragma unroll
        for (int j = 0; j < 4; ++j) {
          red[(wave * 2 + 0) * 32 + lane * 4 + j] = v_sum[j];
          red[(wave * 2 + 1) * 32 + lane * 4 + j] = v_sq[j];
        }
      }
      __syncthreads();
      if (mg == 0 && h == 0 && colok) {
        float ts = 0.f, tq = 0.f;
#pragma unroll
        for (int g = 0; g < MG; ++g) {
          ts += red[((g * NB + cb) * 2 + 0) * 32 + r];
          tq += red[((g * NB + cb) * 2 + 1) * 32 + r];
        }
        const long long row = (long long)n * a.stats_rows_per_n + cidx * (a.tz * a.ty * a.tx) + tile_in_n;
        a.stats[(row * 2 + 0) * a.Co + col] = ts;
        a.stats[(row * 2 + 1) * a.Co + col] = tq;
      }
    }
    return;
  }
  float bias = 0.f, asc = 1.f, ash = 0.f;
  if (colok) {
    if (biasn) bias = biasn[col];
    if (a.add) nl_coeff(a.tadd, n, a.Co, col, asc, ash);
  }
  const int colc = min(col, a.Co - 1);
  const float* addb = a.add;
  float* outb = a.out;
  const long long abase = (long long)n * a.asn + colc, obase = (long long)n * a.osn + colc;
#pragma unroll
  for (int mb = 0; mb < MB; ++mb) {
#pragma unroll
    for (int half = 0; half < 2; ++half) {
      int ooff[8], aoff[8];
      bool ok[8];
#pragma unroll
      for (int j = 0; j < 8; ++j) {
        const int i = half * 8 + j;
        const int row = (i & 3) + 8 * (i >> 2) + 4 * h;
        int zl, yl, xl;
        row_to_local<TZ, TY, TX, BF>((mg * MB + mb) * 32 + row, zl, yl, xl);
        const int gz = gz0 + zl, gy = gy0 + yl, gx = gx0 + xl;
        const int oz = gz * a.so + ci.oz, oy = gy * a.so + ci.oy, ox = gx * a.so + ci.ox;
        ok[j] = colok && gz < ci.Dg && gy < ci.Hg && gx < ci.Wg && oz < a.Do && oy < a.Ho && ox < a.Wo;
        const int cz = min(oz, a.Do - 1), cy = min(oy, a.Ho - 1), cx = min(ox, a.Wo - 1);
        ooff[j] = cz * (int)a.osd + cy * (int)a.osh + cx * (int)a.osw;
        aoff[j] = cz * (int)a.asd + cy * (int)a.ash + cx * (int)a.asw;
      }
      float addv[8], oldv[8];
      if (a.add) {
#pragma unroll
        for (int j = 0; j < 8; ++j) addv[j] = ld1_t<ABF>(addb, abase + aoff[j]);
      }
      if (a.accumulate) {
#pragma unroll
        for (int j = 0; j < 8; ++j) oldv[j] = ld1_t<ABF>(outb, obase + ooff[j]);
      }
#pragma unroll
      for (int j = 0; j < 8; ++j) {
        float v = acc[mb][half * 8 + j] + bias;
        if (a.add) v += nl_apply(addv[j], asc, ash, a.tadd.relu);
        if (a.accumulate) v += oldv[j];
        if (ok[j]) {
          st1_t<ABF>(outb, obase + ooff[j], v);
          s_sum += v;
          s_sq += v * v;
        }
      }
    }
  }
  if (a.stats != nullptr) {
    s_sum += __shfl_xor(s_sum, 32, 64);
    s_sq += __shfl_xor(s_sq, 32, 64);
    float* red = lds;
    if (h == 0) {
      red[(wave * 2 + 0) * 32 + r] = s_sum;
      red[(wave * 2 + 1) * 32 + r] = s_sq;
    }
    __syncthreads();
    if (mg == 0 && h == 0 && colok) {
      float ts = 0.f, tq = 0.f;
#pragma unroll
      for (int g = 0; g < MG; ++g) {
        ts += red[((g * NB + cb) * 2 + 0) * 32 + r];
        tq += red[((g * NB + cb) * 2 + 1) * 32 + r];
      }
      const long long row = (long long)n * a.stats_rows_per_n + cidx * (a.tz * a.ty * a.tx) + tile_in_n;
      a.stats[(row * 2 + 0) * a.Co + col] = ts;
      a.stats[(row * 2 + 1) * a.Co + col] = tq;
    }
  }
```

Before: 110.1.

## Add x-modulo-4 fragment-reuse implicit-GEMM kernel variant for route 12

Adds a new igemm_reuse4 kernel for 3x3x3 stride-1 convolutions on route 12. It stages whole input planes in a custom LDS layout so that activation fragments loaded for one x position are reused across four output column blocks and the three x taps. Weights are prefetched a few box rows ahead, and MFMAs are interleaved with LDS reads through sched_group_barrier. The variant is enabled by default when its applicability checks pass, and it needs new row remapping in the epilogue and split-K store. It costs more LDS and uses occupancy 2.

```diff
diff --git a/include/mmtta.h b/include/mmtta.h
--- a/include/mmtta.h
+++ b/include/mmtta.h
@@ -60,6 +60,7 @@
 #define MMTTA_OPT_CLASS_FUSED_MIN_WORKGROUPS 12
 #define MMTTA_OPT_THIN_MFMA 13
 #define MMTTA_OPT_IGEMM_FRAGMENT_REUSE 14
+#define MMTTA_OPT_IGEMM_FRAGMENT_REUSE4 15
 int mmtta_set_option(int key, int value);
 
 int mmtta_copy_strided(const mmtta_tensor* src, const mmtta_tensor* dst, void* stream);
@@ -118,6 +119,10 @@
 
 int mmtta_conv_route(const mmtta_conv_desc* desc, const mmtta_tensor* x, const mmtta_norm_on_load* x_norm,
                      const mmtta_conv_epilogue* epi, const mmtta_tensor* y, int accumulate, const float* stats);
+
+int mmtta_conv_variant(const mmtta_conv_desc* desc, const mmtta_tensor* x, const mmtta_norm_on_load* x_norm,
+                       const mmtta_conv_epilogue* epi, const mmtta_tensor* y, int accumulate, const float* stats,
+                       const float* bias);
 
 typedef struct {
   int32_t items_per_set;
diff --git a/multimodal_tta_amd/_lib.py b/multimodal_tta_amd/_lib.py
--- a/multimodal_tta_amd/_lib.py
+++ b/multimodal_tta_amd/_lib.py
@@ -123,6 +123,8 @@
     "mmtta_conv_run_sets": (C.c_int, [_P(ConvDesc), _P(Tensor), _P(NormOnLoad), C.c_void_p, C.c_void_p, _P(ConvEpilogue),
                                       _P(Tensor), C.c_int, C.c_void_p, C.c_void_p, C.c_int64, _P(ParamSets), C.c_void_p]),
     "mmtta_conv_route": (C.c_int, [_P(ConvDesc), _P(Tensor), _P(NormOnLoad), _P(ConvEpilogue), _P(Tensor), C.c_int, C.c_void_p]),
+    "mmtta_conv_variant": (C.c_int, [_P(ConvDesc), _P(Tensor), _P(NormOnLoad), _P(ConvEpilogue), _P(Tensor), C.c_int, C.c_void_p,
+                                     C.c_void_p]),
     "mmtta_conv_wgrad_workspace_bytes": (C.c_int64, [_P(ConvDesc), _P(Tensor), _P(Tensor)]),
     "mmtta_conv_wgrad_workspace_bytes_sets": (C.c_int64, [_P(ConvDesc), _P(Tensor), _P(Tensor), _P(ParamSets)]),
     "mmtta_conv_wgrad_plan_sets": (C.c_int, [_P(ConvDesc), _P(Tensor), _P(Tensor), _P(ParamSets), _P(C.c_int32)]),
@@ -254,6 +256,8 @@
         lib.mmtta_set_option(13, int(os.environ["MMTTA_THINMFMA"]))
     if "MMTTA_CLSFUSE" in os.environ:
         lib.mmtta_set_option(12, int(os.environ["MMTTA_CLSFUSE"]))
+    if "MMTTA_REUSE4" in os.environ:
+        lib.mmtta_set_option(15, int(os.environ["MMTTA_REUSE4"]))
     if "MMTTA_LEAN" in os.environ:
         lib.mmtta_set_option(10, int(os.environ["MMTTA_LEAN"]))
     _lib = lib
diff --git a/multimodal_tta_amd/csrc/api.hip b/multimodal_tta_amd/csrc/api.hip
--- a/multimodal_tta_amd/csrc/api.hip
+++ b/multimodal_tta_amd/csrc/api.hip
@@ -14,6 +14,7 @@
 int g_epilogue_vec = 1;
 int g_igemm_lean = 1;
 int g_igemm_reuse = 1;
+int g_igemm_reuse4 = 1;
 int g_cls_fused_min = 128;
 int g_thin_mfma = 2;
 int g_wgrad_vec = 1;
@@ -51,6 +52,11 @@
     mmtta::g_igemm_reuse = value ? 1 : 0;
     return prev;
   }
+  if (key == MMTTA_OPT_IGEMM_FRAGMENT_REUSE4) {
+    const int prev = mmtta::g_igemm_reuse4;
+    mmtta::g_igemm_reuse4 = value ? 1 : 0;
+    return prev;
+  }
   if (key == MMTTA_OPT_EPILOGUE_VEC16) {
     const int prev = mmtta::g_epilogue_vec;
     mmtta::g_epilogue_vec = value ? 1 : 0;
diff --git a/multimodal_tta_amd/csrc/common.h b/multimodal_tta_amd/csrc/common.h
--- a/multimodal_tta_amd/csrc/common.h
+++ b/multimodal_tta_amd/csrc/common.h
@@ -34,6 +34,7 @@
 extern int g_wgrad_vec;
 extern int g_igemm_lean;
 extern int g_igemm_reuse;
+extern int g_igemm_reuse4;
 extern int g_cls_fused_min;
 extern int g_thin_mfma;
 extern int g_epilogue_vec;
diff --git a/multimodal_tta_amd/csrc/conv_igemm.hip b/multimodal_tta_amd/csrc/conv_igemm.hip
--- a/multimodal_tta_amd/csrc/conv_igemm.hip
+++ b/multimodal_tta_amd/csrc/conv_igemm.hip
@@ -90,7 +90,16 @@
   return q * 4 + (x & 3);
 }
 
-template <int TZ, int TY, int TX, int MB, bool PERM, bool ABF, bool XPAR = false>
+constexpr int REUSE4_PLANE = (4 + 2) * LDS_PITCH_BF16 * (16 + 8) + 8;
+__host__ __device__ constexpr int reuse4_row(int i, int b, int hh) {
+  const int z = i >> 2, yl = i & 3, j = ((z ^ (z >> 1)) & 1) ^ hh;
+  int q = 0;
+  for (int c = 0; c < 8; ++c)
+    if (((0xEB14 >> (2 * c)) & 3) == yl && ((c >> 1) & 1) == j) q = c;
+  return z * 32 + q * 4 + b;
+}
+
+template <int TZ, int TY, int TX, int MB, bool PERM, bool ABF, bool XPAR = false, bool XMOD4 = false>
 __device__ __forceinline__ void epilogue_vec16(const GArgs& a, const float* biasp, const ClassInfo& ci, f32x16 (&acc)[MB], float* tr,
                                                int lane, int rowblock0, int colbase, bool colact, int n, int gz0, int gy0, int gx0,
                                                float (&ssum)[4], float (&ssq)[4]) {
@@ -158,7 +167,13 @@
     }
 #pragma unroll
     for (int mb = 0; mb < MB; ++mb) {
-      if constexpr (!XPAR) {
+      if constexpr (XMOD4) {
+#pragma unroll
+        for (int b = 0; b < 4; ++b)
+#pragma unroll
+          for (int y = 0; y < 4; ++y)
+            tr[((h ? reuse4_row(4 * mb + y, b, 1) : reuse4_row(4 * mb + y, b, 0)) - 32 * mb) * 36 + r] = acc[b][4 * mb + y];
+      } else if constexpr (!XPAR) {
 #pragma unroll
         for (int i = 0; i < 16; ++i) tr[((i & 3) + 8 * (i >> 2) + 4 * h) * 36 + r] = acc[mb][i];
       }
@@ -186,7 +201,13 @@
   } else {
 #pragma unroll
   for (int mb = 0; mb < MB; ++mb) {
-    if constexpr (!XPAR) {
+    if constexpr (XMOD4) {
+#pragma unroll
+      for (int b = 0; b < 4; ++b)
+#pragma unroll
+        for (int y = 0; y < 4; ++y)
+          tr[((h ? reuse4_row(4 * mb + y, b, 1) : reuse4_row(4 * mb + y, b, 0)) - 32 * mb) * 36 + r] = acc[b][4 * mb + y];
+    } else if constexpr (!XPAR) {
 #pragma unroll
       for (int i = 0; i < 16; ++i) tr[((i & 3) + 8 * (i >> 2) + 4 * h) * 36 + r] = acc[mb][i];
     }
@@ -231,14 +252,24 @@
 
 template <int NB, int MB, int TZ, int TY, int TX, int KCI, bool BF, int OCC = 2, bool ABF = false>
 __global__ __launch_bounds__(256, OCC) void igemm_kernel(GArgs a) {
-  constexpr bool REUSE = false;
+  constexpr bool REUSE = false, REUSE4 = false;
+  constexpr int REUSE4_LA = 0;
 #include "conv_igemm_body.h"
 }
 
 template <bool ABF>
 __global__ __launch_bounds__(256, 3) void igemm_reuse_kernel(GArgs a) {
   constexpr int NB = 1, MB = 2, TZ = 4, TY = 8, TX = 8, KCI = 16, OCC = 3;
-  constexpr bool BF = true, REUSE = true;
+  constexpr bool BF = true, REUSE = true, REUSE4 = false;
+  constexpr int REUSE4_LA = 0;
+#include "conv_igemm_body.h"
+}
+
+template <bool ABF>
+__global__ __launch_bounds__(256, 2) void igemm_reuse4_kernel(GArgs a) {
+  constexpr int NB = 4, MB = 4, TZ = 4, TY = 4, TX = 8, KCI = 16, OCC = 2;
+  constexpr bool BF = true, REUSE = false, REUSE4 = true;
+  constexpr int REUSE4_LA = 3;
 #include "conv_igemm_body.h"
 }
 
@@ -950,7 +981,9 @@
   int nstages, ksplit, sps;
   int stats_rows;
   int64_t workspace_bytes;
+  int variant;
 };
+enum CVariant : int { V_PLAIN = 0, V_REUSE4 = 1, V_REUSE = 2 };
 
 static int expected_out_dim(const mmtta_conv_desc* d, int in) {
   switch (d->op) {
@@ -983,6 +1016,15 @@
   return g_igemm_reuse && g_igemm_pipeline && g_epilogue_vec && g.route == 14 && !g.classes && d->ksize == 3 && g.si == 1 &&
          g.K == 32 && g.N == 32 && g.ksplit == 1 && rowload_operand(x) && quad_aligned(y, quad_bytes(y)) && (!ad || quad_aligned(ad, quad_bytes(ad))) &&
          is_bf16(x) == is_bf16(y) && (!ad || is_bf16(ad) == is_bf16(y)) && ((uintptr_t)rt.bias) % 16 == 0;
+}
+
+static bool igemm_reuse4_applicable(const mmtta_conv_desc* d, const mmtta_tensor* x, const mmtta_tensor* y, const Geometry& g,
+                                    const RunFacts& rt) {
+  const mmtta_tensor* ad = rt.add;
+  return g_igemm_reuse4 && g_igemm_pipeline && g_epilogue_vec && g.route == 12 && !g.classes && d->ksize == 3 && g.si == 1 &&
+         (d->op == MMTTA_CONV_FWD || d->op == MMTTA_CONV_DGRAD) && g.K % 16 == 0 && g.Np % 128 == 0 && y->c % 4 == 0 && rowload_operand(x) &&
+         quad_aligned(y, quad_bytes(y)) && (!ad || quad_aligned(ad, quad_bytes(ad))) && is_bf16(x) == is_bf16(y) &&
+         (!ad || is_bf16(ad) == is_bf16(y)) && ((uintptr_t)rt.bias) % 16 == 0;
 }
 
 static bool cls_fused_operand(const mmtta_tensor* t) {
@@ -1067,6 +1109,7 @@
   } else if (rt && igemm_reuse_applicable(d, x, y, g, *rt)) {
     g.route = C_IGEMM_REUSE;
   }
+  g.variant = g.route == C_IGEMM_REUSE ? V_REUSE : (rt && igemm_reuse4_applicable(d, x, y, g, *rt)) ? V_REUSE4 : V_PLAIN;
   g.stats_rows = g.tiles * stats_rows_per_tile(g);
   g.workspace_bytes = g.ksplit > 1 ? (int64_t)g.ksplit * g.tiles * g.cfg.TZ * g.cfg.TY * g.cfg.TX * g.Np * (int64_t)sizeof(float) : 0;
   return MMTTA_OK;
@@ -1105,7 +1148,7 @@
   t.zext = zmx - zmn; t.yext = ymx - ymn; t.xext = xmx - xmn;
 }
 
-template <int NB, int MB, int TZ, int TY, int TX, int KCI, bool BF, int OCC, bool ABF, bool REUSE = false>
+template <int NB, int MB, int TZ, int TY, int TX, int KCI, bool BF, int OCC, bool ABF, bool REUSE = false, bool REUSE4 = false>
 static int launch_cfg_t(const GArgs& a_in, const Taps* ht, int tiles, hipStream_t s) {
   GArgs a = a_in;
   size_t lds = 0;
@@ -1130,6 +1173,12 @@
   }
   constexpr size_t epi = (4 * (REUSE ? 2 : 1) * EPI_TILE_FLOATS + 4 * 2 * 32) * sizeof(float);
   if (lds < epi) lds = epi;
+  if constexpr (REUSE4) {
+    if (!(a.rowload && a.ovec && a.si == 1 && a.ncls == 1 && a.cls[0].ntaps == 27 && a.Ci == KCI * a.nstages && a.Np % (32 * NB) == 0))
+      return launch_cfg_t<NB, MB, TZ, TY, TX, KCI, BF, OCC, ABF, false, false>(a_in, ht, tiles, s);
+    const size_t need = (size_t)(TZ + 2) * REUSE4_PLANE * 2;
+    if (lds < need) lds = need;
+  }
   if constexpr (REUSE) {
     if (!(a.rowload && a.ovec && a.ksplit == 1 && a.Ci == KCI * a.nstages))
       return launch_cfg_t<NB, MB, TZ, TY, TX, KCI, BF, OCC, ABF, false>(a_in, ht, tiles, s);
@@ -1141,6 +1190,7 @@
   int st;
   void (*kern)(GArgs) = igemm_kernel<NB, MB, TZ, TY, TX, KCI, BF, OCC, ABF>;
   if constexpr (REUSE) kern = igemm_reuse_kernel<ABF>;
+  if constexpr (REUSE4) kern = igemm_reuse4_kernel<ABF>;
   static bool attr_set = false;
   if (!attr_set) {
     (void)hipFuncSetAttribute((const void*)kern, hipFuncAttributeMaxDynamicSharedMemorySize, 160 * 1024);
@@ -1158,20 +1208,21 @@
   return st;
 }
 
-template <int NB, int MB, int TZ, int TY, int TX, int KCI, bool BF, int OCC = 2, bool REUSE = false>
+template <int NB, int MB, int TZ, int TY, int TX, int KCI, bool BF, int OCC = 2, bool REUSE = false, bool REUSE4 = false>
 static int launch_cfg(const GArgs& a, const Taps* ht, int tiles, hipStream_t s) {
   if constexpr (BF) {
     if (a.in_bf || a.out_bf || a.add_bf) {
       MMTTA_CHECK(a.in_bf && a.out_bf && (a.add == nullptr || a.add_bf), MMTTA_ERR_UNSUPPORTED,
                   "conv: input, output and fused add must share one storage type (in %d out %d add %d)", a.in_bf, a.out_bf,
                   a.add_bf);
-      return launch_cfg_t<NB, MB, TZ, TY, TX, KCI, BF, OCC, true, REUSE>(a, ht, tiles, s);
-    }
-  }
-  return launch_cfg_t<NB, MB, TZ, TY, TX, KCI, BF, OCC, false, REUSE>(a, ht, tiles, s);
-}
-
-static int launch_any(int route, const GArgs& a, const Taps* ht, int tiles, hipStream_t s) {
+      return launch_cfg_t<NB, MB, TZ, TY, TX, KCI, BF, OCC, true, REUSE, REUSE4>(a, ht, tiles, s);
+    }
+  }
+  return launch_cfg_t<NB, MB, TZ, TY, TX, KCI, BF, OCC, false, REUSE, REUSE4>(a, ht, tiles, s);
+}
+
+static int launch_any(int route, int variant, const GArgs& a, const Taps* ht, int tiles, hipStream_t s) {
+  if (route == 12 && variant == V_REUSE4) return launch_cfg<4, 4, 4, 4, 8, 16, true, 2, false, true>(a, ht, tiles, s);
   switch (route) {
     case 0: return launch_cfg<1, 4, 8, 8, 8, 8, false>(a, ht, tiles, s);
     case 1: return launch_cfg<2, 4, 4, 8, 8, 16, false>(a, ht, tiles, s);
@@ -1244,7 +1295,7 @@
   GArgs a; Taps ht[8];
   const int st = fill_gargs(c, g, a, ht);
   if (st) return st;
-  return launch_any(g.route, a, ht, g.tiles, c.stream);
+  return launch_any(g.route, g.variant, a, ht, g.tiles, c.stream);
 }
 
 static int cls_fused_run(const ConvCall& c, const Geometry& g) {
@@ -1425,6 +1476,15 @@
   return g.route;
 }
 
+extern "C" int mmtta_conv_variant(const mmtta_conv_desc* d, const mmtta_tensor* x, const mmtta_norm_on_load* x_norm,
+                                  const mmtta_conv_epilogue* epi, const mmtta_tensor* y, int accumulate, const float* stats,
+                                  const float* bias) {
+  Geometry g;
+  const int st = plan_run(d, x, x_norm, epi, y, accumulate, stats, bias, g);
+  if (st) return st < 0 ? st : -st;
+  return g.variant;
+}
+
 extern "C" int mmtta_conv_run(const mmtta_conv_desc* d, const mmtta_tensor* x, const mmtta_norm_on_load* x_norm,
                               const void* packed, const float* bias, const mmtta_conv_epilogue* epi,
                               const mmtta_tensor* y, int accumulate, float* stats, void* workspace,
diff --git a/multimodal_tta_amd/csrc/conv_igemm_body.h b/multimodal_tta_amd/csrc/conv_igemm_body.h
--- a/multimodal_tta_amd/csrc/conv_igemm_body.h
+++ b/multimodal_tta_amd/csrc/conv_igemm_body.h
@@ -1,6 +1,8 @@
   extern __shared__ float lds[];
   static_assert(!REUSE || (NB == 1 && MB == 2 && TZ == 4 && TY == 8 && TX == 8 && KCI == 16 && BF && OCC > 2),
                 "fragment reuse is built for the lean tile");
+  static_assert(!REUSE4 || (!REUSE && NB == 4 && MB == 4 && TZ == 4 && TY == 4 && TX == 8 && KCI == 16 && BF && OCC == 2),
+                "x modulo 4 fragment reuse is built for the four-block 4 x 4 x 8 tile");
   constexpr int VS = BF ? (KCI + 8) : (KCI + 1);
   static_assert(!BF || KCI % 16 == 0, "bf16 stages are multiples of the MFMA K=16");
   constexpr int MT = TZ * TY * TX;
@@ -34,7 +36,7 @@
   const int iz0 = gz0 * a.si + ci.zmin, iy0 = gy0 * a.si + ci.ymin, ix0 = gx0 * a.si + ci.xmin;
 
   const int colbase = (lby * NB + cb) * 32;
-  const bool colact = REUSE || colbase < a.Np;
+  const bool colact = REUSE || REUSE4 || colbase < a.Np;
 
   int rowaddr[MB];
 #pragma unroll
@@ -43,6 +45,8 @@
     row_to_local<TZ, TY, TX, BF>((mg * MB + mb) * 32 + r, zl, yl, xl);
     rowaddr[mb] = (((zl * a.si) * BY + yl * a.si) * LP + xl * a.si) * VS + (BF ? 8 * h : h);
     if constexpr (REUSE) rowaddr[mb] = ((mg * (TY + 2) + (r >> 3) + 4 * ((r >> 2) & 1)) * LDS_PITCH_BF16 + (r & 3)) * VS + 8 * h;
+    if constexpr (REUSE4)
+      rowaddr[mb] = (r >> 3) * REUSE4_PLANE + ((r & 3) * LDS_PITCH_BF16 + 4 * (__popc((unsigned)(r >> 2)) & 1)) * VS + 8 * h;
   }
 
   f32x16 acc[MB];
@@ -62,9 +66,9 @@
   constexpr int RRPP = 256 / RIPR;
   constexpr int RNROW = RBZ * RBY;
   constexpr int RGP = (RNROW + RRPP - 1) / RRPP;
-  constexpr int RPG = !BF ? 0 : (OCC > 2 ? 0 : (KCI == 16 ? (ABF ? 4 : 2) : 0));
+  constexpr int RPG = REUSE4 ? RGP : !BF ? 0 : (OCC > 2 ? 0 : (KCI == 16 ? (ABF ? 4 : 2) : 0));
   constexpr int RGPA = BF ? RGP : 1;
-  const bool fast = REUSE || (BF && a.rowload && ci.ntaps == 27 && a.si == 1);
+  const bool fast = REUSE || REUSE4 || (BF && a.rowload && ci.ntaps == 27 && a.si == 1);
   const bool pipe = fast && RPG > 0;
   Oct8<ABF> gv[RGPA];
   unsigned voff[RGPA];
@@ -90,6 +94,9 @@
   };
   unsigned short* lh0 = reinterpret_cast<unsigned short*>(lds);
   unsigned short* rst = lh0 + (rrsub * LDS_PITCH_BF16 + (REUSE ? reuse_xslot(rbx) : rbx)) * VS + rcv * 8;
+  static_assert(!REUSE4 || RRPP % RBY == 0, "a pass stages whole planes");
+  constexpr int RPASS = RRPP * LDS_PITCH_BF16 * VS + (REUSE4 ? (RRPP / RBY) * 8 : 0);
+  if constexpr (REUSE4) rst += (rrsub / RBY) * 8;
   float* coef = lds + a.coef_off;
   const int cbase = ks0 * KCI, nch = (ks1 - ks0) * KCI;
   if (fast) {
@@ -119,7 +126,7 @@
     __syncthreads();
   }
 
-  constexpr bool CANON_CFG = BF && OCC > 2;
+  constexpr bool CANON_CFG = BF && (OCC > 2 || REUSE4);
   const long long wslab16 = (long long)(a.Kp / 8) * a.Np * 16;
   const char* const wuni = reinterpret_cast<const char*>(wpn) + (a.flip27 ? 26 * wslab16 : 0);
   const long long wstep16 = a.flip27 ? -wslab16 : wslab16;
@@ -132,12 +139,12 @@
   for (int ks = ks0; ks < ks1; ++ks) {
     const int stage = ks;
     const int c0 = ks * KCI;
-    constexpr int WG0 = BF ? (OCC > 2 ? 3 : (KCI == 16 ? 9 : 5)) : 1;
+    constexpr int WG0 = BF ? (REUSE4 ? 3 * REUSE4_LA : OCC > 2 ? 3 : (KCI == 16 ? 9 : 5)) : 1;
     constexpr int WKS = BF ? KCI / 16 : 1;
     uint4 wfirst[WG0][WKS];
     bool wfirst_ok = false;
     if constexpr (BF) {
-      if (REUSE || (colact && ci.ntaps == 27 && ((min(KCI, a.Ci - c0) + 15) >> 4) == WKS)) {
+      if (REUSE || REUSE4 || (colact && ci.ntaps == 27 && ((min(KCI, a.Ci - c0) + 15) >> 4) == WKS)) {
         wfirst_ok = true;
         const long long slabsz8 = (long long)(a.Kp / 8) * a.Np;
         if (CANON_CFG && fast) {
@@ -182,7 +189,7 @@
           pk.x = pack_bf16x2(v[0], v[1]) & okm; pk.y = pack_bf16x2(v[2], v[3]) & okm;
           pk.z = pack_bf16x2(v[4], v[5]) & okm; pk.w = pack_bf16x2(v[6], v[7]) & okm;
           if (RNROW % RRPP == 0 || P + 1 < RGP || RRPP * P + rrsub < RNROW)
-            *reinterpret_cast<uint4*>(rst + P * (RRPP * LDS_PITCH_BF16 * VS)) = pk;
+            *reinterpret_cast<uint4*>(rst + P * RPASS) = pk;
         };
         static_for<0, R1>(commit_item);
         static_for_step<R1, RGP, RB>([&](auto r0) {
@@ -367,6 +374,44 @@
             f[1] = fn[1];
             __builtin_amdgcn_sched_barrier(0);
           }
+        } else if constexpr (REUSE4) {
+          constexpr int NR = 9, LA = REUSE4_LA;
+          static_assert(WG0 == 3 * LA && LA >= 1 && LA < NR && KS == 1 && WKS == 1, "the first weight request is whole box rows");
+          auto rfrag = [&](int j, int m) {
+            return *reinterpret_cast<const uint4*>(lh + rowaddr[0] + (j / 3) * REUSE4_PLANE + ((j % 3) * LDS_PITCH_BF16 + m) * VS);
+          };
+          uint4 wr[NR][3];
+#pragma unroll
+          for (int t = 0; t < WG0; ++t) wr[t / 3][t % 3] = wfirst[t][0];
+          uint4 f[6], fn[4];
+#pragma unroll
+          for (int m = 0; m < 4; ++m) f[m] = rfrag(0, m);
+#pragma unroll
+          for (int g = 0; g < NR; ++g) {
+            if (g + LA < NR) {
+#pragma unroll
+              for (int t = 0; t < 3; ++t) wr[g + LA][t] = wfrag27(c0, (g + LA) * 3 + t, 0);
+            }
+            if (g == NR - 1 - LA && stage + 1 < ks1) issue(stage + 1);
+            __builtin_amdgcn_sched_barrier(0);
+            const bool nxt = g + 1 < NR;
+#pragma unroll
+            for (int k = 0; k < 12; ++k) {
+              const int t = k >> 2, b = k & 3;
+              if (k < 2) f[4 + k] = rfrag(g, 4 + k);
+              else if (k < 6 && nxt) fn[k - 2] = rfrag(g + 1, k - 2);
+              acc[b] = __builtin_amdgcn_mfma_f32_32x32x16_bf16(__builtin_bit_cast(bf16x8, f[b + t]), __builtin_bit_cast(bf16x8, wr[g][t]),
+                                                               acc[b], 0, 0, 0);
+            }
+#pragma unroll
+            for (int k = 0; k < 12; ++k) {
+              if (k < 2 || (k < 6 && nxt)) __builtin_amdgcn_sched_group_barrier(0x100, 1, 0);
+              __builtin_amdgcn_sched_group_barrier(0x008, 1, 0);
+            }
+#pragma unroll
+            for (int m = 0; m < 4; ++m) f[m] = fn[m];
+            __builtin_amdgcn_sched_barrier(0);
+          }
         } else if (nks == KS && ntap == 27) {
           constexpr int G = OCC > 2 ? 3 : (KS == 1 ? 9 : 5);
           constexpr int NG = (27 + G - 1) / G;
@@ -554,16 +599,17 @@
 #pragma unroll
         for (int i = 0; i < 16; ++i) {
           const int row = (i & 3) + 8 * (i >> 2) + 4 * h;
-          const int v = (mg * MB + mb) * 32 + row;
+          int v = (mg * MB + mb) * 32 + row;
+          if constexpr (REUSE4) v = h ? reuse4_row(i, mb, 1) : reuse4_row(i, mb, 0);
           wsb[(long long)v * a.Np] = acc[mb][i];
         }
     }
     return;
   }
-  if (REUSE || a.ovec) {
+  if (REUSE || REUSE4 || a.ovec) {
     constexpr int ETF = (REUSE ? 2 : 1) * EPI_TILE_FLOATS;
     float v_sum[4], v_sq[4];
-    epilogue_vec16<TZ, TY, TX, MB, BF, ABF, REUSE>(a, biasn, ci, acc, lds + wave * ETF, lane, mg * MB, colbase, colact, n, gz0,
+    epilogue_vec16<TZ, TY, TX, MB, BF, ABF, REUSE, REUSE4>(a, biasn, ci, acc, lds + wave * ETF, lane, mg * MB, colbase, colact, n, gz0,
                                                    gy0, gx0, v_sum, v_sq);
     if (a.stats != nullptr) {
       float* red = lds + 4 * ETF;
```

New measurement: 111.2, median of 6. No clear change (+1.0%).
